# LuZWCHA/MLIC

Measured on AMD Instinct MI355X. Metric: images/sec (enc+dec) at 1920×1088 MLICPP_L, 1/2/4/8 GPU; bpp/PSNR Δ vs ref, higher is better.
Workload: dtype f32 (dense convs: f32 via split-fp16 MFMA, 3 terms); 1 GPU; config 2: MLICPP_L compress+decompress of 1920x1088 images (full rANS bitstreams, inputs resident in HBM); model=MLICPP_L, global_batch=32, per_gpu_images=32, weights=rate set(s) [1] of synthetic.RATE_LAMBDAS, parallelism=image-sharded x1 (no cross-GPU context), request_streams=4, schedule=each request stream runs its K steps back to back (no per-step join)

## Files before the change

include/mlic_hip.h:

```cpp
#ifndef MLIC_HIP_H
#define MLIC_HIP_H
#include <stddef.h>
#include <stdint.h>

#ifdef __cplusplus
extern "C" {
#endif

typedef struct mlic_model mlic_model;

const char* mlic_last_error(void);
const char* mlic_version(void);

int mlic_create(const char* model_name, int n, const char* const* names, const float* const* ptrs,
                const int64_t* shapes, const int* ndims, void* stream, mlic_model** out);
int mlic_destroy(mlic_model* m);

int mlic_forward(mlic_model* m, void* stream, const float* x, int B, int H, int W, float* x_hat, float* y_lik,
                 float* z_lik, float vbr_scale);
int mlic_forward_v(mlic_model* m, void* stream, const float* x, int B, int H, int W, float* x_hat, float* y_lik,
                   float* z_lik, const float* vbr_scales);

int mlic_set_entropy_tables(mlic_model* m, const int32_t* gc_cdf, const int32_t* gc_len, const int32_t* gc_off,
                            int gc_n, int gc_stride, const int32_t* eb_cdf, const int32_t* eb_len,
                            const int32_t* eb_off, int eb_n, int eb_stride);

int mlic_set_lanes(mlic_model* m, int lanes);
int mlic_set_priority_base(mlic_model* m, int base);
int mlic_compress(mlic_model* m, void* stream, const float* x, int B, int H, int W, float vbr_scale);
int mlic_compress_v(mlic_model* m, void* stream, const float* x, int B, int H, int W, const float* vbr_scales);
int mlic_encoded_size(mlic_model* m, int b, size_t* y_len, size_t* z_len);
int mlic_encoded_copy(mlic_model* m, int b, uint8_t* y, uint8_t* z);
int mlic_encoded_streams(mlic_model* m, int b, int64_t* n_y, int64_t* n_z, int32_t* y_sym, int32_t* y_idx,
                         int32_t* z_sym);
int mlic_encoded_bits(mlic_model* m, int b, double* y_bits, double* z_bits);
int mlic_batch_stream(mlic_model* m, int first, int count, uint8_t* out, size_t cap, size_t* len);
int mlic_decompress_batch_stream(mlic_model* m, void* stream, const uint8_t* y, size_t y_len, const uint8_t* const* z,
                                 const size_t* z_len, int B, int hz, int wz, float* x_hat, const float* vbr_scales);
int mlic_decompress(mlic_model* m, void* stream, const uint8_t* const* y, const size_t* y_len,
                    const uint8_t* const* z, const size_t* z_len, int B, int hz, int wz, float* x_hat,
                    float vbr_scale);
int mlic_decompress_v(mlic_model* m, void* stream, const uint8_t* const* y, const size_t* y_len,
                      const uint8_t* const* z, const size_t* z_len, int B, int hz, int wz, float* x_hat,
                      const float* vbr_scales);

int mlic_forward_g(mlic_model* m, void* stream, const float* x, int B, int H, int W, float* x_hat, float* y_lik,
                   float* z_lik, const float* gain_plane);
int mlic_compress_g(mlic_model* m, void* stream, const float* x, int B, int H, int W, const float* gain_plane);
int mlic_decompress_g(mlic_model* m, void* stream, const uint8_t* const* y, const size_t* y_len,
                      const uint8_t* const* z, const size_t* z_len, int B, int hz, int wz, float* x_hat,
                      const float* gain_plane);
int mlic_image_roi_levels_u8(void* stream, const uint8_t* mask, const int64_t* mask_strides, int B, int H, int W, int lo,
                             int hi, uint8_t* levels);
int mlic_roi_gain_plane(void* stream, const uint8_t* levels, int B, int hz, int wz, const float* gains_host,
                        int n_levels, float* g);
int mlic_image_sq_err_roi_u8(void* stream, const uint8_t* a, const int64_t* a_strides, const uint8_t* b,
                             const int64_t* b_strides, const uint8_t* mask, const int64_t* mask_strides, int B, int H,
                             int W, uint64_t* out);

int mlic_run_module(mlic_model* m, void* stream, const char* which, int idx, const float* in0, const float* in1,
                    int B, int Cin, int H, int W, float* out);
int mlic_workspace_bytes(mlic_model* m, size_t* arena, size_t* weights);

int mlic_set_precision(mlic_model* m, int precision);
int mlic_set_synthesis_precision(mlic_model* m, int mode);
int mlic_set_poison(mlic_model* m, int on);
int mlic_set_kernel_option(const char* name, int value);
int mlic_get_kernel_option(const char* name, int* value);
int mlic_ab_families(int* built);
int mlic_range_fallbacks(mlic_model* m, int64_t* forward_full, int64_t* forward_gs, int64_t* decompress_gs,
                         int reset);
int mlic_set_profiling(mlic_model* m, int on);
int mlic_profile_read(mlic_model* m, int cat, int64_t* launches, double* ms, double* flops, double* bytes);
int mlic_profile_layers(mlic_model* m, char* buf, size_t cap, size_t* written);

int mlic_profile_categories(int* n);
int mlic_host_stats(mlic_model* m, double* enc_ms, double* dec_ms, double* wait_ms, int reset);
int mlic_profile_category_name(int cat, char* buf, size_t cap);

int mlic_conv_run(void* stream, int impl, const float* x, const float* w, const float* bias, float* y, int B, int Cin,
                  int Cout, int H, int W, int K, int stride, int epi, const float* aux, const float* res);
int mlic_conv_choice(int B, int Cin, int Cout, int H, int W, int K, int stride, int epi, int* impl);
int mlic_dw_run(void* stream, const float* x, const float* w, const float* bias, float* y, int B, int C, int H, int W,
                int stride, int gelu);
int mlic_dwpw_run(void* stream, const float* x, const float* dww, const float* dwb, const float* w, const float* bias,
                  float* y, int B, int C, int Cout, int H, int W, int epi, const float* res);
int mlic_bench_conv(int impl, int B, int Cin, int Cout, int H, int W, int K, int stride, int epi, int iters,
                    double* ms_per, double* tflops);
int mlic_local_attn_mask(void* stream, float* out, int H, int W);
int mlic_local_attn_run(void* stream, int impl, const float* qkv, const float* rel_table, const int32_t* rel_index,
                        float* out, int C, int H, int W, int B, float scale);
int mlic_local_attn_packed_run(void* stream, const float* qkv, const float* rel_table, const int32_t* rel_index,
                               uint16_t* out, int H, int W, int B, float scale);
int mlic_local_attn_packed_half_run(void* stream, const float* qkv, const float* rel_table, const int32_t* rel_index,
                                    uint16_t* out, int H, int W, int B, float scale, int ckbd);
int mlic_linatt_splits(int HW, int* nsplit);
int mlic_linear_attention_run(void* stream, const float* k, const float* v, const float* q, float* out, float* ctx_out,
                              int B, int heads, int hd, int H, int W, int nsplit, int kmask, int qmask);
int mlic_linatt_pack_run(void* stream, const float* q, const float* ctx, uint16_t* out_halves, int B, int heads, int hd,
                         int H, int W, int K, int qmask);
int mlic_ln_channels_run(void* stream, const float* x, const float* gamma, const float* beta, float* y, int B, int C,
                         int HW);
int mlic_taps_gather_run(void* stream, const float* part, const float* bias, float* out, int B, int H, int W);
int mlic_image_sq_err_u8(void* stream, const float* a, const float* b, int B, int64_t n_per, double* out);
int mlic_ms_ssim_scratch_bytes(int B, int C, int H, int W, size_t* bytes);
int mlic_image_ms_ssim_u8(void* stream, const float* a, const int64_t* a_strides, const float* b,
                          const int64_t* b_strides, int B, int C, int H, int W, void* scratch,
                          size_t scratch_bytes, double* out, double* terms);

typedef struct mlic_lpips mlic_lpips;
int mlic_lpips_create(int n, const char* const* names, const float* const* ptrs, const int64_t* shapes,
                      const int* ndims, void* stream, mlic_lpips** out);
int mlic_lpips_destroy(mlic_lpips* h);
int mlic_lpips_set_precision(mlic_lpips* h, int precision);
int mlic_lpips_scratch_bytes(int B, int H, int W, size_t* bytes);
int mlic_image_lpips_u8(mlic_lpips* h, void* stream, const float* a, const int64_t* a_strides, const float* b,
                        const int64_t* b_strides, int B, int H, int W, void* scratch, size_t scratch_bytes,
                        double* out, double* terms);
int mlic_lpips_profile(mlic_lpips* h, int on, double* ms3);
int mlic_lpips_range_fallbacks(mlic_lpips* h, int64_t* count, int reset);

typedef struct mlic_dists mlic_dists;
int mlic_dists_create(int n, const char* const* names, const float* const* ptrs, const int64_t* shapes,
                      const int* ndims, void* stream, mlic_dists** out);
int mlic_dists_destroy(mlic_dists* h);
int mlic_dists_set_precision(mlic_dists* h, int precision);
int mlic_dists_scratch_bytes(int B, int H, int W, size_t* bytes);
int mlic_image_dists_u8(mlic_dists* h, void* stream, const float* a, const int64_t* a_strides, const float* b,
                        const int64_t* b_strides, int B, int H, int W, void* scratch, size_t scratch_bytes,
                        double* out, double* terms);
int mlic_dists_profile(mlic_dists* h, int on, double* ms3);
int mlic_dists_range_fallbacks(mlic_dists* h, int64_t* count, int reset);

int mlic_image_ingest_u8(void* stream, const uint8_t* src, const int64_t* src_strides, int B, int H, int W, float* dst,
                         int Hp, int Wp);
int mlic_image_egress_u8(void* stream, const float* src, const int64_t* src_strides, int B, int H, int W, uint8_t* dst,
                         const int64_t* dst_strides, const uint8_t* ref, const int64_t* ref_strides, uint64_t* sq_err);
int mlic_image_blur3_pad(void* stream, const float* src, const int32_t* src_index, int n, int H, int W, int Hp, int Wp,
                         const float* w9, float* dst);

typedef struct mlic_container_info {
  uint32_t H, W;
  uint32_t hz, wz;
  int32_t level;
  int32_t reserved;
  uint64_t y_off, y_len;
  uint64_t z_off, z_len;
} mlic_container_info;
int mlic_container_bytes(size_t y_len, size_t z_len, int vbr, size_t* bytes);
int mlic_container_write(uint32_t H, uint32_t W, int level, uint32_t hz, uint32_t wz, const uint8_t* y, size_t y_len,
                         const uint8_t* z, size_t z_len, uint8_t* out, size_t cap, size_t* len);
int mlic_container_parse(const uint8_t* data, size_t n, int vbr, int n_levels, uint64_t max_pixels,
                         mlic_container_info* info);

typedef struct mlic_container_roi_info {
  mlic_container_info file;
  uint64_t map_off, map_len;
} mlic_container_roi_info;
int mlic_container_write_roi(uint32_t H, uint32_t W, int level, uint32_t hz, uint32_t wz, const uint8_t* y,
                             size_t y_len, const uint8_t* z, size_t z_len, const uint8_t* levels, uint8_t* out,
                             size_t cap, size_t* len);
int mlic_container_parse_roi(const uint8_t* data, size_t n, int n_levels, uint64_t max_pixels,
                             mlic_container_roi_info* info, uint8_t* levels, size_t levels_cap);

// ... 45 lines not shown
```

mlic_amd/_lib.py:

```python
from __future__ import annotations

import ctypes as C
import os
import threading

_HERE = os.path.dirname(os.path.abspath(__file__))
LIB_PATH = os.environ.get("MLIC_HIP_LIB", os.path.join(_HERE, "libmlic_hip.so"))

_lock = threading.Lock()
_lib = None


class MlicError(RuntimeError):
    pass


class ContainerInfo(C.Structure):
    _fields_ = [("H", C.c_uint32), ("W", C.c_uint32), ("hz", C.c_uint32), ("wz", C.c_uint32), ("level", C.c_int32),
                ("reserved", C.c_int32), ("y_off", C.c_uint64), ("y_len", C.c_uint64), ("z_off", C.c_uint64),
                ("z_len", C.c_uint64)]


class ContainerRoiInfo(C.Structure):
    _fields_ = [("file", ContainerInfo), ("map_off", C.c_uint64), ("map_len", C.c_uint64)]


class ContainerTiledInfo(C.Structure):
    _fields_ = [("H", C.c_uint32), ("W", C.c_uint32), ("T", C.c_uint32), ("V", C.c_uint32), ("ny", C.c_uint32),
                ("nx", C.c_uint32), ("vbr", C.c_int32), ("reserved", C.c_int32), ("table_off", C.c_uint64),
                ("payload_off", C.c_uint64), ("payload_len", C.c_uint64)]


def _sig(lib):
    p, i, i64, f, sz = C.c_void_p, C.c_int, C.c_int64, C.c_float, C.c_size_t
    P = C.POINTER
    lib.mlic_last_error.restype = C.c_char_p
    lib.mlic_version.restype = C.c_char_p
    sigs = {
        "mlic_create": [C.c_char_p, i, P(C.c_char_p), P(p), P(i64), P(i), p, P(p)],
        "mlic_destroy": [p],
        "mlic_forward": [p, p, p, i, i, i, p, p, p, f],
        "mlic_forward_v": [p, p, p, i, i, i, p, p, p, p],
        "mlic_compress_v": [p, p, p, i, i, i, p],
        "mlic_decompress_v": [p, p, P(p), P(sz), P(p), P(sz), i, i, i, p, p],
        "mlic_set_entropy_tables": [p, p, p, p, i, i, p, p, p, i, i],
        "mlic_compress": [p, p, p, i, i, i, f],
        "mlic_encoded_size": [p, i, P(sz), P(sz)],
        "mlic_encoded_copy": [p, i, p, p],
        "mlic_encoded_streams": [p, i, P(i64), P(i64), p, p, p],
        "mlic_decompress": [p, p, P(p), P(sz), P(p), P(sz), i, i, i, p, f],
        "mlic_run_module": [p, p, C.c_char_p, i, p, p, i, i, i, i, p],
        "mlic_workspace_bytes": [p, P(sz), P(sz)],
        "mlic_local_attn_mask": [p, p, i, i],
        "mlic_set_profiling": [p, i],
        "mlic_set_lanes": [p, i],
        "mlic_set_priority_base": [p, i],
        "mlic_set_precision": [p, i],
        "mlic_set_synthesis_precision": [p, i],
        "mlic_set_poison": [p, i],
        "mlic_set_kernel_option": [C.c_char_p, i],
        "mlic_get_kernel_option": [C.c_char_p, P(i)],
        "mlic_ab_families": [P(i)],
        "mlic_batch_stream": [p, i, i, p, sz, P(sz)],
        "mlic_decompress_batch_stream": [p, p, p, sz, P(p), P(sz), i, i, i, p, p],
        "mlic_range_fallbacks": [p, P(i64), P(i64), P(i64), i],
        "mlic_profile_layers": [p, p, sz, P(sz)],
        "mlic_bench_conv": [i, i, i, i, i, i, i, i, i, i, P(C.c_double), P(C.c_double)],
        "mlic_profile_read": [p, i, P(i64), P(C.c_double), P(C.c_double), P(C.c_double)],
        "mlic_profile_categories": [P(i)],
        "mlic_host_stats": [p, P(C.c_double), P(C.c_double), P(C.c_double), i],
        "mlic_profile_category_name": [i, p, sz],
        "mlic_conv_run": [p, i, p, p, p, p, i, i, i, i, i, i, i, i, p, p],
        "mlic_conv_choice": [i, i, i, i, i, i, i, i, P(i)],
        "mlic_dw_run": [p, p, p, p, p, i, i, i, i, i, i],
        "mlic_dwpw_run": [p, p, p, p, p, p, p, i, i, i, i, i, i, p],
        "mlic_local_attn_run": [p, i, p, p, p, p, i, i, i, i, f],
        "mlic_local_attn_packed_run": [p, p, p, p, p, i, i, i, f],
        "mlic_local_attn_packed_half_run": [p, p, p, p, p, i, i, i, f, i],
        "mlic_linatt_splits": [i, P(i)],
        "mlic_linear_attention_run": [p, p, p, p, p, p, i, i, i, i, i, i, i, i],
        "mlic_linatt_pack_run": [p, p, p, p, i, i, i, i, i, i, i],
        "mlic_ln_channels_run": [p, p, p, p, p, i, i, i],
        "mlic_taps_gather_run": [p, p, p, p, i, i, i],
        "mlic_image_sq_err_u8": [p, p, p, i, i64, p],
        "mlic_ms_ssim_scratch_bytes": [i, i, i, i, P(sz)],
        "mlic_image_ms_ssim_u8": [p, p, P(i64), p, P(i64), i, i, i, i, p, sz, p, p],
        "mlic_lpips_create": [i, P(C.c_char_p), P(p), P(i64), P(i), p, P(p)],
        "mlic_lpips_destroy": [p],
        "mlic_lpips_set_precision": [p, i],
        "mlic_lpips_scratch_bytes": [i, i, i, P(sz)],
        "mlic_image_lpips_u8": [p, p, p, P(i64), p, P(i64), i, i, i, p, sz, p, p],
        "mlic_lpips_range_fallbacks": [p, P(i64), i],
        "mlic_lpips_profile": [p, i, P(C.c_double)],
        "mlic_dists_create": [i, P(C.c_char_p), P(p), P(i64), P(i), p, P(p)],
        "mlic_dists_destroy": [p],
        "mlic_dists_set_precision": [p, i],
        "mlic_dists_scratch_bytes": [i, i, i, P(sz)],
        "mlic_image_dists_u8": [p, p, p, P(i64), p, P(i64), i, i, i, p, sz, p, p],
        "mlic_dists_range_fallbacks": [p, P(i64), i],
        "mlic_dists_profile": [p, i, P(C.c_double)],
        "mlic_image_ingest_u8": [p, p, P(i64), i, i, i, p, i, i],
        "mlic_image_egress_u8": [p, p, P(i64), i, i, i, p, P(i64), p, P(i64), p],
        "mlic_image_blur3_pad": [p, p, p, i, i, i, i, i, p, p],
        "mlic_container_bytes": [sz, sz, i, P(sz)],
        "mlic_container_write": [C.c_uint32, C.c_uint32, i, C.c_uint32, C.c_uint32, p, sz, p, sz, p, sz, P(sz)],
        "mlic_container_parse": [p, sz, i, i, C.c_uint64, P(ContainerInfo)],
        "mlic_forward_g": [p, p, p, i, i, i, p, p, p, p],
        "mlic_compress_g": [p, p, p, i, i, i, p],
        "mlic_decompress_g": [p, p, P(p), P(sz), P(p), P(sz), i, i, i, p, p],
        "mlic_image_roi_levels_u8": [p, p, P(i64), i, i, i, i, i, p],
        "mlic_roi_gain_plane": [p, p, i, i, i, P(f), i, p],
        "mlic_image_sq_err_roi_u8": [p, p, P(i64), p, P(i64), p, P(i64), i, i, i, p],
        "mlic_container_write_roi": [C.c_uint32, C.c_uint32, i, C.c_uint32, C.c_uint32, p, sz, p, sz, p, p, sz, P(sz)],
        "mlic_container_parse_roi": [p, sz, i, C.c_uint64, P(ContainerRoiInfo), p, sz],
        "mlic_tile_grid": [C.c_uint32, C.c_uint32, C.c_uint32, C.c_uint32, P(C.c_uint32), P(C.c_uint32), p, sz],
        "mlic_image_tile_blend_u8": [p, p, p, i, i, i, i, i, i, i, i, p, P(i64), p, P(i64), p],
        "mlic_container_write_tiled": [C.c_uint32, C.c_uint32, C.c_uint32, C.c_uint32, i, p, p, sz, p, sz, P(sz)],
        "mlic_container_parse_tiled": [p, sz, C.c_uint64, P(ContainerTiledInfo)],
        "mlic_container_tiled_tile": [p, sz, P(ContainerTiledInfo), C.c_uint64, P(C.c_uint64), P(C.c_uint64)],
        "mlic_encode_image_u8": [p, p, p, P(i64), i, i, f, i, p, sz, P(sz)],
        "mlic_encode_image_u8_budget": [p, p, p, P(i64), i, i, f, i, C.c_double, i, p, sz, P(sz), P(i)],
        "mlic_decode_image_u8": [p, p, p, sz, i, C.c_uint64, p, p, P(i64), sz, P(i), P(i), P(i)],
        "mlic_neglog2_sum": [p, p, i, i64, p],
        "mlic_gaussian_likelihood": [p, p, p, p, i64, f, p],
        "mlic_scale_indexes": [p, p, i64, p, i, p],
        "mlic_encoded_bits": [p, i, P(C.c_double), P(C.c_double)],
        "mlic_pmf_to_quantized_cdf": [p, i, i, p],
        "mlic_rans_encode": [p, p, i64, p, p, p, i, i, p, sz, P(sz)],
        "mlic_rans_decode": [p, sz, p, i64, p, p, p, i, i, p],
        "mlic_rans_decode_narrow": [p, sz, p, i64, i, p, p, p, i, i, p, P(i)],
    }
    for name, args in sigs.items():
        fn = getattr(lib, name)
        fn.argtypes = args
        fn.restype = C.c_int
    return lib


def _check_build_record():
    import json
    from . import build as _build
    if os.environ.get("MLIC_HIP_LIB"):
        return
    rec_path = _build.RECORD
    if not os.path.exists(rec_path):
        raise MlicError(f"{rec_path} missing: rebuild with `python -m mlic_amd.build` (records the sources the "
                        f"library was built from)")
    with open(rec_path) as f:
        rec = json.load(f)
    if rec.get("sources_sha256") != _build.source_digest():
        raise MlicError("libmlic_hip.so was built from other sources than the ones in this tree (stale build): "
                        "rebuild with `python -m mlic_amd.build`")


def lib():
# ... 30 lines not shown
```

mlic_amd/csrc/capi.cpp:

```cpp
#include "../../include/mlic_hip.h"

#include <algorithm>
#include <cmath>
#include <cstring>
#include <string>
#include <vector>

#include "container.h"
#include "model.h"
#include "options.h"

using namespace mlic;

struct mlic_model {
  Model* impl;
  float* stage = nullptr;
  size_t stage_bytes = 0;
  float* stage2 = nullptr;
  size_t stage2_bytes = 0;
  int enc_H = 0, enc_W = 0, enc_level = -1;
  int enc_passes = 0;
};

struct mlic_lpips {
// ... 462 lines not shown

int mlic_conv_choice(int B, int Cin, int Cout, int H, int W, int K, int stride, int epi, int* impl) {
  return guard([&] {
    MLIC_CHECK(impl && B > 0 && Cin > 0 && Cout > 0 && H > 0 && W > 0 && (K == 1 || K == 3 || K == 5) && stride > 0,
               "conv_choice: bad arguments");
    const int pad = K / 2;
    ConvParams P{};
    P.nseg = 1;
    P.seg[0] = {nullptr, Cin, (int64_t)Cin * H * W};
    P.Cin = Cin; P.H = H; P.W = W; P.Cout = Cout; P.K = K; P.stride = stride; P.pad = pad;
    P.Ho = (H + 2 * pad - K) / stride + 1;
    P.Wo = (W + 2 * pad - K) / stride + 1;
    P.B = B;
    P.epi = epi;
    const int cin_pad = (Cin + 31) / 32 * 32;
    static const _Float16 tag = 0;
    const bool split = Cin >= 16;
    const bool x4 = split && Cout >= 64;
    const ConvWeights cw{nullptr, split ? &tag : nullptr, split ? &tag : nullptr, cin_pad, x4 ? &tag : nullptr, 0};
    *impl = conv_select(P, cw, 2);
  });
}

int mlic_conv_run(void* stream, int impl, const float* x, const float* w, const float* bias, float* y, int B, int Cin,
                  int Cout, int H, int W, int K, int stride, int epi, const float* aux, const float* res) {
  return guard([&] {
    hipStream_t st = (hipStream_t)stream;
    const int pad = K / 2;
    const int Ho = (H + 2 * pad - K) / stride + 1, Wo = (W + 2 * pad - K) / stride + 1;
    const int cin_pad = (Cin + 31) / 32 * 32;
    const int64_t nw = (int64_t)Cout * Cin * K * K, nh = (int64_t)Cout * K * K * cin_pad;
    float* wp = nullptr;
    _Float16 *wh = nullptr, *wl = nullptr;
    HIP_OK(hipMallocAsync((void**)&wp, nw * 4, st));
    HIP_OK(hipMallocAsync((void**)&wh, nh * 2, st));
    HIP_OK(hipMallocAsync((void**)&wl, nh * 2, st));
    pack_conv(w, wp, Cout, Cin, K * K, st);
    const int wexp = split_weights(w, wh, wl, Cout, Cin, K * K, cin_pad, true, st);
    ConvParams P{};
    P.nseg = 1;
    P.seg[0] = {x, Cin, (int64_t)Cin * H * W};
    P.Cin = Cin; P.H = H; P.W = W; P.Cout = Cout; P.Ho = Ho; P.Wo = Wo; P.K = K; P.stride = stride; P.pad = pad;
    P.wpk = wp; P.bias = bias; P.out = y; P.B = B; P.epi = epi;
    const bool shuffle = (epi & EPI_SHUFFLE) != 0;
    MLIC_CHECK(!shuffle || Cout % 4 == 0, "shuffle needs Cout % 4 == 0");
    P.out_cs = shuffle ? (int64_t)4 * Ho * Wo : (int64_t)Ho * Wo;
    P.out_bs = (int64_t)Cout * Ho * Wo;
    MLIC_CHECK(!(epi & (EPI_GDN | EPI_IGDN)) || aux, "GDN epilogue needs aux");
    MLIC_CHECK(!(epi & EPI_RES) || res, "residual epilogue needs res");
    P.aux = aux; P.aux_bs = (int64_t)Cout * Ho * Wo;
    P.res = res; P.res_bs = P.out_bs;
    _Float16 *wx = nullptr, *wxh = nullptr;
    if (conv_x4_ok(P, cin_pad)) {
      HIP_OK(hipMallocAsync((void**)&wx, x4_weight_halves(Cout, K * K, cin_pad) * 2, st));
      x4_pack_weights(wh, wl, Cout, K * K, cin_pad, wx, st);
      if (impl == CONV_X4H) {
        HIP_OK(hipMallocAsync((void**)&wxh, x4_weight_halves(Cout, K * K, cin_pad, true) * 2, st));
        x4_pack_weights(wh, wl, Cout, K * K, cin_pad, wxh, st, true);
      }
    }
    ConvWeights cw{wp, wh, wl, cin_pad, wx, wexp};
    cw.wx4h = wxh;
    const int which = impl < 0 ? conv_select(P, cw, 2) : impl;
    if (which == CONV_X4H) MLIC_CHECK(conv_x4_ok(P, cin_pad), "x4: unsupported shape");
    if (which == CONV_PW) MLIC_CHECK(pw_resident_ok(P, cin_pad), "pw_resident: unsupported shape");
    if (which == CONV_NARROW) MLIC_CHECK(conv_narrow_ok(P), "narrow: unsupported shape");
    if (which == CONV_SMALLCIN) MLIC_CHECK(conv_smallcin_ok(P), "smallcin: unsupported shape");
    if (which == CONV_HALO) MLIC_CHECK(conv_halo_ok(P, cin_pad), "halo: unsupported shape");
    if (which == CONV_X4) MLIC_CHECK(conv_x4_ok(P, cin_pad), "x4: unsupported shape");
    void* ws = nullptr;
    const int64_t wsb = conv_ws_bytes(which, P, cw);
    if (wsb > 0) HIP_OK(hipMallocAsync(&ws, wsb, st));
    conv_run(which, P, cw, st, ws);
    if (ws) HIP_OK(hipFreeAsync(ws, st));
    if (wx) HIP_OK(hipFreeAsync(wx, st));
    if (wxh) HIP_OK(hipFreeAsync(wxh, st));
    HIP_OK(hipFreeAsync(wp, st));
    HIP_OK(hipFreeAsync(wh, st));
    HIP_OK(hipFreeAsync(wl, st));
    HIP_OK(hipStreamSynchronize(st));
  });
}

int mlic_dw_run(void* stream, const float* x, const float* w, const float* bias, float* y, int B, int C, int H, int W,
                int stride, int gelu) {
  return guard([&] {
    DwParams P{};
    P.nseg = 1;
    P.seg[0] = {x, C, (int64_t)C * H * W};
    P.C = C; P.H = H; P.W = W; P.stride = stride;
    P.Ho = (H - 1) / stride + 1;
    P.Wo = (W - 1) / stride + 1;
    P.w = w; P.bias = bias; P.out = y; P.out_bs = (int64_t)C * P.Ho * P.Wo; P.gelu = gelu; P.B = B;
    dw3x3(P, (hipStream_t)stream);
    HIP_OK(hipStreamSynchronize((hipStream_t)stream));
  });
}

int mlic_dwpw_run(void* stream, const float* x, const float* dww, const float* dwb, const float* w, const float* bias,
                  float* y, int B, int C, int Cout, int H, int W, int epi, const float* res) {
  return guard([&] {
    hipStream_t st = (hipStream_t)stream;
    const int cin_pad = (C + 31) / 32 * 32;
    const int64_t nh = (int64_t)Cout * cin_pad;
    _Float16 *wh = nullptr, *wl = nullptr;
    HIP_OK(hipMallocAsync((void**)&wh, nh * 2, st));
    HIP_OK(hipMallocAsync((void**)&wl, nh * 2, st));
    const int wexp = split_weights(w, wh, wl, Cout, C, 1, cin_pad, true, st);
    ConvParams P{};
    P.nseg = 1;
    P.seg[0] = {x, C, (int64_t)C * H * W};
    P.Cin = C; P.H = H; P.W = W; P.Cout = Cout; P.Ho = H; P.Wo = W; P.K = 1; P.stride = 1; P.pad = 0;
    P.wexp = wexp; P.bias = bias; P.out = y; P.B = B; P.epi = epi;
    P.out_cs = (int64_t)H * W;
    P.out_bs = (int64_t)Cout * H * W;
    MLIC_CHECK(!(epi & EPI_RES) || res, "residual epilogue needs res");
    P.res = res; P.res_bs = P.out_bs;
    MLIC_CHECK(dwpw_ok(P, cin_pad), "dwpw: unsupported shape");
    dwpw_forward(P, wh, wl, cin_pad, dww, dwb, st);
    HIP_OK(hipFreeAsync(wh, st));
    HIP_OK(hipFreeAsync(wl, st));
    HIP_OK(hipStreamSynchronize(st));
  });
}

int mlic_local_attn_run(void* stream, int impl, const float* qkv, const float* rel_table, const int32_t* rel_index,
                        float* out, int C, int H, int W, int B, float scale) {
  return guard([&] {
    LocalAttnParams A{};
    A.qkv = qkv;
    A.qkv_bs = (int64_t)3 * C * H * W;
    A.out = out;
    A.out_bs = (int64_t)25 * C * H * W;
    A.rel_table = rel_table;
    A.rel_index = rel_index;
    A.scale = scale;
    A.C = C; A.H = H; A.W = W; A.B = B;
    if (impl == 0) local_attn_valu(A, (hipStream_t)stream);
    else local_attn_mfma(A, (hipStream_t)stream);
    HIP_OK(hipStreamSynchronize((hipStream_t)stream));
  });
}

int mlic_local_attn_packed_run(void* stream, const float* qkv, const float* rel_table, const int32_t* rel_index,
                               uint16_t* out, int H, int W, int B, float scale) {
  return guard([&] {
    LocalAttnParams A{};
    A.qkv = qkv;
    A.qkv_bs = (int64_t)3 * 32 * H * W;
    A.rel_table = rel_table;
    A.rel_index = rel_index;
    A.scale = scale;
    A.C = 32; A.H = H; A.W = W; A.B = B;
    local_attn_packed(A, reinterpret_cast<_Float16*>(out), (H * W + 31) / 32 * 32, (hipStream_t)stream);
    HIP_OK(hipStreamSynchronize((hipStream_t)stream));
  });
}

int mlic_local_attn_packed_half_run(void* stream, const float* qkv, const float* rel_table, const int32_t* rel_index,
                                    uint16_t* out, int H, int W, int B, float scale, int ckbd) {
  return guard([&] {
    MLIC_CHECK(ckbd == 1 || ckbd == 2, "ckbd: 1 (anchors) or 2 (non-anchors)");
    LocalAttnParams A{};
    A.qkv = qkv;
    A.qkv_bs = (int64_t)3 * 32 * H * W;
    A.rel_table = rel_table;
// ... 602 lines not shown
```

mlic_amd/csrc/common.h:

```cpp
#pragma once
#include <hip/hip_runtime.h>

#include <atomic>
#include <cstdint>
#include <cstdio>
#include <stdexcept>
#include <string>

namespace mlic {

struct Error : std::runtime_error {
  using std::runtime_error::runtime_error;
};

#define MLIC_CHECK(cond, msg)                                                                  \
  do {                                                                                          \
    if (!(cond)) throw ::mlic::Error(std::string("mlic: ") + (msg) + " [" #cond "] at " +       \
                                     __FILE__ + ":" + std::to_string(__LINE__));               \
  } while (0)

#define HIP_OK(expr)                                                                            \
  do {                                                                                          \
    hipError_t _e = (expr);                                                                     \
    if (_e != hipSuccess)                                                                       \
      throw ::mlic::Error(std::string("hip: ") + hipGetErrorString(_e) + " in " #expr " at " + \
                          __FILE__ + ":" + std::to_string(__LINE__));                           \
  } while (0)

struct View {
  float* p = nullptr;
  int C = 0, H = 0, W = 0;
  int64_t bs = 0;
  int64_t hw() const { return (int64_t)H * W; }
  View ch(int c0, int nc) const {
    View v = *this;
    v.p = p + (int64_t)c0 * hw();
    v.C = nc;
    return v;
  }
};

enum Epi : int {
  EPI_NONE = 0,
  EPI_GELU = 1,
  EPI_GDN = 2,
  EPI_IGDN = 4,
  EPI_TANH_HALF = 8,
  EPI_MASK_ANCHOR = 16,
  EPI_MASK_NONANCHOR = 32,
  EPI_RES = 64,
  EPI_SHUFFLE = 128,
  EPI_SQUARE_IN = 256,
  EPI_RELU_IN = 512,
};

constexpr int MAXSEG = 6;

struct Seg {
  const float* p;
  int C;
  int64_t bs;
};

struct ConvParams {
  Seg seg[MAXSEG];
  int nseg;
  int Cin, H, W;
  int Cout, Ho, Wo;
  int K, stride, pad;
  const float* wpk;
  int wexp;
  const float* bias;
  float* out;
  int64_t out_bs;
  int64_t out_cs;
  int epi;
  const float* aux;
  int64_t aux_bs;
  const float* res;
  int64_t res_bs;
  int B;
  int* rflag;
  int in_mask;
  int scatter;
  const float* skx;
  int64_t skx_bs;
  int sk_cin, sk_H, sk_W;
  const float* skw;
  const float* skb;
};

__device__ __forceinline__ float softmax_exp(float x) { return __builtin_amdgcn_exp2f(x * 1.44269504088896341f); }

template <int HD>
__device__ __forceinline__ void query_softmax(const float* qp, int HW, float (&q)[HD]) {
  float mx = -3.0e38f;
#pragma unroll
  for (int c = 0; c < HD; ++c) {
    q[c] = qp[(int64_t)c * HW];
    mx = fmaxf(mx, q[c]);
  }
  float sum = 0.0f;
#pragma unroll
  for (int c = 0; c < HD; ++c) {
    q[c] = softmax_exp(q[c] - mx);
    sum += q[c];
  }
  const float inv = 1.0f / sum;
#pragma unroll
  for (int c = 0; c < HD; ++c) q[c] *= inv;
}

__device__ __forceinline__ bool f16_unsafe(float v) { return (__float_as_uint(v) & 0x7fffffffu) >= 0x477ff000u; }
__device__ __forceinline__ void range_report(int* flag, bool bad) {
  if (bad && flag) atomicOr(flag, 1);
}
__device__ __forceinline__ float gelu_erf(float x) {
  const float ax = __builtin_fabsf(x);
  const float z = ax * 0.70710678118654752440f;
  const float t = __builtin_amdgcn_rcpf(__builtin_fmaf(0.3275911f, z, 1.0f));
  float q = __builtin_fmaf(0.5307027101516724f, t, -0.726576030254364f);
  q = __builtin_fmaf(q, t, 0.710706889629364f);
  q = __builtin_fmaf(q, t, -0.14224836230278015f);
  q = __builtin_fmaf(q, t, 0.1274147927761078f);
  q = q * t;
  const float e = __builtin_amdgcn_exp2f(z * (z * -1.44269504088896341f));
  return __builtin_fmaxf(x, 0.0f) - ax * (q * e);
}
typedef float mlic_float2 __attribute__((ext_vector_type(2)));
__device__ __forceinline__ mlic_float2 gelu_erf2(mlic_float2 x) {
  const mlic_float2 ax = {__builtin_fabsf(x.x), __builtin_fabsf(x.y)};
  const mlic_float2 z = ax * 0.70710678118654752440f;
  const mlic_float2 d = __builtin_elementwise_fma(mlic_float2{0.3275911f, 0.3275911f}, z, mlic_float2{1.0f, 1.0f});
  const mlic_float2 t = {__builtin_amdgcn_rcpf(d.x), __builtin_amdgcn_rcpf(d.y)};
  mlic_float2 q = __builtin_elementwise_fma(mlic_float2{0.5307027101516724f, 0.5307027101516724f}, t,
                                            mlic_float2{-0.726576030254364f, -0.726576030254364f});
  q = __builtin_elementwise_fma(q, t, mlic_float2{0.710706889629364f, 0.710706889629364f});
  q = __builtin_elementwise_fma(q, t, mlic_float2{-0.14224836230278015f, -0.14224836230278015f});
  q = __builtin_elementwise_fma(q, t, mlic_float2{0.1274147927761078f, 0.1274147927761078f});
  q = q * t;
  const mlic_float2 zz = z * (z * -1.44269504088896341f);
  const mlic_float2 e = {__builtin_amdgcn_exp2f(zz.x), __builtin_amdgcn_exp2f(zz.y)};
  const mlic_float2 m = {__builtin_fmaxf(x.x, 0.0f), __builtin_fmaxf(x.y, 0.0f)};
  return m - ax * (q * e);
}
__device__ __forceinline__ float gelu_erff(float x) { return 0.5f * x * (1.0f + erff(x * 0.70710678118654752440f)); }
__device__ __forceinline__ float gelu_epi(float x) {
#ifndef MLIC_GELU_EPI_ERFF
  return gelu_erf(x);
#else
  return gelu_erff(x);
#endif
}

__device__ __forceinline__ float gdn_apply(float x, float v, bool inverse) {
  return inverse ? x * __builtin_amdgcn_sqrtf(v) : x * __builtin_amdgcn_rsqf(v);
}

__device__ __forceinline__ bool is_anchor(int h, int w) { return ((h + w) & 1) == 1; }

__device__ __forceinline__ void conv_store(const ConvParams& P, int b, int co, int p, float v) {
  const int epi = P.epi;
  const int HWo = P.Ho * P.Wo;
  v = ldexpf(v, -P.wexp);
  if (P.bias) v += P.bias[co];
  if (epi & EPI_GELU) v = gelu_epi(v);
  if (epi & (EPI_GDN | EPI_IGDN)) {
    const float x = P.aux[(int64_t)b * P.aux_bs + (int64_t)co * HWo + p];
    v = gdn_apply(x, v, (epi & EPI_GDN) == 0);
  }
  if (epi & EPI_TANH_HALF) v = 0.5f * tanhf(v);
  int oh = 0, ow = 0;
  if (epi & (EPI_MASK_ANCHOR | EPI_MASK_NONANCHOR | EPI_SHUFFLE)) {
    oh = p / P.Wo;
    ow = p - oh * P.Wo;
  }
  if (epi & EPI_MASK_ANCHOR) v = is_anchor(oh, ow) ? v : 0.0f;
  if (epi & EPI_MASK_NONANCHOR) v = is_anchor(oh, ow) ? 0.0f : v;
  int64_t off;
  if (epi & EPI_SHUFFLE) {
    const int oc = co >> 2;
    const int y2 = 2 * oh + ((co >> 1) & 1), x2 = 2 * ow + (co & 1);
    off = (int64_t)oc * P.out_cs + (int64_t)y2 * (2 * P.Wo) + x2;
  } else {
    off = (int64_t)co * P.out_cs + p;
  }
  if (epi & EPI_RES) v = P.res[(int64_t)b * P.res_bs + off] + v;
  P.out[(int64_t)b * P.out_bs + off] = v;
}

__host__ __device__ __forceinline__ bool conv_vec_ok(const ConvParams& P) {
  const uintptr_t a = reinterpret_cast<uintptr_t>(P.out) | reinterpret_cast<uintptr_t>(P.aux) |
                      reinterpret_cast<uintptr_t>(P.res);
  return (a & 15) == 0 && ((P.out_bs | P.out_cs | P.aux_bs | P.res_bs) & 3) == 0 && (P.Wo & 3) == 0;
}

__device__ __forceinline__ void conv_store4(const ConvParams& P, int b, int co, int p, float4 v) {
  const int epi = P.epi;
  float a[4] = {v.x, v.y, v.z, v.w};
  const float bi = P.bias ? P.bias[co] : 0.0f;
#pragma unroll
  for (int e = 0; e < 4; ++e) {
    a[e] = ldexpf(a[e], -P.wexp) + bi;
    if (epi & EPI_GELU) a[e] = gelu_epi(a[e]);
  }
  if (epi & (EPI_GDN | EPI_IGDN)) {
    const float4 x = *reinterpret_cast<const float4*>(P.aux + (int64_t)b * P.aux_bs + (int64_t)co * P.Ho * P.Wo + p);
    const float xs[4] = {x.x, x.y, x.z, x.w};
#pragma unroll
    for (int e = 0; e < 4; ++e) a[e] = gdn_apply(xs[e], a[e], (epi & EPI_GDN) == 0);
  }
  if (epi & EPI_TANH_HALF) {
#pragma unroll
    for (int e = 0; e < 4; ++e) a[e] = 0.5f * tanhf(a[e]);
  }
  if (epi & (EPI_MASK_ANCHOR | EPI_MASK_NONANCHOR)) {
    const int oh = p / P.Wo, ow = p - oh * P.Wo;
#pragma unroll
    for (int e = 0; e < 4; ++e) {
      const bool anc = is_anchor(oh, ow + e);
      if ((epi & EPI_MASK_ANCHOR) && !anc) a[e] = 0.0f;
      if ((epi & EPI_MASK_NONANCHOR) && anc) a[e] = 0.0f;
    }
  }
  const int64_t off = (int64_t)co * P.out_cs + p;
  if (epi & EPI_RES) {
    const float4 r = *reinterpret_cast<const float4*>(P.res + (int64_t)b * P.res_bs + off);
    a[0] = r.x + a[0]; a[1] = r.y + a[1]; a[2] = r.z + a[2]; a[3] = r.w + a[3];
  }
  *reinterpret_cast<float4*>(P.out + (int64_t)b * P.out_bs + off) = make_float4(a[0], a[1], a[2], a[3]);
}

__device__ __forceinline__ void conv_store_shuf4(const ConvParams& P, int b, int co0, int p, float4 v) {
  const int epi = P.epi;
  float a[4] = {v.x, v.y, v.z, v.w};
  const float b0 = P.bias ? P.bias[co0] : 0.0f, b1 = P.bias ? P.bias[co0 + 1] : 0.0f;
  a[0] = ldexpf(a[0], -P.wexp) + b0; a[1] = ldexpf(a[1], -P.wexp) + b1;
  a[2] = ldexpf(a[2], -P.wexp) + b0; a[3] = ldexpf(a[3], -P.wexp) + b1;
#pragma unroll
  for (int e = 0; e < 4; ++e) {
    if (epi & EPI_GELU) a[e] = gelu_epi(a[e]);
    if (epi & EPI_TANH_HALF) a[e] = 0.5f * tanhf(a[e]);
  }
  const int oh = p / P.Wo, ow = p - oh * P.Wo;
  const int64_t off = (int64_t)(co0 >> 2) * P.out_cs + (int64_t)(2 * oh + ((co0 >> 1) & 1)) * (2 * P.Wo) + 2 * ow;
  if (epi & EPI_RES) {
    const float4 r = *reinterpret_cast<const float4*>(P.res + (int64_t)b * P.res_bs + off);
    a[0] = r.x + a[0]; a[1] = r.y + a[1]; a[2] = r.z + a[2]; a[3] = r.w + a[3];
  }
  *reinterpret_cast<float4*>(P.out + (int64_t)b * P.out_bs + off) = make_float4(a[0], a[1], a[2], a[3]);
}

inline int device_cu_count() {
  static std::atomic<int> cache[64];
  int dev = 0;
  HIP_OK(hipGetDevice(&dev));
  MLIC_CHECK(dev >= 0 && dev < 64, "device id");
  int n = cache[dev].load(std::memory_order_relaxed);
  if (n == 0) {
    HIP_OK(hipDeviceGetAttribute(&n, hipDeviceAttributeMultiprocessorCount, dev));
    cache[dev].store(n, std::memory_order_relaxed);
  }
  return n;
}

}
```

mlic_amd/csrc/conv_dispatch.cpp:

```cpp
#include "kernels.h"

namespace mlic {

static bool x4_k_on(int K) {
  static const int mask = [] {
    const char* e = opt_str(OPT_X4_K);
    int m = 0;
    for (const char* c = e ? e : "135"; *c; ++c)
      if (*c >= '0' && *c <= '9') m |= 1 << (*c - '0');
    return m;
  }();
  return (mask >> K) & 1;
}

int conv_select(const ConvParams& P, const ConvWeights& w, int precision) {
  if (P.in_mask || P.scatter) return CONV_PW;
  if (conv_smallcin_ok(P)) return CONV_SMALLCIN;
  if (conv_narrow_ok(P)) return CONV_NARROW;
  if (precision == 0 || !w.wh) return CONV_F32;
  if (precision == 1) return CONV_X3;
  if ((int64_t)P.Ho * P.Wo >= 1024 && pw_resident_ok(P, w.cin_pad)) return CONV_PW;
  const bool big1 = (int64_t)P.Cin * P.Cout >= (1 << 18), mid1 = P.Cin >= 192 && P.Cout >= 192;
  const bool x4_shape = P.K == 1 ? (big1 || mid1) : P.Cout >= 64;
  if (w.wx4 && opt(OPT_X4) && x4_k_on(P.K) && x4_shape && conv_x4_ok(P, w.cin_pad)) return CONV_X4;
  if (P.K == 5 && conv_halo_ok(P, w.cin_pad) &&
      (int64_t)((P.Cout + 127) / 128) * ((P.Wo + 31) / 32) * ((P.Ho + 3) / 4) >= 8)
    return CONV_HALO;
  return CONV_X3V2;
}

int conv_prof_cat(int impl, const ConvParams& P) {
  switch (impl) {
    case CONV_F32: return PCAT_CONV_F32 + conv_variant(P);
    case CONV_X3: return PCAT_CONV_X3 + conv_f16x3_variant(P);
    case CONV_X3V2: {
      const int v = conv_x3v2_variant(P);
      return v == 3 ? PCAT_CONV_X3V2_WIDE : PCAT_CONV_X3V2 + v;
    }
    case CONV_PW: return PCAT_CONV_PW;
    case CONV_NARROW: return PCAT_CONV_NARROW;
    case CONV_HALO: return PCAT_CONV_HALO;
    case CONV_X4:
    case CONV_X4H: return PCAT_CONV_X4;
    default: return PCAT_CONV_SMALLCIN;
  }
}

int64_t conv_ws_bytes(int impl, const ConvParams& P, const ConvWeights& w) {
  if (impl != CONV_X4 && impl != CONV_X4H) return 0;
  const bool hi = impl == CONV_X4H;
  const int64_t act = x4_direct_ok(P, hi) ? 0 : (2 * x4_act_halves(P, w.cin_pad, hi) + 255) / 256 * 256;
  return act + x4_part_bytes(P, w.cin_pad, hi);
}

void conv_run(int impl, const ConvParams& P0, const ConvWeights& w, hipStream_t st, void* ws) {
  ConvParams P = P0;
  const bool split = impl == CONV_X3 || impl == CONV_X3V2 || impl == CONV_PW || impl == CONV_HALO || impl == CONV_X4 ||
                     impl == CONV_X4H;
  P.wexp = split ? w.wexp : 0;
  MLIC_CHECK(!(P.epi & EPI_RELU_IN) || impl == CONV_X4 || impl == CONV_X4H,
             "EPI_RELU_IN: only x4's operand pack applies it");
  switch (impl) {
    case CONV_F32: conv_forward(P, st); break;
    case CONV_X3: conv_f16x3_forward(P, w.wh, w.wl, w.cin_pad, st); break;
    case CONV_X3V2: conv_x3v2_forward(P, w.wh, w.wl, w.cin_pad, st); break;
    case CONV_PW: pw_resident_forward(P, w.wh, w.wl, w.cin_pad, st); break;
    case CONV_NARROW: conv_narrow_forward(P, st); break;
    case CONV_SMALLCIN: conv_smallcin_forward(P, st); break;
    case CONV_HALO: conv_halo_forward(P, w.wh, w.wl, w.cin_pad, st); break;
    case CONV_X4:
    case CONV_X4H: {
      const bool hi = impl == CONV_X4H;
      const _Float16* wx = hi ? w.wx4h : w.wx4;
      const bool direct = x4_direct_ok(P, hi);
      MLIC_CHECK((ws || direct) && wx, "conv_x4: workspace and packed weights required");
      _Float16* act = direct ? nullptr : static_cast<_Float16*>(ws);
      const int64_t abytes = direct ? 0 : (2 * x4_act_halves(P, w.cin_pad, hi) + 255) / 256 * 256;
      float* part = x4_part_bytes(P, w.cin_pad, hi) > 0 ? reinterpret_cast<float*>(static_cast<char*>(ws) + abytes)
                                                         : nullptr;
      if (!direct) x4_pack_act(P, w.cin_pad, act, st, hi);
      conv_x4_forward(P, act, wx, w.cin_pad, st, part, hi);
      break;
    }
    default: throw Error("mlic: unknown conv implementation " + std::to_string(impl));
  }
}

const char* prof_cat_name(int cat) {
  static const char* names[PCAT_COUNT] = {
      "conv_mfma_kernel<64,64>",     "conv_mfma_kernel<64,128>",  "conv_mfma_kernel<128,64>",
      "conv_mfma_kernel<128,128>",   "conv_f16x3_kernel<32,256>", "conv_f16x3_kernel<64,128>",
      "conv_f16x3_kernel<128,64>",   "conv_f16x3_kernel<128,128>", "conv_x3v2_kernel<64,128>",
      "conv_x3v2_kernel<128,256>",   "conv_x3v2_kernel<128,128>", "conv_x3v2_kernel<256,256>",
      "pw_resident_kernel",
      "conv3x3_narrow_kernel",       "conv1x1_smallcin_kernel",   "conv_halo_kernel",
      "dw3x3_kernel",
      "local_attn_kernel",           "linear_attention",          "elementwise",
      "conv_x4_kernel",              "chain_kernel",              "dwpw_kernel"};
  return (cat >= 0 && cat < PCAT_COUNT) ? names[cat] : "";
}

}
```

mlic_amd/csrc/conv_pw.hip:

```cpp
#include "common.h"
#include "kernels.h"

namespace mlic {

typedef float floatx16 __attribute__((ext_vector_type(16)));
typedef _Float16 half8 __attribute__((ext_vector_type(8)));

constexpr int PW_WAVES = 8;
constexpr int PW_THREADS = PW_WAVES * 64;
constexpr int LDS_BYTES = 160 * 1024;

__device__ __forceinline__ __amdgpu_buffer_rsrc_t make_rsrc(const float* base, uint32_t bytes) {
  const uint64_t a = reinterpret_cast<uint64_t>(base);
  const uint32_t lo = __builtin_amdgcn_readfirstlane((uint32_t)a);
  const uint32_t hi = __builtin_amdgcn_readfirstlane((uint32_t)(a >> 32));
  float* pb = reinterpret_cast<float*>(((uint64_t)hi << 32) | lo);
  return __builtin_amdgcn_make_buffer_rsrc(pb, 0, bytes, 0x00020000);
}

__device__ __forceinline__ void opaque(uint32_t& v) { asm volatile("" : "+s"(v)); }

template <int CIN>
constexpr int pw_apitch() { return CIN + 8; }

template <int CIN, int CT, int MODE, bool RES, int XF = 0>
__global__ __launch_bounds__(PW_THREADS) void pw_resident_kernel(ConvParams P, const _Float16* __restrict__ wh,
                                                                  const _Float16* __restrict__ wl, int cin_pad) {
  constexpr int KS = CIN / 16;
  constexpr int APITCH = pw_apitch<CIN>();
  constexpr int ROWS = CT * 32;
  constexpr int A_SZ = ROWS * APITCH;
  static_assert(CIN % 16 == 0 && 2 * A_SZ * 2 + ROWS * 4 <= LDS_BYTES, "pw_resident: weights must fit in LDS");
  __shared__ __attribute__((aligned(16))) _Float16 sm[2 * A_SZ + 2 * ROWS];
  float* sbias = reinterpret_cast<float*>(sm + 2 * A_SZ);

  const int tid = threadIdx.x;
  constexpr int QPR = CIN / 8;
  constexpr int NIT = (ROWS * QPR + PW_THREADS - 1) / PW_THREADS;
  uint4 wst[2 * NIT];
#pragma unroll
  for (int it = 0; it < NIT; ++it) {
    const int id = tid + it * PW_THREADS;
    const int row = id / QPR, q = id - row * QPR;
    wst[2 * it] = wst[2 * it + 1] = make_uint4(0, 0, 0, 0);
    if (id < ROWS * QPR && row < P.Cout) {
      wst[2 * it] = *reinterpret_cast<const uint4*>(wh + (int64_t)row * cin_pad + 8 * q);
      wst[2 * it + 1] = *reinterpret_cast<const uint4*>(wl + (int64_t)row * cin_pad + 8 * q);
    }
  }
  const float bias_v = (tid < ROWS && P.bias && tid < P.Cout) ? P.bias[tid] : 0.0f;
#pragma unroll
  for (int it = 0; it < NIT; ++it) {
    const int id = tid + it * PW_THREADS;
    const int row = id / QPR, q = id - row * QPR;
    if (id < ROWS * QPR) {
      *reinterpret_cast<uint4*>(sm + row * APITCH + 8 * q) = wst[2 * it];
      *reinterpret_cast<uint4*>(sm + A_SZ + row * APITCH + 8 * q) = wst[2 * it + 1];
    }
  }
  static_assert(ROWS <= PW_THREADS, "one bias per thread");
  if (tid < ROWS) sbias[tid] = bias_v;
  __syncthreads();

  const int lane = tid & 63;
  const int wave = __builtin_amdgcn_readfirstlane(tid >> 6);
  const int l32 = lane & 31, h = lane >> 5;
  const int HW = P.Ho * P.Wo;
  const int tpi = (HW + 31) >> 5;
  const int ntiles = tpi * P.B;
  const int tstride = gridDim.x * PW_WAVES;
  int tile = blockIdx.x * PW_WAVES + wave;
  if (tile >= ntiles) return;

  constexpr bool square = MODE == 2 || MODE == 3;
  const float* xbase = P.seg[0].p;
  const int64_t xbs = P.seg[0].bs;
  const uint32_t hw4 = (uint32_t)(P.H * P.W) * 4u;
  const uint32_t ho4 = (uint32_t)HW * 4u;
  const uint32_t img_bytes = (uint32_t)CIN * hw4;
  const int S = P.stride;

  auto rsrc_of = [&](int t) { return make_rsrc(xbase + (int64_t)(t / tpi) * xbs, img_bytes); };
  auto voff_of = [&](int t) {
    const int b = t / tpi;
    const int p = min(((t - b * tpi) << 5) + l32, HW - 1);
    const int pin = S == 1 ? p : (p / P.Wo) * S * P.W + (p % P.Wo) * S;
    return (uint32_t)pin * 4u + (uint32_t)(8 * h) * hw4;
  };

  constexpr int D = KS / 2;
  float ring[D][8];
  {
    const auto rs = rsrc_of(tile);
    const uint32_t vo = voff_of(tile);
#pragma unroll
    for (int j = 0; j < D; ++j)
#pragma unroll
      for (int i = 0; i < 8; ++i)
        ring[j][i] = __builtin_bit_cast(float, __builtin_amdgcn_raw_buffer_load_b32(rs, vo, (16 * j + i) * hw4, 0));
  }

  const _Float16* Ah = sm + l32 * APITCH + 8 * h;
  const _Float16* Al = Ah + A_SZ;
  bool bad = false;
  for (; tile < ntiles; tile += tstride) {
    int nt = tile + tstride;
    if (nt >= ntiles) nt = tile;
    const auto rsc = rsrc_of(tile);
// ... 6 lines not shown
      const int pt = min(((tile - bt * tpi) << 5) + l32, HW - 1);
      const int yt = pt / P.Wo;
      kin = is_anchor(yt, pt - yt * P.Wo) == (P.in_mask == 1);
    }

    floatx16 acc[CT];
#pragma unroll
    for (int c = 0; c < CT; ++c)
#pragma unroll
      for (int r = 0; r < 16; ++r) acc[c][r] = 0.0f;
    uint32_t so = (uint32_t)(16 * D) * hw4;
    opaque(so);

#pragma unroll
    for (int j = 0; j < KS; ++j) {
      half8 bh, bl;
#pragma unroll
      for (int i = 0; i < 8; ++i) {
        float v = ring[j % D][i];
        if (XF & 1) v = kin ? v : 0.0f;
        if (square) v *= v;
        const _Float16 hv = (_Float16)v;
        bh[i] = hv;
        bl[i] = (_Float16)(v - (float)hv);
      }
      if (j == KS - D) {
        so = 0;
        opaque(so);
      }
#pragma unroll
      for (int i = 0; i < 8; ++i) {
        ring[j % D][i] = __builtin_bit_cast(float, j + D < KS ? __builtin_amdgcn_raw_buffer_load_b32(rsc, voc, so, 0)
                                                              : __builtin_amdgcn_raw_buffer_load_b32(rsn, von, so, 0));
        so += (i == 7) ? 9 * hw4 : hw4;
        opaque(so);
      }
      __builtin_amdgcn_sched_barrier(0);
#ifndef MLIC_PW_ABL
#define MLIC_PW_ABL 0
#endif
      if (MLIC_PW_ABL & 1) {
        const half8 ah0 = *reinterpret_cast<const half8*>(Ah + 16 * j);
        acc[0] = __builtin_amdgcn_mfma_f32_32x32x16_f16(ah0, bh + bl, acc[0], 0, 0, 0);
        continue;
      }
#pragma unroll
      for (int c = 0; c < CT; c += 2) {
        const int c1 = (c + 1 < CT) ? c + 1 : c;
        const half8 ah0 = *reinterpret_cast<const half8*>(Ah + c * 32 * APITCH + 16 * j);
        const half8 al0 = *reinterpret_cast<const half8*>(Al + c * 32 * APITCH + 16 * j);
        const half8 ah1 = *reinterpret_cast<const half8*>(Ah + c1 * 32 * APITCH + 16 * j);
        const half8 al1 = *reinterpret_cast<const half8*>(Al + c1 * 32 * APITCH + 16 * j);
        acc[c] = __builtin_amdgcn_mfma_f32_32x32x16_f16(al0, bh, acc[c], 0, 0, 0);
        if (c1 != c) acc[c1] = __builtin_amdgcn_mfma_f32_32x32x16_f16(al1, bh, acc[c1], 0, 0, 0);
        acc[c] = __builtin_amdgcn_mfma_f32_32x32x16_f16(ah0, bl, acc[c], 0, 0, 0);
        if (c1 != c) acc[c1] = __builtin_amdgcn_mfma_f32_32x32x16_f16(ah1, bl, acc[c1], 0, 0, 0);
        acc[c] = __builtin_amdgcn_mfma_f32_32x32x16_f16(ah0, bh, acc[c], 0, 0, 0);
        if (c1 != c) acc[c1] = __builtin_amdgcn_mfma_f32_32x32x16_f16(ah1, bh, acc[c1], 0, 0, 0);
      }
    }

    const int b = tile / tpi;
    const int p = ((tile - b * tpi) << 5) + l32;
    const uint32_t cs4 = (uint32_t)P.out_cs * 4u;
    int pf = p;
    if (XF & 2) {
      const int y = p / P.Wo, q = p - y * P.Wo;
      pf = y * 2 * P.Wo + 2 * q + ((y + (P.scatter == 1 ? 1 : 0)) & 1);
    }
    const uint32_t vo_out = (uint32_t)pf * 4u + (uint32_t)(4 * h) * cs4;
    const auto rs_out = make_rsrc(P.out + (int64_t)b * P.out_bs, (uint32_t)P.Cout * cs4);
    constexpr bool gdn = MODE == 2 || MODE == 3, igdn = MODE == 3, gelu = MODE == 1, tanh_mask = MODE == 4;
    bool keep = true;
    if (tanh_mask && (P.epi & (EPI_MASK_ANCHOR | EPI_MASK_NONANCHOR))) {
      const int oh = p / P.Wo, ow = p - oh * P.Wo;
      keep = is_anchor(oh, ow) == ((P.epi & EPI_MASK_ANCHOR) != 0);
    }
    constexpr bool res = RES;
    const auto rs_aux = make_rsrc(gdn ? P.aux + (int64_t)b * P.aux_bs : P.out, gdn ? (uint32_t)P.Cout * ho4 : 0u);
    const uint32_t vo_aux = (uint32_t)p * 4u + (uint32_t)(4 * h) * ho4;
    const auto rs_res = make_rsrc(res ? P.res + (int64_t)b * P.res_bs : P.out, res ? (uint32_t)P.Cout * cs4 : 0u);
    const float* sb = sbias + 4 * h;
    const float unscale = ldexpf(1.0f, -P.wexp);
    uint32_t so_o = 0, so_a = 0;
    if (p < HW) {
#pragma unroll
      for (int c = 0; c < CT; ++c) {
        float xa[16], xr[16];
        uint32_t oo = so_o, oa = so_a;
#pragma unroll
        for (int r = 0; r < 16; ++r) {
          if (r > 0) {
            const uint32_t step = ((r & 3) == 0) ? 5u : 1u;
            oo += step * cs4;
            oa += step * ho4;
            opaque(oo);
            opaque(oa);
          }
          if (gdn) xa[r] = __builtin_bit_cast(float, __builtin_amdgcn_raw_buffer_load_b32(rs_aux, vo_aux, oa, 0));
          xr[r] = res ? __builtin_bit_cast(float, __builtin_amdgcn_raw_buffer_load_b32(rs_res, vo_out, oo, 0)) : 0.0f;
        }
        float4 bq[4];
#pragma unroll
        for (int g = 0; g < 4; ++g) bq[g] = *reinterpret_cast<const float4*>(sb + c * 32 + 8 * g);
        float v[16];
#pragma unroll
        for (int r = 0; r < 16; ++r) {
          const float4 b4 = bq[r >> 2];
          const float bv = (r & 3) == 0 ? b4.x : (r & 3) == 1 ? b4.y : (r & 3) == 2 ? b4.z : b4.w;
          float x = __builtin_fmaf(acc[c][r], unscale, bv);
          bad |= !(fabsf(x) <= 3.4e38f);
          if (gelu) x = gelu_erf(x);
          if (gdn) x = gdn_apply(xa[r], x, igdn);
          if (tanh_mask) x = keep ? 0.5f * tanhf(x) : 0.0f;
          v[r] = x + xr[r];
        }
        oo = so_o;
        if ((MLIC_PW_ABL & 2) && P.Cout > 0) {
          asm volatile("" :: "v"(v[0]), "v"(v[5]), "v"(v[10]), "v"(v[15]));
        } else
        if (c * 32 + 32 <= P.Cout) {
#pragma unroll
          for (int r = 0; r < 16; ++r) {
            if (r > 0) {
              oo += (((r & 3) == 0) ? 5u : 1u) * cs4;
              opaque(oo);
            }
            __builtin_amdgcn_raw_buffer_store_b32(__builtin_bit_cast(uint32_t, v[r]), rs_out, vo_out, oo, 0);
          }
        } else {
#pragma unroll
          for (int r = 0; r < 16; ++r) {
            if (r > 0) {
              oo += (((r & 3) == 0) ? 5u : 1u) * cs4;
              opaque(oo);
            }
            if (c * 32 + (r & 3) + 8 * (r >> 2) + 4 * h < P.Cout)
              __builtin_amdgcn_raw_buffer_store_b32(__builtin_bit_cast(uint32_t, v[r]), rs_out, vo_out, oo, 0);
          }
        }
        so_o += 32 * cs4;
        so_a += 32 * ho4;
        opaque(so_o);
        opaque(so_a);
      }
    }
  }
  range_report(P.rflag, bad);
}

static int num_cus() { return device_cu_count(); }

static int pw_mode(const ConvParams& P) {
  const int e = P.epi & ~EPI_RES;
  if (e == EPI_NONE) return 0;
  if (e == EPI_GELU) return 1;
  if (e == (EPI_GDN | EPI_SQUARE_IN)) return 2;
  if (e == (EPI_IGDN | EPI_SQUARE_IN)) return 3;
  if (e == EPI_TANH_HALF || e == (EPI_TANH_HALF | EPI_MASK_ANCHOR) || e == (EPI_TANH_HALF | EPI_MASK_NONANCHOR))
    return 4;
  return -1;
}

#define PW_ALL(X, CIN, CT) \
  X(CIN, CT, 0, 0) X(CIN, CT, 0, 1) X(CIN, CT, 1, 0) X(CIN, CT, 1, 1) \
  X(CIN, CT, 2, 0) X(CIN, CT, 2, 1) X(CIN, CT, 3, 0) X(CIN, CT, 3, 1)
#define PW_COMBOS(X)                                                                              \
  PW_ALL(X, 96, 3) PW_ALL(X, 128, 4) PW_ALL(X, 160, 5) PW_ALL(X, 192, 6)                          \
                           \
  PW_ALL(X, 48, 2)                                                                                \
                               \
  X(192, 4, 0, 0) X(96, 4, 0, 0) X(48, 4, 0, 0)                                                   \
     \
  X(224, 4, 1, 0) X(128, 1, 4, 1)                                                                 \
                                   \
  X(32, 6, 1, 0) X(64, 6, 1, 0) X(96, 6, 1, 0) X(128, 6, 1, 0) X(160, 6, 1, 0) X(192, 4, 1, 0)   \
                     \
  X(32, 1, 0, 0) X(64, 2, 0, 0) X(32, 3, 0, 0)                                                    \
        \
  X(96, 4, 1, 0) X(64, 4, 1, 0) X(128, 2, 0, 1) X(96, 2, 0, 0)
#define PW_XCOMBOS(X) X(32, 1, 0, 0, 1) X(128, 1, 4, 1, 2) X(128, 2, 0, 1, 2)

static int pw_xf(const ConvParams& P) { return (P.in_mask ? 1 : 0) | (P.scatter ? 2 : 0); }

bool pw_resident_ok(const ConvParams& P, int cin_pad) {
  if (P.K != 1 || (P.stride != 1 && P.stride != 2) || P.pad != 0 || P.nseg != 1) return false;
  const int mode = pw_mode(P);
  if (mode < 0) return false;
  if (P.Ho != (P.H - 1) / P.stride + 1 || P.Wo != (P.W - 1) / P.stride + 1) return false;
  if (P.seg[0].C != P.Cin || cin_pad < P.Cin) return false;
  if (P.stride != 1 && (mode == 2 || mode == 3 || mode == 4)) return false;
  const int64_t HW = (int64_t)P.H * P.W;
  if ((int64_t)P.Cin * HW * 4 >= (1ll << 31) || (int64_t)P.Cout * HW * 4 >= (1ll << 31)) return false;
  const int ct = (P.Cout + 31) / 32;
  const int res = (P.epi & EPI_RES) ? 1 : 0;
  if (const int xf = pw_xf(P)) {
    if (P.stride != 1 || (unsigned)P.in_mask > 2u || (unsigned)P.scatter > 2u) return false;
    if (P.scatter && ((P.epi & (EPI_MASK_ANCHOR | EPI_MASK_NONANCHOR)) || P.out_cs != 2 * HW ||
                      (int64_t)P.Cout * P.out_cs * 4 >= (1ll << 31)))
      return false;
#define MLIC_PW_XOK(CIN, CT, M, R, X) \
  if (P.Cin == CIN && ct == CT && mode == M && res == R && xf == X) return true;
    PW_XCOMBOS(MLIC_PW_XOK)
#undef MLIC_PW_XOK
    return false;
  }
#define MLIC_PW_OK(CIN, CT, M, R) \
  if (P.Cin == CIN && ct == CT && mode == M && res == R) return true;
  PW_COMBOS(MLIC_PW_OK)
#undef MLIC_PW_OK
  return false;
}

template <int CIN, int CT, int M, bool R, int XF = 0>
static void launch_pw(const ConvParams& P, const _Float16* wh, const _Float16* wl, int cin_pad, hipStream_t st) {
  const int64_t ntiles = (int64_t)((P.Ho * P.Wo + 31) / 32) * P.B;
  const int64_t want = (ntiles + PW_WAVES - 1) / PW_WAVES;
  const dim3 grid((unsigned)std::min<int64_t>(want, (int64_t)num_cus()));
  hipLaunchKernelGGL((pw_resident_kernel<CIN, CT, M, R, XF>), grid, dim3(PW_THREADS), 0, st, P, wh, wl, cin_pad);
  HIP_OK(hipGetLastError());
}

void pw_resident_forward(const ConvParams& P, const _Float16* wh, const _Float16* wl, int cin_pad, hipStream_t st) {
  MLIC_CHECK(pw_resident_ok(P, cin_pad), "pw_resident: unsupported shape");
  const int mode = pw_mode(P);
  const int ct = (P.Cout + 31) / 32;
  const int res = (P.epi & EPI_RES) ? 1 : 0;
  if (const int xf = pw_xf(P)) {
#define MLIC_PW_XRUN(CIN, CT, M, R, X)                                 \
  if (P.Cin == CIN && ct == CT && mode == M && res == R && xf == X) {  \
    launch_pw<CIN, CT, M, R != 0, X>(P, wh, wl, cin_pad, st);          \
    return;                                                            \
  }
    PW_XCOMBOS(MLIC_PW_XRUN)
#undef MLIC_PW_XRUN
  }
  if (pw3_ok(P, cin_pad)) return pw3_forward(P, wh, wl, cin_pad, st);
  MLIC_CHECK(!P.skx, "pw_resident: the computed skip residual is pw3's");
#define MLIC_PW_RUN(CIN, CT, M, R)                                  \
  if (P.Cin == CIN && ct == CT && mode == M && res == R) {          \
    launch_pw<CIN, CT, M, R != 0>(P, wh, wl, cin_pad, st);          \
    return;                                                         \
  }
  PW_COMBOS(MLIC_PW_RUN)
#undef MLIC_PW_RUN
}

constexpr int NR_TH = 16, NR_TW = 128, NR_CC = 2;
constexpr int NR_PH = NR_TH + 2, NR_PQ = NR_TW / 4 + 2;
constexpr int NR_PITCH = NR_PQ * 4;
constexpr int NR_PATCH4 = NR_CC * NR_PH * NR_PQ;
constexpr int NR_STAGE = (NR_PATCH4 + 255) / 256;

template <int COUT>
__global__ __launch_bounds__(256) void conv3x3_narrow_kernel(ConvParams P) {
  typedef float float2v __attribute__((ext_vector_type(2)));
  typedef float float4v __attribute__((ext_vector_type(4)));
  constexpr int NW = NR_CC * 9 * COUT / 2;
  static_assert(COUT % 2 == 0, "Cout pairs");
  __shared__ __attribute__((aligned(16))) float4v sp[2][NR_PATCH4];
  __shared__ __attribute__((aligned(16))) float4v swp[2][NW];
  const int tid = threadIdx.x;
  const int tx = tid & 15, ty = tid >> 4;
  const int ow0 = blockIdx.x * NR_TW, oh0 = blockIdx.y * NR_TH;
  const int b = blockIdx.z;
  const int H = P.H, W = P.W, W4 = W >> 2;
  const int64_t HW = (int64_t)H * W;
  const float4v* x4 = reinterpret_cast<const float4v*>(P.seg[0].p + (int64_t)b * P.seg[0].bs);
  const int nchunk = (P.Cin + NR_CC - 1) / NR_CC;
  const float* w = P.wpk;
  constexpr int WSTAGE = (NW + 255) / 256;

  float4v stage[NR_STAGE];
  float4v wst[WSTAGE];
  auto load = [&](int ch) {
#pragma unroll
    for (int s = 0; s < NR_STAGE; ++s) {
      const int e = tid + s * 256;
      float4v v = {0.f, 0.f, 0.f, 0.f};
      if (e < NR_PATCH4) {
        const int c = e / (NR_PH * NR_PQ), rem = e - c * (NR_PH * NR_PQ);
        const int py = rem / NR_PQ, pq = rem - py * NR_PQ;
        const int ci = ch * NR_CC + c, ih = oh0 + py - 1, iq = (ow0 >> 2) - 1 + pq;
        if (ci < P.Cin && ih >= 0 && ih < H && iq >= 0 && iq < W4) v = x4[(ci * HW >> 2) + (int64_t)ih * W4 + iq];
      }
      stage[s] = v;
    }
#pragma unroll
    for (int s = 0; s < WSTAGE; ++s) {
      const int e = tid + s * 256;
      float4v v = {0.f, 0.f, 0.f, 0.f};
      if (e < NW) {
        const int c = e / (9 * COUT / 2), rem = e - c * (9 * COUT / 2);
        const int tap = rem / (COUT / 2), cp = rem - tap * (COUT / 2);
        const int ci = ch * NR_CC + c;
        if (ci < P.Cin) {
          const float* wr = w + ((int64_t)tap * P.Cin + ci) * COUT + 2 * cp;
          v = float4v{wr[0], wr[0], wr[1], wr[1]};
        }
      }
      wst[s] = v;
    }
  };
  auto store = [&](int buf) {
#pragma unroll
    for (int s = 0; s < NR_STAGE; ++s) {
      const int e = tid + s * 256;
      if (e < NR_PATCH4) sp[buf][e] = stage[s];
    }
#pragma unroll
// ... 235 lines not shown
```

mlic_amd/csrc/conv_x4.hip:

```cpp
#include "common.h"
#include "kernels.h"

#include <cstdio>
#include <type_traits>
#include <utility>
#include <vector>

namespace mlic {

typedef float floatx4 __attribute__((ext_vector_type(4)));
typedef _Float16 half8 __attribute__((ext_vector_type(8)));

namespace {
constexpr int X4T = 512;
constexpr int TR = 8, TC = 32;
constexpr int BN = TR * TC;
constexpr int ROWB = 128;
constexpr int ROWH = 64;

#ifndef MLIC_X4_HALO_PITCH
#define MLIC_X4_HALO_PITCH 144
#endif
#ifndef MLIC_X4_HALO_SKEW
#define MLIC_X4_HALO_SKEW (MLIC_X4_HALO_PITCH == 144)
#endif
constexpr int HPITCH = MLIC_X4_HALO_PITCH;
constexpr bool HPAD = HPITCH != ROWB;
constexpr bool HSKEW = MLIC_X4_HALO_SKEW;
static_assert(HPITCH == ROWB || (HPITCH >= ROWB + 16 && HPITCH % 16 == 0), "x4 halo pitch");
static_assert(!HSKEW || HPITCH == 144, "x4 halo skew: 9-granule rows");
__host__ __device__ constexpr int hgran(int g) {
  return (HSKEW ? ((g >> 1) & 1) + (g >> 2) * 4 + (g & 1) * 16 : g) * 16;
}
constexpr int HLO = hgran(4) - hgran(0);
static_assert(hgran(5) - hgran(1) == HLO && hgran(6) - hgran(2) == HLO && hgran(7) - hgran(3) == HLO, "x4 halo lo offset");
constexpr int HTAIL = (HPAD && hgran(7) + 16 > HPITCH) ? hgran(7) + 16 - HPITCH : 0;
constexpr int x4_halo_lds(int K, int bm) {
  return 2 * bm * ROWB + 2 * (TR + K - 1) * (TC + K - 1) * HPITCH + HTAIL;
}

__device__ __forceinline__ int swz(int row) { return (row >> 1) & 7; }

__device__ __forceinline__ void glds16(const void* src, void* lds) {
  __builtin_amdgcn_global_load_lds((const __attribute__((address_space(1))) void*)src,
                                   (__attribute__((address_space(3))) void*)lds, 16, 0, 0);
}

__device__ __forceinline__ void glds16_asm(const void* src, const void* lds) {
  const uint32_t l = __builtin_amdgcn_readfirstlane(
      (uint32_t)reinterpret_cast<uintptr_t>((const __attribute__((address_space(3))) void*)lds));
  asm volatile("s_mov_b32 m0, %1\n\ts_nop 0\n\tglobal_load_lds_dwordx4 %0, off" : : "v"(src), "s"(l) : "m0");
}

__device__ __forceinline__ half8 lds_frag(const char* base, int row, int granule) {
  return *reinterpret_cast<const half8*>(base + row * ROWB + ((granule ^ swz(row)) << 4));
}
}

#ifndef MLIC_X4_ABL_RS
#define MLIC_X4_ABL_RS 0
#endif
#ifndef MLIC_X4_SPREAD
#define MLIC_X4_SPREAD 0
#endif
#ifndef MLIC_X4_STAGGER
#define MLIC_X4_STAGGER 0
#endif
template <int K, int BM, bool RS, bool HI, bool DIR = false, bool HALO = false>
__global__ __launch_bounds__(X4T) void conv_x4_kernel(ConvParams P, const _Float16* __restrict__ act,
                                                      const _Float16* __restrict__ wx, int nchunk, int H, int W,
                                                      int abl, int nsplit) {
  constexpr int KK = K * K;
  constexpr int WAVES_M = BM == 192 ? 4 : (BM == 96 || BM == 224) ? 2 : BM / 64, WAVES_N = 8 / WAVES_M;
  constexpr int WN = BN / WAVES_N;
  constexpr int TM = BM / (16 * WAVES_M), TN = WN / 16;
  constexpr int WR = 16 * TM;
  constexpr int A_BYTES = BM * ROWB, B_BYTES = BN * ROWB;
  constexpr int NAB = RS ? 2 : 3;
  constexpr int HR = TR + K - 1, HC = TC + K - 1, HLINES = HR * HC;
  constexpr int BSLOT = HALO ? HLINES * HPITCH : B_BYTES;
  constexpr int B_OFF = NAB * A_BYTES, LDS = NAB * A_BYTES + 2 * BSLOT + (HALO ? HTAIL : 0);
  static_assert(!HALO || LDS == x4_halo_lds(K, BM), "x4 halo: the launch rule's footprint");
  constexpr int NA = A_BYTES / 1024 / 8;
  constexpr int NB = B_BYTES / 1024 / 8;
  static_assert(NA >= 1 && NB == 4 && LDS <= 160 * 1024, "x4 tile");
  static_assert(!HALO || (RS && !DIR && K > 1), "x4 halo: register-staged K x K only");
  __shared__ __attribute__((aligned(1024))) char sm[LDS];

  const int tid = threadIdx.x, lane = tid & 63, wave = tid >> 6;
  const int wm = wave / WAVES_N, wn = wave % WAVES_N;
  const int pad = K / 2;
  const int npix = P.Ho * P.Wo;
  const int S = K == 1 ? 1 : P.stride;
  const int Hp = (K == 1 ? H : P.H) + 2 * pad, Wp = (K == 1 ? W : P.W) + 2 * pad;
  const int ntx = (W + TC - 1) / TC;
  const int nct = gridDim.x, npt = gridDim.y, nblk = nct * npt;
  const int bid = blockIdx.y * nct + blockIdx.x;
  int logical = bid;
  if (nblk >= 16) {
    const int xcd = bid & 7, q = nblk >> 3, r = nblk & 7;
    logical = (xcd < r ? xcd * (q + 1) : r * (q + 1) + (xcd - r) * q) + (bid >> 3);
  }
  constexpr int XG = 4;
  int ct, pt;
  if (K == 1 && nct >= 2 * XG) {
    const int band = XG * npt, g = logical / band, first = g * XG, r = logical - g * band;
    const int gs = min(XG, nct - first);
    ct = first + r % gs;
    pt = r / gs;
  } else {
    ct = logical % nct;
    pt = logical / nct;
  }
  const int oy0 = (pt / ntx) * TR, ox0 = (pt % ntx) * TC;
  const int b = blockIdx.z % P.B, split = blockIdx.z / P.B;
  const int nsteps = nchunk * KK;
  const int s0 = HALO ? split * nchunk / nsplit * KK : split * nsteps / nsplit;
  const int s1 = HALO ? (split + 1) * nchunk / nsplit * KK : (split + 1) * nsteps / nsplit;
  if (nsplit > 1) P.out += (int64_t)split * P.B * P.out_bs;

  const int64_t plane = (int64_t)Hp * Wp * ROWH;
  const _Float16* bsrc[NB];
#pragma unroll
  for (int i = 0; i < NB; ++i) {
    const int n = (wave * NB + i) * 8 + (lane >> 3);
    const int oy = min(oy0 + n / TC, H - 1), ox = min(ox0 + n % TC, W - 1);
    const int G = (lane & 7) ^ swz(n);
    bsrc[i] = act + (int64_t)b * nchunk * plane + ((int64_t)oy * S * Wp + ox * S) * ROWH + G * 8;
  }
  const _Float16* asrc = wx + ((int64_t)ct * nsteps * BM) * ROWH + (wave * NA) * 512 + lane * 8;

  auto glds_one = [&](int g, int sb, int sa, int abuf) {
    if (g < NB) {
      const int cc = sb / KK, tap = sb - cc * KK;
      const int ky = tap / K, kx = tap - ky * K;
      const int64_t d = cc * plane + ((int64_t)ky * Wp + kx) * ROWH;
      glds16_asm(bsrc[g] + d, sm + B_OFF + (sb & 1) * B_BYTES + (wave * NB + g) * 1024);
    } else {
      const int i = g - NB;
      glds16_asm(asrc + (int64_t)sa * BM * ROWH + i * 512, sm + abuf * A_BYTES + (wave * NA + i) * 1024);
    }
  };
  constexpr int NG = NA + NB;

  floatx4 acc[TM][TN];
#pragma unroll
  for (int i = 0; i < TM; ++i)
#pragma unroll
    for (int j = 0; j < TN; ++j) acc[i][j] = floatx4{0.f, 0.f, 0.f, 0.f};

  const int G = lane >> 4, l16 = lane & 15;
// ... 282 lines not shown
#pragma unroll
    for (int i = 0; i < TM; ++i) {
      const int row = wm * WR + i * 16 + l16;
      ah[i] = lds_frag(As, row, G);
      al[i] = lds_frag(As, row, G + 4);
    }
    half8 bh[2], bl[2];
    bh[0] = lds_frag(Bs, wn * WN + l16, G);
    bl[0] = lds_frag(Bs, wn * WN + l16, G + 4);
#pragma unroll
    for (int j = 0; j < TN; ++j) {
      if (!(abl & 1)) {
#pragma unroll
        for (int g = j * NG / TN; g < (j + 1) * NG / TN; ++g) glds_one(g, sb, sa, anext);
      }
      __builtin_amdgcn_sched_barrier(0);
      if (j + 1 < TN) {
        const int n = wn * WN + (j + 1) * 16 + l16;
        bh[(j + 1) & 1] = lds_frag(Bs, n, G);
        bl[(j + 1) & 1] = lds_frag(Bs, n, G + 4);
      }
      if (abl & 2) {
        asm volatile("" :: "v"(bh[j & 1]), "v"(bl[j & 1]));
        continue;
      }
#pragma unroll
      for (int i = 0; i < TM; ++i)
        acc[i][j] = __builtin_amdgcn_mfma_f32_16x16x32_f16(al[i], bh[j & 1], acc[i][j], 0, 0, 0);
#pragma unroll
      for (int i = 0; i < TM; ++i)
        acc[i][j] = __builtin_amdgcn_mfma_f32_16x16x32_f16(ah[i], bl[j & 1], acc[i][j], 0, 0, 0);
#pragma unroll
      for (int i = 0; i < TM; ++i)
        acc[i][j] = __builtin_amdgcn_mfma_f32_16x16x32_f16(ah[i], bh[j & 1], acc[i][j], 0, 0, 0);
    }

  }
  }

  constexpr int EP = WN + 4;
  asm volatile("s_waitcnt vmcnt(0)" ::: "memory");
  __syncthreads();
  if (abl & 4) {
#pragma unroll
    for (int i = 0; i < TM; ++i)
#pragma unroll
      for (int j = 0; j < TN; ++j) asm volatile("" :: "v"(acc[i][j]));
    return;
  }
  float* ep = reinterpret_cast<float*>(sm) + wave * 16 * EP;
  const int co_w = ct * BM + wm * WR;
  const bool shuf = (P.epi & EPI_SHUFFLE) != 0;
  const bool vec = conv_vec_ok(P) && !(shuf && (P.epi & (EPI_GDN | EPI_IGDN | EPI_MASK_ANCHOR | EPI_MASK_NONANCHOR)));
#pragma unroll
  for (int i = 0; i < TM; ++i) {
#pragma unroll
    for (int j = 0; j < TN; ++j)
#pragma unroll
      for (int e = 0; e < 4; ++e) ep[(4 * G + e) * EP + j * 16 + l16] = acc[i][j][e];
#pragma unroll 1
    for (int k = 0; k < WN / 16; ++k) {
      const int idx = k * 64 + lane;
      int r0, n;
      float4 v;
      if (!shuf) {
        r0 = idx / (WN / 4);
        n = 4 * (idx % (WN / 4));
        v = *reinterpret_cast<const float4*>(ep + r0 * EP + n);
      } else {
        const int combo = idx / (WN / 2);
        r0 = 4 * (combo >> 1) + 2 * (combo & 1);
        n = 2 * (idx % (WN / 2));
        const float2 c0 = *reinterpret_cast<const float2*>(ep + r0 * EP + n);
        const float2 c1 = *reinterpret_cast<const float2*>(ep + (r0 + 1) * EP + n);
        v = make_float4(c0.x, c1.x, c0.y, c1.y);
      }
      const int nn = wn * WN + n;
      const int oy = oy0 + nn / TC, ox = ox0 + nn % TC;
      const int co = co_w + i * 16 + r0;
      const int p = oy * W + ox;
      if (oy >= H || ox >= W || p >= npix) continue;
      if (!shuf) {
        if (vec && co < P.Cout && ox + 3 < W && p + 3 < npix) {
          conv_store4(P, b, co, p, v);
        } else if (co < P.Cout) {
          const float vs[4] = {v.x, v.y, v.z, v.w};
#pragma unroll
          for (int e = 0; e < 4; ++e)
            if (ox + e < W && p + e < npix) conv_store(P, b, co, p + e, vs[e]);
        }
      } else {
        if (vec && co + 1 < P.Cout && ox + 1 < W) {
          conv_store_shuf4(P, b, co, p, v);
        } else {
          if (co < P.Cout) conv_store(P, b, co, p, v.x);
          if (co + 1 < P.Cout) conv_store(P, b, co + 1, p, v.y);
          if (ox + 1 < W) {
            if (co < P.Cout) conv_store(P, b, co, p + 1, v.z);
            if (co + 1 < P.Cout) conv_store(P, b, co + 1, p + 1, v.w);
          }
        }
      }
    }
  }
}

struct X4Pack {
  Seg seg[MAXSEG];
  int nseg, Cin, H, W, pad, nchunk, square, npix;
  int relu;
  int hi;
  _Float16* dst;
  int* rflag;
};

__global__ __launch_bounds__(256) void x4_pack_act_kernel(X4Pack Q) {
  const int Hp = Q.H + 2 * Q.pad, Wp = Q.W + 2 * Q.pad;
  const int pos = blockIdx.x * 64 + (threadIdx.x & 63);
  const int g = threadIdx.x >> 6;
  const int cc = blockIdx.y, b = blockIdx.z;
  const int y = pos / Wp - Q.pad, x = pos % Wp - Q.pad;
  const bool inb = pos < Hp * Wp && y >= 0 && y < Q.H && x >= 0 && x < Q.W && y * Q.W + x < Q.npix;
  const int64_t HW = Q.npix;
  bool bad = false;
  auto load8 = [&](int ch0, float (&v)[8]) {
    int s = 0, c0 = 0;
    while (s + 1 < Q.nseg && ch0 >= c0 + Q.seg[s].C) { c0 += Q.seg[s].C; ++s; }
    const Seg sg = Q.seg[s];
    const float* src = sg.p + (int64_t)b * sg.bs + (int64_t)(ch0 - c0) * HW + (int64_t)y * Q.W + x;
#pragma unroll
    for (int j = 0; j < 8; ++j) {
      const bool ok = inb && ch0 + j < Q.Cin && ch0 - c0 + j < sg.C;
      v[j] = ok ? src[(int64_t)j * HW] : 0.0f;
      if (Q.square) v[j] *= v[j];
      if (Q.relu) v[j] = v[j] < 0.0f ? 0.0f : v[j];
      bad |= f16_unsafe(v[j]);
    }
  };
  half8 h, l;
  float v[8];
  if (Q.hi) {
    load8(cc * 64 + 8 * g, v);
#pragma unroll
    for (int j = 0; j < 8; ++j) h[j] = (_Float16)v[j];
    load8(cc * 64 + 32 + 8 * g, v);
#pragma unroll
    for (int j = 0; j < 8; ++j) l[j] = (_Float16)v[j];
  } else {
    load8(cc * 32 + 8 * g, v);
#pragma unroll
    for (int j = 0; j < 8; ++j) {
      const _Float16 hv = (_Float16)v[j];
      h[j] = hv;
      l[j] = (_Float16)(v[j] - (float)hv);
    }
  }
  constexpr int SP = ROWH + 8;
  __shared__ __attribute__((aligned(16))) _Float16 stg[64 * SP];
  const int lane = threadIdx.x & 63;
  *reinterpret_cast<half8*>(stg + lane * SP + 8 * g) = h;
  *reinterpret_cast<half8*>(stg + lane * SP + 32 + 8 * g) = l;
  __syncthreads();
  const int nlines = min(64, Hp * Wp - (int)blockIdx.x * 64);
  _Float16* d = Q.dst + (((int64_t)b * Q.nchunk + cc) * Hp * Wp + (int64_t)blockIdx.x * 64) * ROWH;
#pragma unroll
  for (int k = 0; k < 2; ++k) {
    const int q = k * 256 + threadIdx.x;
    if (q / 8 < nlines)
      *reinterpret_cast<half8*>(d + q * 8) = *reinterpret_cast<const half8*>(stg + (q / 8) * SP + (q % 8) * 8);
  }
  range_report(Q.rflag, bad);
}
// ... 148 lines not shown
                     hipStream_t st, bool hi) {
  const int64_t n = x4_weight_halves(Cout, KK, cin_pad, hi);
  hipLaunchKernelGGL(x4_pack_weights_kernel, dim3((unsigned)((n + 255) / 256)), dim3(256), 0, st, wh, wl, dst, Cout,
                     KK, cin_pad, x4_bm(Cout), n, hi ? 1 : 0);
  HIP_OK(hipGetLastError());
}
static void x4_grid(const ConvParams& P, int& H, int& W) {
  H = P.K == 1 ? (P.H * P.W + TC - 1) / TC : P.H;
  W = P.K == 1 ? TC : P.W;
}
static void x4_tgrid(const ConvParams& P, int& H, int& W) {
  H = P.K == 1 ? (P.H * P.W + TC - 1) / TC : P.Ho;
  W = P.K == 1 ? TC : P.Wo;
}

int64_t x4_act_halves(const ConvParams& P, int cin_pad, bool hi) {
  const int pad = P.K / 2;
  int H, W;
  x4_grid(P, H, W);
  return (int64_t)P.B * x4_nchunk(cin_pad, hi) * (H + 2 * pad) * (W + 2 * pad) * ROWH;
}

bool conv_x4_ok(const ConvParams& P, int cin_pad) {
  if (!(P.K == 1 || P.K == 3 || P.K == 5) || P.pad != P.K / 2) return false;
  if (!(P.stride == 1 || (P.stride == 2 && P.K == 3))) return false;
  if (P.Ho != (P.H - 1) / P.stride + 1 || P.Wo != (P.W - 1) / P.stride + 1) return false;
  if (cin_pad % 32 != 0 || cin_pad < P.Cin || P.Cout < 32) return false;
  for (int s = 0; s + 1 < P.nseg; ++s)
    if (P.seg[s].C % 16 != 0) return false;
  return true;
}

void x4_pack_act(const ConvParams& P, int cin_pad, _Float16* dst, hipStream_t st, bool hi) {
  X4Pack Q{};
  for (int s = 0; s < P.nseg; ++s) Q.seg[s] = P.seg[s];
  Q.nseg = P.nseg;
  Q.Cin = P.Cin;
  x4_grid(P, Q.H, Q.W);
  Q.npix = P.H * P.W;
  Q.pad = P.K / 2;
  Q.nchunk = x4_nchunk(cin_pad, hi);
  Q.hi = hi ? 1 : 0;
  Q.square = (P.epi & EPI_SQUARE_IN) ? 1 : 0;
  Q.relu = (P.epi & EPI_RELU_IN) ? 1 : 0;
  Q.dst = dst;
  Q.rflag = P.rflag;
  const int npos = (Q.H + 2 * Q.pad) * (Q.W + 2 * Q.pad);
  hipLaunchKernelGGL(x4_pack_act_kernel, dim3((npos + 63) / 64, Q.nchunk, P.B), dim3(256), 0, st, Q);
  HIP_OK(hipGetLastError());
}

__global__ __launch_bounds__(256) void x4_split_reduce_kernel(ConvParams P, const float* __restrict__ part,
                                                              int nsplit) {
  const int HWo = P.Ho * P.Wo;
  const int64_t n = (int64_t)P.B * P.Cout * HWo;
  const int64_t i = (int64_t)blockIdx.x * 256 + threadIdx.x;
  if (i >= n) return;
  const int p = (int)(i % HWo);
  const int64_t r = i / HWo;
  const int co = (int)(r % P.Cout), b = (int)(r / P.Cout);
  float v = part[i];
  for (int k = 1; k < nsplit; ++k) v += part[(int64_t)k * n + i];
  conv_store(P, b, co, p, v);
}

static bool x4_rs() { return opt(OPT_X4_RS) != 0; }

template <int K, int BM>
constexpr bool x4_halo_fits() {
  return K > 1 && x4_halo_lds(K, BM) <= 160 * 1024;
}
static bool x4_halo(const ConvParams& P, bool hi) {
  const int setting = opt(OPT_X4_HALO);
  if (setting == 0 || P.K == 1 || P.stride != 1) return false;
  if (P.K == 3 && setting == 5) return false;
  const int bm = x4_bm(P.Cout);
  return x4_halo_lds(P.K, bm) <= 160 * 1024;
}

bool x4_direct_ok(const ConvParams& P, bool hi) {
  return opt(OPT_X4_DIRECT) && P.K == 1 && !hi && !(P.epi & (EPI_SQUARE_IN | EPI_RELU_IN)) && x4_rs();
}

template <int K, int BM>
static void launch_x4(const ConvParams& P, const _Float16* act, const _Float16* wx, int nchunk, hipStream_t st,
                      int nsplit, bool hi) {
  int H, W;
  x4_tgrid(P, H, W);
  const int ntx = (W + TC - 1) / TC, nty = (H + TR - 1) / TR;
  dim3 grid((P.Cout + BM - 1) / BM, ntx * nty, P.B * nsplit);
  const int abl = opt(OPT_X4_ABL);
  if (K == 1 && !act)
    hipLaunchKernelGGL((conv_x4_kernel<K, BM, true, false, K == 1>), grid, dim3(X4T), 0, st, P, act, wx, nchunk, H, W,
                       abl, nsplit);
  else if (hi && x4_halo(P, hi)) {
    if constexpr (x4_halo_fits<K, BM>())
      hipLaunchKernelGGL((conv_x4_kernel<K, BM, true, true, false, true>), grid, dim3(X4T), 0, st, P, act, wx, nchunk,
                         H, W, abl, nsplit);
  } else if (hi)
    hipLaunchKernelGGL((conv_x4_kernel<K, BM, true, true>), grid, dim3(X4T), 0, st, P, act, wx, nchunk, H, W, abl,
                       nsplit);
  else if (x4_rs() && x4_halo(P, hi)) {
    if constexpr (x4_halo_fits<K, BM>())
      hipLaunchKernelGGL((conv_x4_kernel<K, BM, true, false, false, true>), grid, dim3(X4T), 0, st, P, act, wx, nchunk,
                         H, W, abl, nsplit);
  } else if (x4_rs())
    hipLaunchKernelGGL((conv_x4_kernel<K, BM, true, false>), grid, dim3(X4T), 0, st, P, act, wx, nchunk, H, W, abl,
                       nsplit);
  else if constexpr (BM != 192 && BM != 96 && BM != 224)
    hipLaunchKernelGGL((conv_x4_kernel<K, BM, false, false>), grid, dim3(X4T), 0, st, P, act, wx, nchunk, H, W, abl, 1);
  else
    hipLaunchKernelGGL((conv_x4_kernel<K, BM, true, false>), grid, dim3(X4T), 0, st, P, act, wx, nchunk, H, W, abl,
                       nsplit);
  HIP_OK(hipGetLastError());
}

int x4_splitk(const ConvParams& P, int cin_pad, bool hi) {
  if (!opt(OPT_X4_SPLITK) || !x4_rs() || P.K == 1) return 1;
  int H, W;
  x4_tgrid(P, H, W);
  const int tiles = ((P.Cout + x4_bm(P.Cout) - 1) / x4_bm(P.Cout)) * ((W + TC - 1) / TC) * ((H + TR - 1) / TR);
  const int nsteps = x4_nchunk(cin_pad, hi) * P.K * P.K;
  if (tiles > 48 || nsteps < 48) return 1;
  const int s = std::min(4, nsteps / 24);
  return x4_halo(P, hi) ? std::max(1, std::min(s, x4_nchunk(cin_pad, hi))) : s;
}

int64_t x4_part_bytes(const ConvParams& P, int cin_pad, bool hi) {
  const int s = x4_splitk(P, cin_pad, hi);
  return s > 1 ? (int64_t)s * P.B * P.Cout * P.Ho * P.Wo * 4 : 0;
}

void conv_x4_forward(const ConvParams& P, const _Float16* act, const _Float16* wx, int cin_pad, hipStream_t st,
                     float* part, bool hi) {
  MLIC_CHECK(conv_x4_ok(P, cin_pad) && wx && (act || x4_direct_ok(P, hi)), "conv_x4: unsupported shape");
  ConvParams Q = P;
  if (act) Q.epi &= ~(EPI_SQUARE_IN | EPI_RELU_IN);
  const int nchunk = x4_nchunk(cin_pad, hi);
  const int bm = x4_bm(P.Cout);
  const int nsplit = part ? x4_splitk(P, cin_pad, hi) : 1;
  ConvParams R = Q;
  if (nsplit > 1) {
    R.epi = EPI_NONE;
    R.bias = nullptr;
    R.wexp = 0;
    R.aux = nullptr;
    R.res = nullptr;
    R.out = part;
    R.out_cs = (int64_t)P.Ho * P.Wo;
    R.out_bs = (int64_t)P.Cout * R.out_cs;
  }
#define MLIC_X4_BM(K)                                                  \
  (bm == 256 ? launch_x4<K, 256>(R, act, wx, nchunk, st, nsplit, hi)       \
   : bm == 192 ? launch_x4<K, 192>(R, act, wx, nchunk, st, nsplit, hi)     \
   : bm == 96 ? launch_x4<K, 96>(R, act, wx, nchunk, st, nsplit, hi)       \
   : bm == 224 ? launch_x4<K, 224>(R, act, wx, nchunk, st, nsplit, hi)     \
   : bm == 128 ? launch_x4<K, 128>(R, act, wx, nchunk, st, nsplit, hi)     \
               : launch_x4<K, 64>(R, act, wx, nchunk, st, nsplit, hi))
  switch (P.K) {
    case 1: MLIC_X4_BM(1); break;
    case 3: MLIC_X4_BM(3); break;
    default: MLIC_X4_BM(5); break;
  }
#undef MLIC_X4_BM
  if (nsplit > 1) {
    const int64_t n = (int64_t)P.B * P.Cout * P.Ho * P.Wo;
    hipLaunchKernelGGL(x4_split_reduce_kernel, dim3((unsigned)((n + 255) / 256)), dim3(256), 0, st, Q,
                       (const float*)part, nsplit);
    HIP_OK(hipGetLastError());
  }
}

}
```

mlic_amd/csrc/kernels.h:

```cpp
#pragma once
#include "common.h"
#include "options.h"

#include <algorithm>

namespace mlic {

int conv_variant(const ConvParams& P);
void conv_forward(const ConvParams& P, hipStream_t st);

int conv_f16x3_variant(const ConvParams& P);
void conv_f16x3_forward(const ConvParams& P, const _Float16* wh, const _Float16* wl, int cin_pad, hipStream_t st);
int conv_x3v2_variant(const ConvParams& P);
void conv_x3v2_forward(const ConvParams& P, const _Float16* wh, const _Float16* wl, int cin_pad, hipStream_t st);
int split_weights(const float* w, _Float16* wh, _Float16* wl, int Cout, int Cin, int KK, int cin_pad, bool prescale,
                  hipStream_t st);

bool pw_resident_ok(const ConvParams& P, int cin_pad);
void pw_resident_forward(const ConvParams& P, const _Float16* wh, const _Float16* wl, int cin_pad, hipStream_t st);
bool conv_narrow_ok(const ConvParams& P);
void conv_narrow_forward(const ConvParams& P, hipStream_t st);
bool ab_families_built();
bool conv_halo_ok(const ConvParams& P, int cin_pad);
void conv_halo_forward(const ConvParams& P, const _Float16* wh, const _Float16* wl, int cin_pad, hipStream_t st);
void taps_gather(const float* part, int64_t part_bs, const float* bias, float* out, int64_t out_bs, int H, int W,
                 int B, hipStream_t st);
bool conv_smallcin_ok(const ConvParams& P);
void conv_smallcin_forward(const ConvParams& P, hipStream_t st);

bool dwpw_ok(const ConvParams& P, int cin_pad);
bool dwpw_grid_ok(const ConvParams& P);
bool dwpw2_ok(const ConvParams& P, int cin_pad);
bool dwpw2_lds_ok(const ConvParams& P, int cin_pad);
void dwpw2_lds_forward(const ConvParams& P, const _Float16* wh, const _Float16* wl, int cin_pad, const float* dww,
                       const float* dwb, hipStream_t st);
bool dwpw3_shape_ok(const ConvParams& P, int cin_pad);
bool pw3_ok(const ConvParams& P, int cin_pad);
void pw3_forward(const ConvParams& P, const _Float16* wh, const _Float16* wl, int cin_pad, hipStream_t st);
void dwpw3_forward(const ConvParams& P, const _Float16* wh, const _Float16* wl, int cin_pad, const float* dww,
                   const float* dwb, hipStream_t st);
void dwpw2_forward(const ConvParams& P, const _Float16* wh, const _Float16* wl, int cin_pad, const float* dww,
                   const float* dwb, hipStream_t st);
void dwpw_forward(const ConvParams& P, const _Float16* wh, const _Float16* wl, int cin_pad, const float* dww,
                  const float* dwb, hipStream_t st);

int x4_bm(int Cout);
int x4_nchunk(int cin_pad, bool hi);
int64_t x4_weight_halves(int Cout, int KK, int cin_pad, bool hi = false);
void x4_pack_weights(const _Float16* wh, const _Float16* wl, int Cout, int KK, int cin_pad, _Float16* dst,
                     hipStream_t st, bool hi = false);
int64_t x4_act_halves(const ConvParams& P, int cin_pad, bool hi = false);
bool conv_x4_ok(const ConvParams& P, int cin_pad);
void x4_pack_act(const ConvParams& P, int cin_pad, _Float16* dst, hipStream_t st, bool hi = false);
bool x4_direct_ok(const ConvParams& P, bool hi);
int x4_splitk(const ConvParams& P, int cin_pad, bool hi = false);
int64_t x4_part_bytes(const ConvParams& P, int cin_pad, bool hi = false);
void conv_x4_forward(const ConvParams& P, const _Float16* act, const _Float16* wx, int cin_pad, hipStream_t st,
                     float* part = nullptr, bool hi = false);

enum ConvImpl : int {
  CONV_F32 = 0, CONV_X3 = 1, CONV_X3V2 = 2, CONV_PW = 3, CONV_NARROW = 4, CONV_SMALLCIN = 5, CONV_HALO = 6,
  CONV_X4 = 7,
  CONV_X4H = 8
};
struct ConvWeights {
  const float* wpk;
  const _Float16* wh;
  const _Float16* wl;
  int cin_pad;
  const _Float16* wx4 = nullptr;
  int wexp = 0;
  const _Float16* wx4h = nullptr;
};
int conv_select(const ConvParams& P, const ConvWeights& w, int precision);
int64_t conv_ws_bytes(int impl, const ConvParams& P, const ConvWeights& w);
void conv_run(int impl, const ConvParams& P, const ConvWeights& w, hipStream_t st, void* ws = nullptr);

enum ProfCat : int {
  PCAT_CONV_F32 = 0,
  PCAT_CONV_X3 = 4,
  PCAT_CONV_X3V2 = 8,
  PCAT_CONV_X3V2_WIDE = 11,
  PCAT_CONV_PW = 12,
  PCAT_CONV_NARROW = 13,
  PCAT_CONV_SMALLCIN = 14,
  PCAT_CONV_HALO = 15,
  PCAT_DW = 16,
  PCAT_LOCAL = 17,
  PCAT_LINATT = 18,
  PCAT_ELEM = 19,
  PCAT_CONV_X4 = 20,
  PCAT_CHAIN = 21,
  PCAT_DWPW = 22,
  PCAT_COUNT = 23
};
int conv_prof_cat(int impl, const ConvParams& P);
const char* prof_cat_name(int cat);

struct DwParams {
  Seg seg[MAXSEG];
  int nseg;
  int C, H, W, Ho, Wo, stride;
  const float* w;
  const float* bias;
  float* out;
  int64_t out_bs;
  int gelu;
  int B;
  int ckbd;
};
void dw3x3(const DwParams& P, hipStream_t st);
bool dw_half_ok(const DwParams& P);

void ln_channels(const float* x, int64_t x_bs, float* y, int64_t y_bs, const float* g, const float* b, int C,
                 int HW, int B, hipStream_t st);

struct LocalAttnParams {
  const float* qkv;
  int64_t qkv_bs;
  float* out;
  int64_t out_bs;
  const float* rel_table;
  const int* rel_index;
  float scale;
  int C, H, W, B;
  int ckbd;
};
void local_attn(const LocalAttnParams& P, hipStream_t st);
void local_attn_mfma(const LocalAttnParams& P, hipStream_t st);
void local_attn_valu(const LocalAttnParams& P, hipStream_t st);
void local_attn_packed(const LocalAttnParams& P, _Float16* out, int npos, hipStream_t st);

inline int ctx_splits(int HW) { return std::max(1, std::min(64, HW / 256)); }
int64_t linear_attention_part_floats(int heads, int hd, int B, int nsplit);
void linear_attention(const float* K, int64_t k_bs, const float* V, int64_t v_bs, const float* Q, int64_t q_bs,
                      float* out, int64_t o_bs, float* part, float* ctx, int heads, int hd, int H, int W, int B,
                      int nsplit, int kmask, int qmask, hipStream_t st);
// ... 137 lines not shown
```

mlic_amd/csrc/model.cpp:

```cpp
#include "model.h"


#include <algorithm>
#include <cmath>
#include <cstdio>
#include <cstring>
#include <thread>

namespace mlic {

static bool gs_subpel(const std::string& name, const ConvW& w) {
  return name.rfind("g_s.", 0) == 0 && w.K == 3 && w.wh != nullptr;
}

Cfg config_for(const std::string& name) {
  Cfg c;
  c.name = name;
  if (name == "MLICPP_L" || name == "MLICPP_L_VBR") { c.N = 192; c.M = 320; c.S = 10; }
  else if (name == "MLICPP_S" || name == "MLICPP_S_VBR") { c.N = 96; c.M = 160; c.S = 5; }
  else if (name == "MLICPP_M") { c.N = 160; c.M = 256; c.S = 8; }
  else if (name == "MLICPP_S2") { c.N = 128; c.M = 128; c.S = 2; }
  else if (name == "MLICPP_M_SMALL_DEC" || name == "MLICPP_M_SMALL_DEC_VBR") { c.N = 192; c.M = 320; c.S = 10; c.sd = true; }
  else throw Error("mlic: unknown model name " + name);
  c.vbr = name.size() > 4 && name.substr(name.size() - 4) == "_VBR";
// ... 115 lines not shown
    CopyDesc* dd = nullptr;
    HIP_OK(hipMalloc(&dd, copies.size() * sizeof(CopyDesc)));
    owned_.push_back(dd);
    HIP_OK(hipMemcpyAsync(dd, copies.data(), copies.size() * sizeof(CopyDesc), hipMemcpyHostToDevice, st));
    copy_many(dd, (int)copies.size(), st);
    HIP_OK(hipStreamSynchronize(st));
  }
  for (auto& kv : convs_) {
    const std::string b = ends_with(kv.first, ".__x4perm") ? kv.first.substr(0, kv.first.size() - 9) : kv.first;
    auto it = raw_.find(b + ".bias");
    if (it != raw_.end()) kv.second.b = it->second;
  }
  for (auto& kv : dws_) {
    auto it = raw_.find(kv.first + ".bias");
    if (it != raw_.end()) kv.second.b = it->second;
  }
  for (int i = 0; i < n; ++i) {
    const std::string k = names[i];
    if (!ends_with(k, ".gamma") || ndims[i] != 2) continue;
    const std::string p = k.substr(0, k.size() - 6);
    const int C = shape(i, 0);
    float* beta_eff = take(C);
    float* gamma_pk = take((int64_t)C * C);
    float* gamma_eff = take((int64_t)C * C);
    MLIC_CHECK(off <= total, "weight block");
    gdn_prep(rw(p + ".beta"), rw(p + ".gamma"), rw(p + ".beta_reparam.lower_bound.bound"),
             rw(p + ".beta_reparam.pedestal"), rw(p + ".gamma_reparam.lower_bound.bound"),
             rw(p + ".gamma_reparam.pedestal"), beta_eff, gamma_pk, gamma_eff, C, st);
    ConvW w;
    w.w = gamma_pk;
    w.b = beta_eff;
    w.Cin = w.Cout = C;
    w.K = 1;
    w.cin_pad = (C + 31) / 32 * 32;
    const int64_t nh = (int64_t)C * w.cin_pad;
    w.wh = reinterpret_cast<_Float16*>(take((nh + 1) / 2));
    w.wl = reinterpret_cast<_Float16*>(take((nh + 1) / 2));
    MLIC_CHECK(off <= total, "weight block");
    w.wexp = split_weights(gamma_eff, w.wh, w.wl, C, C, 1, w.cin_pad, true, st);
    w.name = p + ".__gdn";
    convs_[p + ".__gdn"] = w;
  }
  MLIC_CHECK(off <= total, "weight block overflow");
  {
    int64_t nx = 0;
    for (auto& kv : convs_) {
      const ConvW& w = kv.second;
      if (w.wh && (w.K == 1 || w.K == 3 || w.K == 5) && w.Cout >= 64) {
        nx += (x4_weight_halves(w.Cout, w.K * w.K, w.cin_pad) + 127) & ~(int64_t)127;
        if (gs_subpel(kv.first, w)) nx += (x4_weight_halves(w.Cout, w.K * w.K, w.cin_pad, true) + 127) & ~(int64_t)127;
      }
    }
    if (nx > 0) {
      _Float16* xb = nullptr;
      HIP_OK(hipMalloc(&xb, nx * sizeof(_Float16)));
      owned_.push_back(xb);
      wbytes_ += nx * sizeof(_Float16);
      int64_t xo = 0;
      for (auto& kv : convs_) {
        ConvW& w = kv.second;
        if (!(w.wh && (w.K == 1 || w.K == 3 || w.K == 5) && w.Cout >= 64)) continue;
        w.wx4 = xb + xo;
        x4_pack_weights(w.wh, w.wl, w.Cout, w.K * w.K, w.cin_pad, w.wx4, st);
        xo += (x4_weight_halves(w.Cout, w.K * w.K, w.cin_pad) + 127) & ~(int64_t)127;
        if (gs_subpel(kv.first, w)) {
          w.wx4h = xb + xo;
          x4_pack_weights(w.wh, w.wl, w.Cout, w.K * w.K, w.cin_pad, w.wx4h, st, true);
          xo += (x4_weight_halves(w.Cout, w.K * w.K, w.cin_pad, true) + 127) & ~(int64_t)127;
        }
      }
    }
  }
  {
    const int win = cfg_.win, ww = win * win;
    std::vector<int> ri(ww * ww);
    for (int a = 0; a < ww; ++a)
      for (int c = 0; c < ww; ++c)
        ri[a * ww + c] = (a / win - c / win + win - 1) * (2 * win - 1) + (a % win - c % win + win - 1);
    rel_index_ = reinterpret_cast<int*>(take(ww * ww));
    HIP_OK(hipMemcpyAsync(rel_index_, ri.data(), ri.size() * 4, hipMemcpyHostToDevice, st));
  }
  add_chains(st);
  add_hoist(ep0, st);
  MLIC_CHECK(raw_.count("__scale_table"), "scale table missing");
  scale_table_ = const_cast<float*>(raw_["__scale_table"]);
  HIP_OK(hipStreamSynchronize(st));
}

void Model::add_fusion_x4(const std::string& base, const float* w_dev, int Cout, hipStream_t st) {
  constexpr int CIN = 800;
  std::vector<float> w((size_t)Cout * CIN), wp((size_t)Cout * CIN);
  HIP_OK(hipMemcpyAsync(w.data(), w_dev, w.size() * 4, hipMemcpyDeviceToHost, st));
  HIP_OK(hipStreamSynchronize(st));
  for (int co = 0; co < Cout; ++co)
    for (int c = 0; c < 32; ++c)
      for (int cell = 0; cell < 25; ++cell) wp[(size_t)co * CIN + cell * 32 + c] = w[(size_t)co * CIN + c * 25 + cell];
  const int64_t nh = (int64_t)Cout * CIN, nx = x4_weight_halves(Cout, 1, CIN);
  char* blk = nullptr;
  const size_t bytes = (size_t)nh * 4 + 2 * (size_t)nh * 2 + (size_t)nx * 2 + 1024;
  HIP_OK(hipMalloc(&blk, bytes));
  owned_.push_back(blk);
  wbytes_ += bytes;
  float* wf = reinterpret_cast<float*>(blk);
  _Float16* wh = reinterpret_cast<_Float16*>(blk + (size_t)nh * 4);
  _Float16* wl = wh + nh;
  _Float16* wx = reinterpret_cast<_Float16*>((reinterpret_cast<uintptr_t>(wl + nh) + 255) & ~(uintptr_t)255);
  HIP_OK(hipMemcpyAsync(wf, wp.data(), wp.size() * 4, hipMemcpyHostToDevice, st));
  const int wexp = split_weights(wf, wh, wl, Cout, CIN, 1, CIN, true, st);
  x4_pack_weights(wh, wl, Cout, 1, CIN, wx, st);
  HIP_OK(hipStreamSynchronize(st));
  ConvW cw;
  cw.w = wf;
  cw.Cout = Cout;
  cw.Cin = CIN;
  cw.K = 1;
  cw.wh = wh;
  cw.wl = wl;
  cw.cin_pad = CIN;
  cw.wx4 = wx;
  cw.wexp = wexp;
  cw.name = base;
  convs_[base + ".__x4perm"] = cw;
}

void Model::add_taps(const std::string& base, const float* w_dev, int Cin, hipStream_t st) {
  constexpr int C = 12;
  std::vector<float> w((size_t)C * Cin * 9), wt((size_t)9 * C * Cin);
  HIP_OK(hipMemcpyAsync(w.data(), w_dev, w.size() * 4, hipMemcpyDeviceToHost, st));
  HIP_OK(hipStreamSynchronize(st));
  for (int c = 0; c < C; ++c)
    for (int ci = 0; ci < Cin; ++ci)
      for (int t = 0; t < 9; ++t) wt[((size_t)t * C + c) * Cin + ci] = w[((size_t)c * Cin + ci) * 9 + t];
  float* tmp = nullptr;
  HIP_OK(hipMalloc(&tmp, wt.size() * 4));
  HIP_OK(hipMemcpyAsync(tmp, wt.data(), wt.size() * 4, hipMemcpyHostToDevice, st));
  convs_[base + ".__taps"] = make_conv(tmp, 9 * C, Cin, 1, base + ".__taps", st);
  HIP_OK(hipStreamSynchronize(st));
  HIP_OK(hipFree(tmp));
}

bool Model::taps_on() const {
  return opt(OPT_TAPS) && prec() == PREC_F16X3_V2;
}

void Model::add_chains(hipStream_t st) {
  std::vector<std::pair<std::string, std::vector<std::string>>> todo;
  for (auto& kv : convs_) {
    const std::string& k = kv.first;
    if (k.rfind("entropy_parameters", 0) == 0 && ends_with(k, ".fusion.0")) {
      const std::string p = k.substr(0, k.size() - 2);
      todo.push_back({p, {p + ".0", p + ".2", p + ".4", p + ".6"}});
    } else if (k.rfind("local_context", 0) == 0 && ends_with(k, ".mlp.fc1")) {
      const std::string p = k.substr(0, k.size() - 4);
      todo.push_back({p, {p + ".fc1", p + ".fc2"}});
    }
  }
  const int hyp = 2 * cfg_.hM();
  int64_t total = 0;
  std::vector<ChainW> cws;
  for (auto& t : todo) {
    ChainW c;
    c.name = t.first;
    c.nl = (int)t.second.size();
    bool ok = true;
    for (int l = 0; l < c.nl; ++l) {
      auto it = convs_.find(t.second[l]);
// ... 24 lines not shown
  owned_.push_back(blk);
  wbytes_ += (size_t)total * sizeof(_Float16);
  int64_t off = 0;
  for (ChainW& c : cws) {
    c.wimg = blk + off;
    const bool ctx = ends_with(c.name, "#ctx");
    const std::string base = ctx ? c.name.substr(0, c.name.size() - 4) : c.name;
    const auto& names = c.nl == 4 ? std::vector<std::string>{base + ".0", base + ".2", base + ".4", base + ".6"}
                                  : std::vector<std::string>{base + ".fc1", base + ".fc2"};
    for (int l = 0; l < c.nl; ++l) {
      const ConvW& w = convs_.at(names[l]);
      const int cin = l == 0 ? c.cin0 : w.Cin;
      if (cin > 0) chain_pack(w.wh, w.wl, w.Cout, cin, w.cin_pad, l > 0 ? 1 : 0, blk + off, st);
      off += chain_layer_halves(w.Cout, cin);
    }
    if (ctx) {
      c.name = base;
      chains_ctx_[base] = c;
    } else {
      chains_[c.name] = c;
    }
  }
}

ConvW Model::make_conv(const float* w_dev, int Cout, int Cin, int K, const std::string& name, hipStream_t st) {
  ConvW w;
  w.Cout = Cout;
  w.Cin = Cin;
  w.K = K;
  w.cin_pad = (Cin + 31) / 32 * 32;
  w.name = name;
  const int64_t nw = (int64_t)Cout * Cin * K * K, nh = (int64_t)Cout * K * K * w.cin_pad;
  const int64_t nx = (K == 1 || K == 3 || K == 5) && Cout >= 64 ? x4_weight_halves(Cout, K * K, w.cin_pad) : 0;
  const size_t bytes = ((size_t)nw * 4 + 255) / 256 * 256 + 2 * (((size_t)nh * 2 + 255) / 256 * 256) + (size_t)nx * 2 + 256;
  char* blk = nullptr;
  HIP_OK(hipMalloc(&blk, bytes));
  owned_.push_back(blk);
  wbytes_ += bytes;
  w.w = reinterpret_cast<float*>(blk);
  w.wh = reinterpret_cast<_Float16*>(blk + ((size_t)nw * 4 + 255) / 256 * 256);
  w.wl = w.wh + ((size_t)nh * 2 + 255) / 256 * 256 / 2;
  pack_conv(w_dev, w.w, Cout, Cin, K * K, st);
  w.wexp = split_weights(w_dev, w.wh, w.wl, Cout, Cin, K * K, w.cin_pad, true, st);
  if (nx) {
    w.wx4 = w.wl + ((size_t)nh * 2 + 255) / 256 * 256 / 2;
    x4_pack_weights(w.wh, w.wl, Cout, K * K, w.cin_pad, w.wx4, st);
  }
  return w;
}

void Model::add_hoist(const std::map<std::string, std::pair<const float*, int>>& ep0, hipStream_t st) {
  const int hyp = 2 * cfg_.hM(), S = cfg_.S;
  if ((int)ep0.size() != 2 * S || chains_ctx_.size() != (size_t)(2 * S)) return;
  const int C1 = convs_.at("entropy_parameters_anchor.0.fusion.0").Cout;
  float* tmp = nullptr;
  HIP_OK(hipMalloc(&tmp, sizeof(float) * (size_t)2 * S * C1 * hyp));
  for (int i = 0; i < S; ++i)
    for (int k = 0; k < 2; ++k) {
      const std::string p = std::string("entropy_parameters_") + (k ? "nonanchor." : "anchor.") + std::to_string(i) +
                            ".fusion.0";
      auto it = ep0.find(p);
      MLIC_CHECK(it != ep0.end() && convs_.at(p).Cout == C1, "hoist: EP layer 0");
      const float* src = it->second.first;
      const int cin = it->second.second;
      HIP_OK(hipMemcpy2DAsync(tmp + (size_t)(2 * i + k) * C1 * hyp, (size_t)hyp * 4, src + (cin - hyp), (size_t)cin * 4,
                              (size_t)hyp * 4, C1, hipMemcpyDeviceToDevice, st));
    }
  hoist_ = make_conv(tmp, 2 * S * C1, hyp, 1, "__hyper_hoist", st);
  hoist_rows_ = C1;
  HIP_OK(hipStreamSynchronize(st));
  HIP_OK(hipFree(tmp));
}

bool Model::hoist_on() const {
  const int env = opt(OPT_HOIST);
  bool want = env >= 0 ? env != 0 : false;
  if (env < 0)
    for (int i = 0; i < cfg_.S && !want; ++i)
      for (const char* k : {"anchor", "nonanchor"})
        if (!chains_.count(std::string("entropy_parameters_") + k + "." + std::to_string(i) + ".fusion")) want = true;
  return want && chain_on() && hoist_.Cout > 0;
}

bool Model::dwpw_on() const {
  return opt(OPT_DWPW) && prec() == PREC_F16X3_V2;
}

bool Model::chain_on() const {
  return opt(OPT_CHAIN) && prec() == PREC_F16X3_V2;
}

Model::~Model() {
  lanes_.clear();
  for (void* p : owned_) (void)hipFree(p);
}

Lane::~Lane() {
  if (rflag) (void)hipFree(rflag);
  for (void* p : {(void*)h_sym, (void*)h_sym16, (void*)h_idx8, (void*)hc_sym, (void*)hc_sym16, (void*)hc_idx8})
    if (p) (void)hipHostFree(p);
  if (cev) (void)hipEventDestroy(cev);
  if (cst) (void)hipStreamDestroy(cst);
  for (hipEvent_t e : ev_pool) (void)hipEventDestroy(e);
  if (own_stream && st) (void)hipStreamDestroy(st);
}

thread_local Lane* Model::tl_lane_ = nullptr;

Lane& Model::lane(int i) {
  while ((int)lanes_.size() <= i) {
    auto l = std::make_unique<Lane>();
    if (opt(OPT_LANE_PRIORITY)) {
      int least = 0, greatest = 0;
      HIP_OK(hipDeviceGetStreamPriorityRange(&least, &greatest));
      const int prio = std::min(least, greatest + prio_base_ + (int)lanes_.size());
      HIP_OK(hipStreamCreateWithPriority(&l->st, hipStreamNonBlocking, prio));
    } else {
      HIP_OK(hipStreamCreateWithFlags(&l->st, hipStreamNonBlocking));
    }
    l->own_stream = true;
    l->prof = prof_;
    HIP_OK(hipMalloc(&l->rflag, sizeof(int)));
    HIP_OK(hipMemsetAsync(l->rflag, 0, sizeof(int), l->st));
    lanes_.push_back(std::move(l));
  }
  return *lanes_[i];
}

void Model::set_lanes(int n) {
  MLIC_CHECK(n >= 1 && n <= 16, "lanes must be in [1, 16]");
  nlanes_ = n;
}

void Model::set_profiling(bool on) {
  prof_ = on;
  for (auto& l : lanes_) l->prof = on;
}

size_t Model::arena_bytes() const {
  size_t s = 0;
  for (auto& l : lanes_) s += l->arena.capacity();
  return s;
}

const ConvW& Model::cw(const std::string& k) const {
  auto it = convs_.find(k);
  if (it == convs_.end()) throw Error("mlic: missing conv weight " + k);
  return it->second;
}
const DwW& Model::dww(const std::string& k) const {
  auto it = dws_.find(k);
  if (it == dws_.end()) throw Error("mlic: missing depthwise weight " + k);
  return it->second;
}
const float* Model::rw(const std::string& k) const {
  auto it = raw_.find(k);
  if (it == raw_.end()) throw Error("mlic: missing tensor " + k);
  return it->second;
}

View Model::alloc(int C, int H, int W) {
  View v;
  v.p = L().arena.alloc((int64_t)L().B * C * H * W);
  v.C = C;
  v.H = H;
  v.W = W;
  v.bs = (int64_t)C * H * W;
  return v;
}

void Model::conv(const std::vector<View>& ins, const ConvW& w, int stride, int pad, const View& out, int epi,
                 const View* aux, const View* res) {
  const ConvParams P = conv_params(ins, w, stride, pad, out, epi, aux, res);
  run_conv(P, w, nullptr);
}

void Model::conv_pair(const std::vector<View>& ins, const ConvW& w1, const View& out1, int epi1, const ConvW& w2,
                      const View& out2, int epi2) {
  const ConvParams P1 = conv_params(ins, w1, 1, w1.K / 2, out1, epi1, nullptr, nullptr);
  const ConvParams P2 = conv_params(ins, w2, 1, w2.K / 2, out2, epi2, nullptr, nullptr);
  const ConvWeights c1{w1.w, w1.wh, w1.wl, w1.cin_pad, w1.wx4, w1.wexp}, c2{w2.w, w2.wh, w2.wl, w2.cin_pad, w2.wx4, w2.wexp};
  if (conv_select(P1, c1, prec()) != CONV_X4 || conv_select(P2, c2, prec()) != CONV_X4 ||
      w1.cin_pad != w2.cin_pad || w1.K != w2.K) {
    run_conv(P1, w1, nullptr);
    run_conv(P2, w2, nullptr);
    return;
  }
  const bool hi = gs_fp16_ && w1.wx4h && w2.wx4h;
  const size_t m = L().arena.mark();
  _Float16* act = reinterpret_cast<_Float16*>(L().arena.alloc((2 * x4_act_halves(P1, w1.cin_pad, hi) + 3) / 4));
  timed(PCAT_ELEM, 0.0, (hi ? 6.0 : 8.0) * L().B * P1.Cin * P1.H * P1.W,
        [&] { x4_pack_act(P1, w1.cin_pad, act, L().st, hi); }, w1.name + ".__x4_pack");
  run_conv(P1, w1, act, hi);
  run_conv(P2, w2, act, hi);
  L().arena.release(m);
}

void Model::run_conv(const ConvParams& P, const ConvW& w, const _Float16* packed, bool hi, bool split) {
  const ConvWeights cw{w.w, w.wh, w.wl, w.cin_pad, w.wx4, w.wexp};
  const int impl = packed ? (hi ? CONV_X4H : CONV_X4) : conv_select(P, cw, prec());
  const double outn = (double)P.B * w.Cout * P.Ho * P.Wo;
  const double flops = 2.0 * outn * P.Cin * w.K * w.K;
  const double bytes = 4.0 * ((double)P.B * P.Cin * P.H * P.W + (double)w.Cout * P.Cin * w.K * w.K +
                              outn * (1 + (P.aux ? 1 : 0) + (P.res ? 1 : 0)));
  std::string tag;
  if (L().prof) {
    char sh[96];
    std::snprintf(sh, sizeof sh, " [%d>%d k%d s%d e%x n%d]", P.Cin, P.Cout, P.K, P.stride, P.epi, P.nseg);
    tag = w.name + sh;
  }
  if (packed) {
    const int64_t pb = split ? x4_part_bytes(P, w.cin_pad, hi) : 0;
    const size_t m = L().arena.mark();
    float* part = pb > 0 ? L().arena.alloc((pb + 3) / 4) : nullptr;
    timed(conv_prof_cat(impl, P), flops, bytes,
          [&] { conv_x4_forward(P, packed, hi ? w.wx4h : w.wx4, w.cin_pad, L().st, part, hi); }, tag);
    L().arena.release(m);
    return;
  }
  const int64_t wsb = conv_ws_bytes(impl, P, cw);
  const size_t m = L().arena.mark();
  void* ws = wsb > 0 ? static_cast<void*>(L().arena.alloc((wsb + 3) / 4)) : nullptr;
  timed(conv_prof_cat(impl, P), flops, bytes, [&] { conv_run(impl, P, cw, L().st, ws); }, tag);
  L().arena.release(m);
}

ConvParams Model::conv_params(const std::vector<View>& ins, const ConvW& w, int stride, int pad, const View& out,
                              int epi, const View* aux, const View* res) {
  ConvParams P{};
  MLIC_CHECK(!ins.empty() && (int)ins.size() <= MAXSEG, "conv inputs");
  P.nseg = (int)ins.size();
  int cin = 0;
  for (int s = 0; s < P.nseg; ++s) {
    MLIC_CHECK(ins[s].H == ins[0].H && ins[s].W == ins[0].W, "concat inputs must share H, W");
    P.seg[s] = {ins[s].p, ins[s].C, ins[s].bs};
    cin += ins[s].C;
  }
  MLIC_CHECK(cin == w.Cin, "conv Cin mismatch");
  P.Cin = cin;
  P.H = ins[0].H;
  P.W = ins[0].W;
  P.Cout = w.Cout;
  P.K = w.K;
  P.stride = stride;
  P.pad = pad;
  P.Ho = (P.H + 2 * pad - w.K) / stride + 1;
  P.Wo = (P.W + 2 * pad - w.K) / stride + 1;
  P.wpk = w.w;
  P.wexp = w.wexp;
  P.rflag = L().rflag;
  P.bias = w.b;
  P.epi = epi;
  if (epi & EPI_SHUFFLE) {
    MLIC_CHECK(out.C * 4 == w.Cout && out.H == 2 * P.Ho && out.W == 2 * P.Wo, "shuffle output shape");
  } else {
    MLIC_CHECK(out.C == w.Cout && out.H == P.Ho && out.W == P.Wo, "conv output shape");
  }
  P.out = out.p;
  P.out_bs = out.bs;
  P.out_cs = out.hw();
  if (aux) {
    MLIC_CHECK(aux->C == w.Cout && aux->H == P.Ho && aux->W == P.Wo, "aux shape");
    P.aux = aux->p;
    P.aux_bs = aux->bs;
  }
  if (res) {
    MLIC_CHECK(res->C == out.C && res->H == out.H && res->W == out.W, "residual shape");
    P.res = res->p;
    P.res_bs = res->bs;
    P.epi |= EPI_RES;
  }
  P.B = L().B;
  return P;
}

DwParams Model::dw_params(const std::vector<View>& ins, const DwW& w, int stride, const View& out, bool gelu,
                          int ckbd) {
  DwParams P{};
  P.nseg = (int)ins.size();
  int c = 0;
  for (int s = 0; s < P.nseg; ++s) {
    P.seg[s] = {ins[s].p, ins[s].C, ins[s].bs};
    c += ins[s].C;
  }
  MLIC_CHECK(c == w.C && out.C == w.C, "depthwise channels");
  P.C = c;
  P.H = ins[0].H;
  P.W = ins[0].W;
  P.stride = stride;
  P.Ho = (P.H - 1) / stride + 1;
  P.Wo = (P.W - 1) / stride + 1;
  MLIC_CHECK(out.H == P.Ho && out.W * (ckbd ? 2 : 1) == P.Wo, "depthwise output shape");
  P.w = w.w;
  P.bias = w.b;
  P.out = out.p;
  P.out_bs = out.bs;
  P.gelu = gelu ? 1 : 0;
  P.B = L().B;
  P.ckbd = ckbd;
  return P;
}

void Model::dw(const std::vector<View>& ins, const DwW& w, int stride, const View& out, bool gelu, int ckbd) {
  const DwParams P = dw_params(ins, w, stride, out, gelu, ckbd);
  const double outn = (double)L().B * P.C * out.H * out.W;
  timed(PCAT_DW, 18.0 * outn, 4.0 * ((double)L().B * P.C * P.H * P.W + outn), [&] { dw3x3(P, L().st); }, w.name);
}

bool Model::dw_pw_half(const std::vector<View>& ins, const DwW& d, bool gelu, const ConvW& w, int epi, int mask_epi,
                       const View& out, const View* res, int ckbd, bool fusable) {
  const int H = ins[0].H, W = ins[0].W;
  if (W % 2 != 0 || !w.wh) return false;
  const View geo{nullptr, d.C, H, W, (int64_t)d.C * H * W};
  const ConvParams PF = conv_params({geo}, w, 1, 0, out, epi | mask_epi, nullptr, res);
  const ConvWeights cwt{w.w, w.wh, w.wl, w.cin_pad, w.wx4, w.wexp};
  if (fusable && dwpw_on() && ins.size() == 1 && dwpw_ok(PF, w.cin_pad) && dwpw_grid_ok(PF)) return false;
  if (conv_select(PF, cwt, prec()) != CONV_PW || pw3_ok(PF, w.cin_pad)) return false;
  const size_t m = L().arena.mark();
  const View sq = alloc(d.C, H, W / 2);
  const View og{out.p, out.C, H, W / 2, out.bs};
  View rg;
  if (res) rg = View{res->p, res->C, H, W / 2, res->bs};
  ConvParams PX = conv_params({sq}, w, 1, 0, og, epi, nullptr, res ? &rg : nullptr);
  PX.out_cs = out.hw();
  PX.scatter = ckbd;
  const bool ok = dw_half_ok(dw_params(ins, d, 1, sq, gelu, ckbd)) && pw_resident_ok(PX, w.cin_pad);
  if (ok) {
    dw(ins, d, 1, sq, gelu, ckbd);
    run_conv(PX, w, nullptr);
  }
  L().arena.release(m);
  return ok;
// ... 250 lines not shown
    A.qkv_bs = qkv.bs;
    A.rel_table = rw(p + ".relative_position_table");
    A.rel_index = rel_index_;
    A.scale = (float)std::pow((double)(C / 2), -0.5);
    A.C = C;
    A.H = H;
    A.W = W;
    A.B = L().B;
    A.ckbd = half ? 2 : 0;
    const double fl = (half ? 0.5 : 1.0) * pix * 2.0 * 2 * 25 * 25 * (C / 2) * 2;
    timed(PCAT_LOCAL, fl, 4.0 * pix * (3 * C + (half ? 0.5 : 1.0) * 25 * C), [&] { local_attn_packed(A, tp, npos, L().st); },
          p + ".attn");
    const View tv{nullptr, 25 * C, H, Wq, (int64_t)25 * C * H * Wq};
    run_conv(conv_params({tv}, fw, 1, 0, f, EPI_NONE, nullptr, nullptr), fw, tp);
  } else {
  View t = alloc(25 * C, H, W);
  {
    LocalAttnParams A{};
    A.qkv = qkv.p;
    A.qkv_bs = qkv.bs;
    A.out = t.p;
    A.out_bs = t.bs;
    A.rel_table = rw(p + ".relative_position_table");
    A.rel_index = rel_index_;
    A.scale = (float)std::pow((double)(C / 2), -0.5);
    A.C = C;
    A.H = H;
    A.W = W;
    A.B = L().B;
    const double fl = pix * 2.0 * 2 * 25 * 25 * (C / 2) * 2;
    timed(PCAT_LOCAL, fl, 4.0 * pix * (3 * C + 25 * C), [&] { local_attn(A, L().st); }, p + ".attn");
  }
  conv({t}, cw(p + ".fusion"), 1, 0, f, EPI_NONE);
  }
  View pj = conv1x1(f, p + ".proj", 1, EPI_NONE);
  View n2 = alloc(2 * C, H, Wq);
  const double pq = (double)L().B * H * Wq;
  timed(PCAT_ELEM, 16.0 * pq * C, 16.0 * pq * C, [&] {
    ln_channels(pj.p, pj.bs, n2.p, n2.bs, rw(p + ".norm2.weight"), rw(p + ".norm2.bias"), 2 * C, H * Wq, L().B, L().st);
  }, p + ".norm2");
  auto ch = cit;
  if (half) {
    run_chain(ch->second, {n2}, out, &pj, nullptr, 0, 0, 2, true);
  } else if (chain_on() && ch != chains_.end() && (H * W) % 4 == 0) {
    run_chain(ch->second, {n2}, out, &pj);
  } else {
    View h1 = conv1x1(n2, p + ".mlp.fc1", 1, EPI_GELU);
    conv({h1}, cw(p + ".mlp.fc2"), 1, 0, out, EPI_NONE, nullptr, &pj);
  }
  L().arena.release(m);
  return out;
}

View Model::channel_context(const View& x, int i) {
  const std::string p = "channel_context." + std::to_string(i) + ".fushion";
  const bool dwsep = !cfg_.sd;
  const int Cout = dwsep ? cw(p + ".4.point_conv").Cout : cw(p + ".4").Cout;
  View out = alloc(Cout, x.H, x.W);
  const size_t m = L().arena.mark();
  View a = conv3x3({x}, p + ".0", 1, dwsep, EPI_GELU);
  View b = conv3x3({a}, p + ".2", 1, dwsep, EPI_GELU);
  conv3x3({b}, p + ".4", 1, dwsep, EPI_NONE, nullptr, &out);
  L().arena.release(m);
  return out;
}

View Model::qkv_branch(const View& x, const std::string& p) {
  const DwW& d = dww(p + ".1");
  View out = alloc(d.C, x.H, x.W);
  const size_t m = L().arena.mark();
  View t = conv1x1(x, p + ".0", 1, EPI_NONE);
  dw({t}, d, 1, out, false);
  L().arena.release(m);
  return out;
}

View Model::inter_context(const View& x, int i) {
  const std::string p = "global_inter_context." + std::to_string(i);
  const int D = x.C, H = x.H, W = x.W, HW = H * W;
  const int heads = D / 32, hd = 32;
  const ConvW& sk = cw(p + ".skip");
  View out = alloc(sk.Cout, H, W);
  const size_t m = L().arena.mark();
  View q = qkv_branch(x, p + ".queries");
  View k = qkv_branch(x, p + ".keys");
  View v = qkv_branch(x, p + ".values");
  const ConvW& rp = cw(p + ".reprojection");
  View a = alloc(rp.Cout, H, W);
  linatt_reproject(k, v, q, heads, hd, 0, 0, rp, a, p + ".attn");
  View m1 = conv1x1(a, p + ".mlp.0", 1, EPI_GELU);
  View m2 = alloc(m1.C, H, W);
  dw({m1}, dww(p + ".mlp.2"), 1, m2, true);
  View s = conv1x1(a, p + ".skip", 1, EPI_NONE);
  conv({m2}, cw(p + ".mlp.4"), 1, 0, out, EPI_NONE, nullptr, &s);
  L().arena.release(m);
  return out;
}

void Model::linatt_reproject(const View& k, const View& v, const View& q, int heads, int hd, int kmask, int qmask,
                             const ConvW& rp, const View& a, const std::string& tag) {
  const int H = q.H, W = q.W, HW = H * W, D = heads * hd, B = L().B;
  const int nsplit = ctx_splits(HW);
  const size_t m = L().arena.mark();
  float* part = L().arena.alloc(linear_attention_part_floats(heads, hd, B, nsplit));
  float* ctx = L().arena.alloc((int64_t)B * heads * hd * hd);
  const double fl = (double)B * HW * D * hd * 4.0, by = 4.0 * B * HW * D * 4.0;
  const View geo{nullptr, D, H, W, (int64_t)D * HW};
  const ConvParams P = conv_params({geo}, rp, 1, 2, a, EPI_NONE, nullptr, nullptr);
  const ConvWeights cwt{rp.w, rp.wh, rp.wl, rp.cin_pad, rp.wx4, rp.wexp};
  if (opt(OPT_LINATT_FUSED) && rp.cin_pad == D && D % 32 == 0 && conv_select(P, cwt, prec()) == CONV_X4) {
    timed(PCAT_LINATT, fl * 0.5, 4.0 * B * HW * D * 2.0, [&] {
      linear_attention_ctx(k.p, k.bs, v.p, v.bs, part, ctx, heads, hd, H, W, B, nsplit, kmask, L().st);
    }, tag);
    _Float16* act = reinterpret_cast<_Float16*>(L().arena.alloc((2 * x4_act_halves(P, rp.cin_pad) + 3) / 4));
    timed(PCAT_LINATT, fl * 0.5, 4.0 * B * HW * D * 2.0, [&] {
      linatt_pack(q.p, q.bs, ctx, heads, hd, qmask, P, act, L().st);
    }, tag + ".pack");
    run_conv(P, rp, act, false, true);
  } else {
    View att = alloc(D, H, W);
    timed(PCAT_LINATT, fl, by, [&] {
      linear_attention(k.p, k.bs, v.p, v.bs, q.p, q.bs, att.p, att.bs, part, ctx, heads, hd, H, W, B, nsplit, kmask, qmask,
                       L().st);
    }, tag);
    conv({att}, rp, 1, 2, a, EPI_NONE);
  }
  L().arena.release(m);
}

View Model::intra_context(const View& x1, const View& x2, int i, bool half) {
  const std::string p = "global_intra_context." + std::to_string(i);
  const int D = x1.C, H = x1.H, W = x1.W, HW = H * W;
  const int heads = 2, hd = D / 2;
  const bool on = opt(OPT_INTRA_HALF) != 0;
  View out = alloc(2 * D, H, W);
  const size_t m = L().arena.mark();
  auto masked_branch = [&](const std::string& bp, int parity, View& o) {
    const ConvW& w = cw(bp + ".0");
    const DwW& d = dww(bp + ".1");
    const View geo{nullptr, w.Cout, H, W, (int64_t)w.Cout * HW};
    const ConvParams P0 = conv_params({x1}, w, 1, 0, geo, EPI_NONE, nullptr, nullptr);
    const ConvWeights cwt{w.w, w.wh, w.wl, w.cin_pad, w.wx4, w.wexp};
    ConvParams PX = P0;
    PX.in_mask = parity;
    if (!on || !w.wh || conv_select(P0, cwt, prec()) != CONV_PW || pw3_ok(P0, w.cin_pad) ||
        !pw_resident_ok(PX, w.cin_pad))
      return false;
    o = alloc(d.C, H, W);
    const size_t m3 = L().arena.mark();
    const View t = alloc(w.Cout, H, W);
    PX.out = t.p;
    PX.out_bs = t.bs;
    run_conv(PX, w, nullptr);
    dw({t}, d, 1, o, false);
    L().arena.release(m3);
    return true;
  };
  View q, k;
  {
    const size_t m2 = L().arena.mark();
    if (!masked_branch(p + ".queries", 2, q) || !masked_branch(p + ".keys", 1, k)) {
      L().arena.release(m2);
      View x1n = alloc(D, H, W);
      View x1a = alloc(D, H, W);
      timed(PCAT_ELEM, 0.0, 16.0 * L().B * D * HW, [&] {
        ckbd_mask(x1.p, x1.bs, x1n.p, x1n.bs, D, H, W, L().B, 0, L().st);
        ckbd_mask(x1.p, x1.bs, x1a.p, x1a.bs, D, H, W, L().B, 1, L().st);
      }, p + ".ckbd");
      q = qkv_branch(x1n, p + ".queries");
      k = qkv_branch(x1a, p + ".keys");
    }
  }
  View v = qkv_branch(x2, p + ".values");
  const ConvW& rp = cw(p + ".reprojection");
  View a = alloc(rp.Cout, H, W);
  linatt_reproject(k, v, q, heads, hd, 1, 2, rp, a, p + ".attn");
  View m1 = conv1x1(a, p + ".mlp.0", 1, EPI_GELU);
  if (!(on && half && dw_pw_half({m1}, dww(p + ".mlp.2"), true, cw(p + ".mlp.4"), EPI_NONE, 0, out, &a, 2, false))) {
    View m2 = alloc(m1.C, H, W);
    dw({m1}, dww(p + ".mlp.2"), 1, m2, true);
    conv({m2}, cw(p + ".mlp.4"), 1, 0, out, EPI_NONE, nullptr, &a);
  }
  L().arena.release(m);
  return out;
}

bool Model::ep_half_chain(const std::string& kind, int i, int H, int W, bool hoisted) const {
  const std::string p = "entropy_parameters_" + kind + "." + std::to_string(i) + ".fusion";
  if (!opt(OPT_EP_HALF) || W % 2 != 0 || (H * W) % 4 != 0) return false;
  return hoisted ? chains_ctx_.count(p) > 0 : (chain_on() && chains_.count(p) > 0);
}

View Model::entropy_parameters(const std::vector<View>& ctx, const View* hyper, const std::string& kind, int i,
                               const View* hoisted, bool phase_only) {
  const std::string p = "entropy_parameters_" + kind + "." + std::to_string(i) + ".fusion";
  const View& geo = ctx.empty() ? *hyper : ctx[0];
  const int H = geo.H, W = geo.W;
  const int ckbd = phase_only && opt(OPT_EP_HALF) && W % 2 == 0 ? (kind == "nonanchor" ? 2 : 1) : 0;
  const ConvW& l3 = cw(p + ".6");
  View out = alloc(l3.Cout, H, W);
  auto hc = chains_ctx_.find(p);
  if (hoisted && hc != chains_ctx_.end() && (H * W) % 4 == 0) {
    const int slot = 2 * i + (kind == "nonanchor" ? 1 : 0);
    const View aux = hoisted->ch(slot * hoist_rows_, hoist_rows_);
    run_chain(hc->second, ctx, out, nullptr, &aux, H, W, ckbd);
    return out;
  }
  std::vector<View> ins = ctx;
  if (hyper) ins.push_back(*hyper);
  auto ch = chains_.find(p);
  if (chain_on() && ch != chains_.end() && (H * W) % 4 == 0) {
    run_chain(ch->second, ins, out, nullptr, nullptr, 0, 0, ckbd);
    return out;
  }
  const size_t m = L().arena.mark();
  View a = alloc(cw(p + ".0").Cout, H, W);
  conv(ins, cw(p + ".0"), 1, 0, a, EPI_GELU);
  View b = conv1x1(a, p + ".2", 1, EPI_GELU);
  View c = conv1x1(b, p + ".4", 1, EPI_GELU);
  conv({c}, l3, 1, 0, out, EPI_NONE);
  L().arena.release(m);
  return out;
}

void Model::lrp(const std::vector<View>& ins, const std::string& kind, int i, const View& yh, bool anchor) {
  const std::string p = "lrp_" + kind + "." + std::to_string(i) + ".lrp_transform";
  const int nl = cfg_.sd ? 4 : 3;
  const size_t m = L().arena.mark();
  std::vector<View> cur = ins;
  for (int l = 0; l < nl; ++l) {
    const std::string q = p + "." + std::to_string(2 * l);
    if (l + 1 < nl) {
      View o = conv3x3(cur, q, 1, true, EPI_GELU);
      cur = {o};
    } else {
      const int mask = anchor ? EPI_MASK_ANCHOR : EPI_MASK_NONANCHOR;
      if (opt(OPT_LRP_HALF) && dw_pw_half(cur, dww(q + ".depth_conv"), false, cw(q + ".point_conv"), EPI_TANH_HALF,
                                          mask, yh, &yh, anchor ? 1 : 2, true))
        continue;
      conv3x3(cur, q, 1, true, EPI_TANH_HALF | mask, &yh, &yh);
    }
  }
  L().arena.release(m);
}
// ... 693 lines not shown
```

mlic_amd/csrc/model.h:

```cpp
#pragma once
#include <atomic>
#include <chrono>
#include <map>
#include <memory>
#include <cstring>
#include <string>
#include <vector>

#include "common.h"
#include "kernels.h"
#include "pool.h"
#include "rans.h"

namespace mlic {

struct Cfg {
  std::string name;
  int N = 0, M = 0, S = 0, C = 0, win = 5;
  bool sd = false, vbr = false;
  int hM() const { return sd ? M / 4 : M; }
  int gN() const { return sd ? N / 4 : N; }
};
Cfg config_for(const std::string& name);

struct ConvW {
  float* w = nullptr;
  const float* b = nullptr;
  int Cin = 0, Cout = 0, K = 0;
  _Float16* wh = nullptr;
  _Float16* wl = nullptr;
  int cin_pad = 0;
  _Float16* wx4 = nullptr;
  _Float16* wx4h = nullptr;
  int wexp = 0;
  std::string name;
};

struct ChainW {
  _Float16* wimg = nullptr;
  int nl = 0, cin0 = 0;
  int cout[4] = {0, 0, 0, 0};
  const float* bias[4] = {nullptr, nullptr, nullptr, nullptr};
  int wexp[4] = {0, 0, 0, 0};
  std::string name;
};

enum Precision : int { PREC_F32 = 0, PREC_F16X3 = 1, PREC_F16X3_V2 = 2 };
struct DwW {
  const float* w = nullptr;
  const float* b = nullptr;
  int C = 0;
  std::string name;
};

class Arena {
 public:
  ~Arena();
  void ensure(size_t bytes);
  float* alloc(int64_t nfloats);
  size_t mark() const { return top_; }
  void release(size_t m) { top_ = m; }
  void begin(bool dry) { dry_ = dry; top_ = 0; peak_ = 0; }
  size_t peak() const { return peak_; }
  size_t capacity() const { return cap_; }
  void poison_on(hipStream_t st) { poison_st_ = st; poison_ = true; }
  void poison_off() { poison_ = false; }

 private:
  char* base_ = nullptr;
  size_t cap_ = 0, top_ = 0, peak_ = 0;
  bool dry_ = false;
  bool poison_ = false;
  hipStream_t poison_st_ = nullptr;
};

struct ProfStat {
  int64_t launches = 0;
  double ms = 0, flops = 0, bytes = 0;
};

struct CoderView {
  const int32_t* sym = nullptr;
  const int16_t* sym16 = nullptr;
  const uint8_t* idx = nullptr;
  int64_t n_per = 0, stride = 0;
  int nph = 0;
  int64_t size() const { return n_per * nph; }
  void gather(int32_t* s, int32_t* i) const {
    for (int k = 0; k < nph; ++k) {
      for (int64_t j = 0; j < n_per; ++j) {
        if (s) s[k * n_per + j] = sym16 ? (int32_t)sym16[k * stride + j] : sym[k * stride + j];
        if (i) i[k * n_per + j] = (int32_t)idx[k * stride + j];
      }
    }
  }
  template <class E, class T>
  void put_phase(E& e, int k, const T& tables) const {
    if (sym16) e.put_reverse(sym16 + k * stride, idx + k * stride, n_per, tables);
    else e.put_reverse(sym + k * stride, idx + k * stride, n_per, tables);
  }
};

struct CoderBufs {
  int32_t* sym = nullptr;
  int16_t* sym16 = nullptr;
  uint8_t* idx8 = nullptr;
  int* ovf = nullptr;
};

struct EncodedImage {
  std::string y;
  std::string z;
  CoderView y_in;
  std::vector<int32_t> z_sym;
  double y_bits = 0, z_bits = 0;
};

// ... 18 lines not shown
  bool dry = false;
  std::vector<float> vbr_host;
  bool vbr_on = false;
  const float* gplane = nullptr;
  std::vector<EncodedImage> enc;
  int32_t* h_sym = nullptr;
  int16_t* h_sym16 = nullptr;
  uint8_t* h_idx8 = nullptr;
  size_t h_cap = 0;
  hipStream_t cst = nullptr;
  hipEvent_t cev = nullptr;
  int32_t* hc_sym = nullptr;
  int16_t* hc_sym16 = nullptr;
  uint8_t* hc_idx8 = nullptr;
  size_t hc_cap = 0;
  bool phase_d2h = false;
  struct ProfRec {
    hipEvent_t a, b;
    int cat;
    double flops, bytes;
    std::string tag;
  };
  bool prof = false;
  int* rflag = nullptr;
  int prec_force = -1;
  std::vector<ProfRec> recs;
  std::vector<hipEvent_t> ev_pool;
  size_t ev_used = 0;
  ~Lane();
};

class Model {
 public:
  Model(const std::string& name, int n, const char* const* names, const float* const* ptrs, const int64_t* shapes,
        const int* ndims, hipStream_t st);
  ~Model();
  const Cfg& cfg() const { return cfg_; }
  HostStats& host_stats() { return hstats_; }
  HostPool& host_pool();

  void forward(const float* x, int B, int H, int W, float* x_hat, float* y_lik, float* z_lik, const float* vbr_scales,
               hipStream_t st, const float* gain_plane = nullptr);
  void compress(const float* x, int B, int H, int W, const float* vbr_scales, hipStream_t st,
                const float* gain_plane = nullptr);
  const EncodedImage& encoded(int b) const { return enc_all_.at(b); }
  void decompress(const uint8_t* const* y, const size_t* ylen, const uint8_t* const* z, const size_t* zlen, int B,
                  int hz, int wz, float* x_hat, const float* vbr_scales, hipStream_t st, bool batch_stream = false,
                  const float* gain_plane = nullptr);
  std::string batch_stream(int first, int count) const;
  void set_tables(const CdfTables& gc, const CdfTables& eb) {
    gc_ = gc;
    eb_ = eb;
  }
  size_t arena_bytes() const;
  void set_profiling(bool on);
  void set_lanes(int n);
  void set_precision(int p) { precision_ = p; }
  int precision() const { return precision_; }
  void set_synthesis_precision(int p) { gs_fp16_ = p == 1; }
  int synthesis_precision() const { return gs_fp16_ ? 1 : 0; }
  int lanes() const { return nlanes_; }
  void set_priority_base(int b) { prio_base_ = b; }
  void set_poison(bool on) { poison_ = on; }
  struct Fallbacks {
    std::atomic<int64_t> forward_full{0}, forward_gs{0}, decompress_gs{0};
  };
  Fallbacks& fallbacks() { return fb_; }
  ProfStat profile_read(int cat);
  std::string profile_layers();
  size_t weight_bytes() const { return wbytes_; }
  void run_module(const std::string& which, int idx, const float* in0, const float* in1, int B, int Cin, int H, int W,
                  float* out, hipStream_t st);

 private:
  enum class Mode { Forward, Encode, Decode };
  Cfg cfg_;
  std::map<std::string, ConvW> convs_;
  std::map<std::string, ChainW> chains_;
  std::map<std::string, ChainW> chains_ctx_;
  ConvW hoist_;
  int hoist_rows_ = 0;
  bool hoist_on() const;
  void add_hoist(const std::map<std::string, std::pair<const float*, int>>& ep0, hipStream_t st);
  ConvW make_conv(const float* w_dev, int Cout, int Cin, int K, const std::string& name, hipStream_t st);
  void add_chains(hipStream_t st);
  bool range_hit(Lane& l);
  void range_clear(Lane& l);
  int prec() const { return L().prec_force >= 0 ? L().prec_force : precision_; }
  void run_chain(const ChainW& c, const std::vector<View>& ins, const View& out, const View* res,
                 const View* aux = nullptr, int H = 0, int W = 0, int ckbd = 0, bool sq_in = false);
  bool chain_on() const;
  bool dwpw_on() const;
  std::map<std::string, DwW> dws_;
  std::map<std::string, const float*> raw_;
  std::vector<void*> owned_;
  size_t wbytes_ = 0;
  float* scale_table_ = nullptr;
  int* rel_index_ = nullptr;
  CdfTables gc_, eb_;
  std::vector<EncodedImage> enc_all_;
  std::vector<std::unique_ptr<Lane>> lanes_;
  int nlanes_ = 4;
  int prio_base_ = 0;
  int precision_ = PREC_F16X3_V2;
  bool gs_fp16_ = false;
  HostStats hstats_;
  bool prof_ = false;
  bool poison_ = false;
  Fallbacks fb_;
  void gs_fp32_rerun(Lane& l, const View& yhat, const View& out, int B);
  static thread_local Lane* tl_lane_;
  Lane& L() const { return *tl_lane_; }
  Lane& lane(int i);
  hipEvent_t next_event();
  template <class F>
  void timed(int cat, double flops, double bytes, F&& launch, const std::string& tag = std::string());
  template <class F>
  void over_lanes(int B, hipStream_t caller, F&& fn, int max_lanes = 16);
  void compress_lane(const float* x, int B, int H, int W);
  void decompress_lane(const uint8_t* const* y, const size_t* ylen, const uint8_t* const* z, const size_t* zlen,
                       int B, int hz, int wz, float* x_hat, bool batch_stream);

  const ConvW& cw(const std::string& k) const;
  const DwW& dww(const std::string& k) const;
  const float* rw(const std::string& k) const;
  bool has(const std::string& k) const { return convs_.count(k) || dws_.count(k) || raw_.count(k); }

  View alloc(int C, int H, int W);
  void conv(const std::vector<View>& ins, const ConvW& w, int stride, int pad, const View& out, int epi,
            const View* aux = nullptr, const View* res = nullptr);
  ConvParams conv_params(const std::vector<View>& ins, const ConvW& w, int stride, int pad, const View& out, int epi,
                         const View* aux, const View* res);
  void run_conv(const ConvParams& P, const ConvW& w, const _Float16* packed, bool hi = false, bool split = false);
  void linatt_reproject(const View& k, const View& v, const View& q, int heads, int hd, int kmask, int qmask,
                        const ConvW& rp, const View& a, const std::string& tag);
  void add_fusion_x4(const std::string& base, const float* w_dev, int Cout, hipStream_t st);
  void add_taps(const std::string& base, const float* w_dev, int Cin, hipStream_t st);
  bool taps_on() const;
  void conv_pair(const std::vector<View>& ins, const ConvW& w1, const View& out1, int epi1, const ConvW& w2,
                 const View& out2, int epi2);
  DwParams dw_params(const std::vector<View>& ins, const DwW& w, int stride, const View& out, bool gelu, int ckbd);
  void dw(const std::vector<View>& ins, const DwW& w, int stride, const View& out, bool gelu, int ckbd = 0);
  bool dw_pw_half(const std::vector<View>& ins, const DwW& d, bool gelu, const ConvW& w, int epi, int mask_epi,
                  const View& out, const View* res, int ckbd, bool fusable);
  View conv3x3(const std::vector<View>& ins, const std::string& p, int stride, bool dwsep, int epi,
               const View* res = nullptr, const View* out = nullptr);
  View conv1x1(const View& in, const std::string& p, int stride, int epi, const View* res = nullptr);
  void gdn(const View& x, const std::string& p, bool inverse, const View& out, const View* res);
  View rbws(const View& x, const std::string& p, bool dwsep);
  View rb(const View& x, const std::string& p, bool dwsep);
  View rbu(const View& x, const std::string& p);
  View g_a(const View& x);
  View h_a(const View& y);
  View h_s(const View& z_hat);
  void g_s(const View& y_hat, const View& out);
  View local_context(const View& x, int i, bool half = false);
  bool ep_half_chain(const std::string& kind, int i, int H, int W, bool hoisted) const;
  View channel_context(const View& x, int i);
  View inter_context(const View& x, int i);
  View intra_context(const View& x1, const View& x2, int i, bool half = false);
  View entropy_parameters(const std::vector<View>& ctx, const View* hyper, const std::string& kind, int i,
                          const View* hoisted = nullptr, bool phase_only = false);
  void lrp(const std::vector<View>& ins, const std::string& kind, int i, const View& yh_slice, bool anchor);
  View qkv_branch(const View& x, const std::string& p);
  void slice_loop(Mode mode, const View& hyper, const View* y, const View& yhat, float* y_lik, const CoderBufs* cb,
                  class PhaseDecoder* dec);
  void eb(const View& z, const View& z_hat, float* z_lik, int32_t* z_sym);

  template <class F>
  void planned(int B, hipStream_t st, F&& body);
  void ensure_host(size_t n);
  void ensure_chost(size_t n);
  static int phase_d2h_mode();
  void set_vbr(const float* scales, int B, const float* gain_plane = nullptr);
  bool enc_plane_ = false;
};

}
```

mlic_amd/csrc/options.cpp:

```cpp
#include "options.h"

#include <atomic>
#include <cstdlib>
#include <cstring>
#include <stdexcept>
#include <string>

namespace mlic {
namespace {

int env_int(const char* e, int d) { return e ? std::atoi(e) : d; }
int raw(int v, const char* e, int d) { return v >= 0 ? v : env_int(e, d); }
int flag(int v, const char* e, int d) { return v >= 0 ? v != 0 : env_int(e, d) != 0; }
int lead0(int, const char* e, int) { return !(e && e[0] == '0'); }
int is1(int, const char* e, int d) { return env_int(e, d) == 1; }
int str(int, const char* e, int) { return e != nullptr; }
int halo(int v, const char* e, int d) { return v >= 0 ? (v == 0 ? 0 : 2) : env_int(e, d); }
int nj(int v, const char* e, int d) { return (v > 0 ? v : env_int(e, d)) == 2 ? 2 : 1; }
int narrow(int v, const char*, int d) { return v <= 0 || v > d ? d : v; }

struct Row {
  const char* name;
  const char* env;
  int dflt;
  int (*rule)(int v, const char* e, int d);
};
const Row kRows[] = {
    {"x4_halo", "MLIC_X4_HALO", 1, halo},
    {"x4_splitk", "MLIC_X4_SPLITK", 0, flag},
    {"linatt_fused", "MLIC_LINATT_FUSED", 1, flag},
    {"dw_strip", "MLIC_DW_STRIP", 1, flag},
    {"ep_half", "MLIC_EP_HALF", 1, flag},
    {"chain_nj", "MLIC_CHAIN_NJ", 1, nj},
    {"dwpw2", "MLIC_DWPW2", 2, raw},
    {"pw3", "MLIC_PW3", 1, raw},
    {"narrow_limit", nullptr, 32767, narrow},
    {"image_io_path", nullptr, -1, raw},
    {"lrp_half", "MLIC_LRP_HALF", 0, flag},
    {"intra_half", "MLIC_INTRA_HALF", 0, raw},
    {"gdn_skip", "MLIC_GDN_SKIP", 1, flag},
    {nullptr, "MLIC_X4", 1, flag},           {nullptr, "MLIC_X4_K", 0, str},
    {nullptr, "MLIC_X4_BM_FOR", 0, str},     {nullptr, "MLIC_X4_BM96", 1, lead0},
    {nullptr, "MLIC_X4_BM224", 1, lead0},    {nullptr, "MLIC_X4_RS", 1, flag},
    {nullptr, "MLIC_X4_DIRECT", 1, flag},    {nullptr, "MLIC_X4_ABL", 0, raw},
    {nullptr, "MLIC_V2_WIDE", 1, flag},      {nullptr, "MLIC_LOCAL_ATTN_VALU", 0, flag},
    {nullptr, "MLIC_TAPS", 1, flag},         {nullptr, "MLIC_HOIST", -1, raw},
    {nullptr, "MLIC_DWPW", 1, flag},         {nullptr, "MLIC_CHAIN", 1, flag},
    {nullptr, "MLIC_LA_PACKED", 1, flag},    {nullptr, "MLIC_LANE_PRIORITY", 1, flag},
    {nullptr, "MLIC_PHASE_D2H", 0, raw},     {nullptr, "MLIC_HOST_THREADS", 0, raw},
    {nullptr, "MLIC_POOL_PRIO", 2, raw},     {nullptr, "MLIC_LANES", 0, raw},
    {nullptr, "MLIC_PRECISION", 0, raw},     {nullptr, "MLIC_SYNTH_FP16", 0, is1},
    {nullptr, "MLIC_POISON", 0, flag},
};
static_assert(sizeof(kRows) / sizeof(kRows[0]) == OPT_COUNT, "one row per Opt");

struct {
  std::atomic<int> v{-1};
} g_set[OPT_SETTABLE];

struct Env {
  bool has[OPT_COUNT];
  std::string text[OPT_COUNT];
  int frozen[OPT_COUNT];
  Env() {
    for (int i = 0; i < OPT_COUNT; ++i) {
      const char* e = kRows[i].env ? std::getenv(kRows[i].env) : nullptr;
      has[i] = e != nullptr;
      if (e) text[i] = e;
      frozen[i] = kRows[i].rule(-1, e, kRows[i].dflt);
    }
  }
  const char* get(int i) const { return has[i] ? text[i].c_str() : nullptr; }
};
const Env& env() {
  static const Env e;
  return e;
}

Opt find(const char* name) {
  for (int i = 0; i < OPT_SETTABLE; ++i)
    if (std::strcmp(name, kRows[i].name) == 0) return (Opt)i;
  throw std::runtime_error(std::string("mlic: unknown kernel option ") + name);
}

}

int opt_live(Opt o) {
  const Env& e = env();
  if (o >= OPT_SETTABLE) return e.frozen[o];
  return kRows[o].rule(g_set[o].v.load(std::memory_order_relaxed), e.get(o), kRows[o].dflt);
}

const char* opt_str(Opt o) { return env().get(o); }

void opt_set(const char* name, int value) {
  const Opt o = find(name);
  if (o == OPT_IMAGE_IO_PATH && (value < -1 || value > 2))
    throw std::runtime_error("mlic: image_io_path must be -1 (by layout), 0, 1 or 2");
  g_set[o].v.store(value, std::memory_order_relaxed);
}

int opt_get(const char* name) { return opt_live(find(name)); }

OptionScope::OptionScope() : owner_(tl_opt_snap == nullptr) {
  if (!owner_) return;
  for (int i = 0; i < OPT_COUNT; ++i) vals_[i] = opt_live((Opt)i);
  tl_opt_snap = vals_;
}

OptionScope::OptionScope(const int* snap) : owner_(tl_opt_snap == nullptr && snap != nullptr) {
  if (owner_) tl_opt_snap = snap;
}

}
```

mlic_amd/csrc/options.h:

```cpp
#pragma once

namespace mlic {

enum Opt : int {
  OPT_X4_HALO, OPT_X4_SPLITK, OPT_LINATT_FUSED, OPT_DW_STRIP, OPT_EP_HALF, OPT_CHAIN_NJ, OPT_DWPW2, OPT_PW3,
  OPT_NARROW_LIMIT, OPT_IMAGE_IO_PATH, OPT_LRP_HALF, OPT_INTRA_HALF, OPT_GDN_SKIP,
  OPT_SETTABLE,
  OPT_X4 = OPT_SETTABLE, OPT_X4_K, OPT_X4_BM_FOR, OPT_X4_BM96, OPT_X4_BM224, OPT_X4_RS, OPT_X4_DIRECT, OPT_X4_ABL,
  OPT_V2_WIDE, OPT_LOCAL_ATTN_VALU, OPT_TAPS, OPT_HOIST, OPT_DWPW, OPT_CHAIN, OPT_LA_PACKED, OPT_LANE_PRIORITY,
  OPT_PHASE_D2H, OPT_HOST_THREADS, OPT_POOL_PRIO, OPT_LANES, OPT_PRECISION, OPT_SYNTH_FP16, OPT_POISON,
  OPT_COUNT
};

int opt_live(Opt o);
const char* opt_str(Opt o);
void opt_set(const char* name, int value);
int opt_get(const char* name);

inline thread_local const int* tl_opt_snap = nullptr;

inline int opt(Opt o) {
  const int* s = tl_opt_snap;
  return s ? s[o] : opt_live(o);
}

class OptionScope {
 public:
  OptionScope();
  explicit OptionScope(const int* snap);
  ~OptionScope() { if (owner_) tl_opt_snap = nullptr; }
  OptionScope(const OptionScope&) = delete;
  OptionScope& operator=(const OptionScope&) = delete;
  static const int* current() { return tl_opt_snap; }

 private:
  int vals_[OPT_COUNT];
  bool owner_;
};

}
```

Before: 116.2 images/sec.

## Group sibling 1x1 convs sharing an input into one stacked launch

Stacks the weights of sibling 1x1 convolutions that read the same input (q/k/v projections, mlp.0 with the skip branch, masked q/k) into one grouped weight block at load time. Each group then runs as a single pointwise or x4 launch with per-row-range weight exponents, partial GELU and anchor masking, followed by one shared depthwise pass. This is meant to read the input activation once instead of several times and to cut kernel launches. In exchange it adds extra template instantiations and per-row epilogue branching, and it falls back to the old path whenever shapes or the chosen kernel family do not match.

```diff
diff --git a/include/mlic_hip.h b/include/mlic_hip.h
--- a/include/mlic_hip.h
+++ b/include/mlic_hip.h
@@ -80,6 +80,8 @@
 
 int mlic_conv_run(void* stream, int impl, const float* x, const float* w, const float* bias, float* y, int B, int Cin,
                   int Cout, int H, int W, int K, int stride, int epi, const float* aux, const float* res);
+int mlic_conv_run_grouped(void* stream, int impl, const float* x, const float* w, const float* bias, float* y, int B,
+                          int Cin, int H, int W, int nmem, const int* rows, int act_rows, int mask_split);
 int mlic_conv_choice(int B, int Cin, int Cout, int H, int W, int K, int stride, int epi, int* impl);
 int mlic_dw_run(void* stream, const float* x, const float* w, const float* bias, float* y, int B, int C, int H, int W,
                 int stride, int gelu);
diff --git a/mlic_amd/_lib.py b/mlic_amd/_lib.py
--- a/mlic_amd/_lib.py
+++ b/mlic_amd/_lib.py
@@ -71,6 +71,7 @@
         "mlic_host_stats": [p, P(C.c_double), P(C.c_double), P(C.c_double), i],
         "mlic_profile_category_name": [i, p, sz],
         "mlic_conv_run": [p, i, p, p, p, p, i, i, i, i, i, i, i, i, p, p],
+        "mlic_conv_run_grouped": [p, i, p, p, p, p, i, i, i, i, i, P(i), i, i],
         "mlic_conv_choice": [i, i, i, i, i, i, i, i, P(i)],
         "mlic_dw_run": [p, p, p, p, p, i, i, i, i, i, i],
         "mlic_dwpw_run": [p, p, p, p, p, p, p, i, i, i, i, i, i, p],
diff --git a/mlic_amd/csrc/capi.cpp b/mlic_amd/csrc/capi.cpp
--- a/mlic_amd/csrc/capi.cpp
+++ b/mlic_amd/csrc/capi.cpp
@@ -568,6 +568,55 @@
   });
 }
 
+int mlic_conv_run_grouped(void* stream, int impl, const float* x, const float* w, const float* bias, float* y, int B,
+                          int Cin, int H, int W, int nmem, const int* rows, int act_rows, int mask_split) {
+  return guard([&] {
+    hipStream_t st = (hipStream_t)stream;
+    MLIC_CHECK(nmem >= 1 && nmem <= 3 && (impl == CONV_PW || impl == CONV_X4), "grouped conv: 1..3 members, impl 3 or 7");
+    int Cout = 0;
+    for (int k = 0; k < nmem; ++k) Cout += rows[k];
+    const int cin_pad = (Cin + 31) / 32 * 32;
+    const int64_t nh = (int64_t)Cout * cin_pad;
+    _Float16 *wh = nullptr, *wl = nullptr, *wx = nullptr;
+    HIP_OK(hipMallocAsync((void**)&wh, nh * 2, st));
+    HIP_OK(hipMallocAsync((void**)&wl, nh * 2, st));
+    ConvParams P{};
+    int r0 = 0;
+    for (int k = 0; k < nmem; ++k) {
+      const int e = split_weights(w + (int64_t)r0 * Cin, wh + (int64_t)r0 * cin_pad, wl + (int64_t)r0 * cin_pad, rows[k],
+                                  Cin, 1, cin_pad, true, st);
+      if (k == 0) P.wexp = e;
+      else {
+        P.grp_rows[k - 1] = r0;
+        P.grp_wexp[k - 1] = e;
+      }
+      r0 += rows[k];
+    }
+    P.nseg = 1;
+    P.seg[0] = {x, Cin, (int64_t)Cin * H * W};
+    P.Cin = Cin; P.H = H; P.W = W; P.Cout = Cout; P.Ho = H; P.Wo = W; P.K = 1; P.stride = 1; P.pad = 0;
+    P.bias = bias; P.out = y; P.B = B; P.epi = act_rows > 0 ? EPI_GELU : EPI_NONE;
+    P.out_cs = (int64_t)H * W;
+    P.out_bs = (int64_t)Cout * H * W;
+    P.act_rows = act_rows < Cout ? act_rows : 0;
+    P.mask_split = mask_split;
+    MLIC_CHECK(conv_grouped(P), "grouped conv: no grouped field set");
+    if (impl == CONV_X4) {
+      MLIC_CHECK(x4_grouped_ok(P, cin_pad), "x4: unsupported grouped shape");
+      HIP_OK(hipMallocAsync((void**)&wx, x4_weight_halves(Cout, 1, cin_pad) * 2, st));
+      x4_pack_weights(wh, wl, Cout, 1, cin_pad, wx, st);
+    } else {
+      MLIC_CHECK(pw_resident_ok(P, cin_pad), "pw_resident: unsupported grouped shape");
+    }
+    ConvWeights cw{nullptr, wh, wl, cin_pad, wx, P.wexp};
+    conv_run(impl, P, cw, st, nullptr);
+    if (wx) HIP_OK(hipFreeAsync(wx, st));
+    HIP_OK(hipFreeAsync(wh, st));
+    HIP_OK(hipFreeAsync(wl, st));
+    HIP_OK(hipStreamSynchronize(st));
+  });
+}
+
 int mlic_dw_run(void* stream, const float* x, const float* w, const float* bias, float* y, int B, int C, int H, int W,
                 int stride, int gelu) {
   return guard([&] {
diff --git a/mlic_amd/csrc/common.h b/mlic_amd/csrc/common.h
--- a/mlic_amd/csrc/common.h
+++ b/mlic_amd/csrc/common.h
@@ -88,7 +88,21 @@
   int sk_cin, sk_H, sk_W;
   const float* skw;
   const float* skb;
-};
+  int act_rows;
+  int mask_split;
+  int grp_rows[2];
+  int grp_wexp[2];
+};
+
+__host__ __device__ __forceinline__ bool conv_grouped(const ConvParams& P) {
+  return P.act_rows != 0 || P.mask_split != 0 || P.grp_rows[0] != 0;
+}
+__host__ __device__ __forceinline__ int conv_row_wexp(const ConvParams& P, int co) {
+  int e = P.wexp;
+  if (P.grp_rows[0] && co >= P.grp_rows[0]) e = P.grp_wexp[0];
+  if (P.grp_rows[1] && co >= P.grp_rows[1]) e = P.grp_wexp[1];
+  return e;
+}
 
 __device__ __forceinline__ float softmax_exp(float x) { return __builtin_amdgcn_exp2f(x * 1.44269504088896341f); }
 
@@ -159,12 +173,17 @@
 
 __device__ __forceinline__ bool is_anchor(int h, int w) { return ((h + w) & 1) == 1; }
 
+template <bool GX = false>
 __device__ __forceinline__ void conv_store(const ConvParams& P, int b, int co, int p, float v) {
   const int epi = P.epi;
   const int HWo = P.Ho * P.Wo;
-  v = ldexpf(v, -P.wexp);
+  v = ldexpf(v, -(GX ? conv_row_wexp(P, co) : P.wexp));
+  if (GX && P.mask_split) {
+    const int mh = p / P.Wo;
+    if (is_anchor(mh, p - mh * P.Wo) != (co >= P.mask_split)) v = 0.0f;
+  }
   if (P.bias) v += P.bias[co];
-  if (epi & EPI_GELU) v = gelu_epi(v);
+  if ((epi & EPI_GELU) && (!GX || P.act_rows == 0 || co < P.act_rows)) v = gelu_epi(v);
   if (epi & (EPI_GDN | EPI_IGDN)) {
     const float x = P.aux[(int64_t)b * P.aux_bs + (int64_t)co * HWo + p];
     v = gdn_apply(x, v, (epi & EPI_GDN) == 0);
@@ -195,14 +214,20 @@
   return (a & 15) == 0 && ((P.out_bs | P.out_cs | P.aux_bs | P.res_bs) & 3) == 0 && (P.Wo & 3) == 0;
 }
 
+template <bool GX = false>
 __device__ __forceinline__ void conv_store4(const ConvParams& P, int b, int co, int p, float4 v) {
   const int epi = P.epi;
   float a[4] = {v.x, v.y, v.z, v.w};
   const float bi = P.bias ? P.bias[co] : 0.0f;
+  const int wexp = GX ? conv_row_wexp(P, co) : P.wexp;
+  const bool act = (epi & EPI_GELU) && (!GX || P.act_rows == 0 || co < P.act_rows);
+  const int mh = (GX && P.mask_split) ? p / P.Wo : 0, mw = p - mh * P.Wo;
 #pragma unroll
   for (int e = 0; e < 4; ++e) {
-    a[e] = ldexpf(a[e], -P.wexp) + bi;
-    if (epi & EPI_GELU) a[e] = gelu_epi(a[e]);
+    a[e] = ldexpf(a[e], -wexp);
+    if (GX && P.mask_split && is_anchor(mh, mw + e) != (co >= P.mask_split)) a[e] = 0.0f;
+    a[e] = a[e] + bi;
+    if (act) a[e] = gelu_epi(a[e]);
   }
   if (epi & (EPI_GDN | EPI_IGDN)) {
     const float4 x = *reinterpret_cast<const float4*>(P.aux + (int64_t)b * P.aux_bs + (int64_t)co * P.Ho * P.Wo + p);
diff --git a/mlic_amd/csrc/conv_dispatch.cpp b/mlic_amd/csrc/conv_dispatch.cpp
--- a/mlic_amd/csrc/conv_dispatch.cpp
+++ b/mlic_amd/csrc/conv_dispatch.cpp
@@ -60,6 +60,8 @@
   P.wexp = split ? w.wexp : 0;
   MLIC_CHECK(!(P.epi & EPI_RELU_IN) || impl == CONV_X4 || impl == CONV_X4H,
              "EPI_RELU_IN: only x4's operand pack applies it");
+  MLIC_CHECK(!conv_grouped(P) || impl == CONV_PW || impl == CONV_X4,
+             "grouped launches: the resident and the x4 1x1 kernels only");
   switch (impl) {
     case CONV_F32: conv_forward(P, st); break;
     case CONV_X3: conv_f16x3_forward(P, w.wh, w.wl, w.cin_pad, st); break;
diff --git a/mlic_amd/csrc/conv_pw.hip b/mlic_amd/csrc/conv_pw.hip
--- a/mlic_amd/csrc/conv_pw.hip
+++ b/mlic_amd/csrc/conv_pw.hip
@@ -23,7 +23,7 @@
 template <int CIN>
 constexpr int pw_apitch() { return CIN + 8; }
 
-template <int CIN, int CT, int MODE, bool RES, int XF = 0>
+template <int CIN, int CT, int MODE, bool RES, int XF = 0, bool GX = false>
 __global__ __launch_bounds__(PW_THREADS) void pw_resident_kernel(ConvParams P, const _Float16* __restrict__ wh,
                                                                   const _Float16* __restrict__ wl, int cin_pad) {
   constexpr int KS = CIN / 16;
@@ -196,6 +196,11 @@
     const auto rs_res = make_rsrc(res ? P.res + (int64_t)b * P.res_bs : P.out, res ? (uint32_t)P.Cout * cs4 : 0u);
     const float* sb = sbias + 4 * h;
     const float unscale = ldexpf(1.0f, -P.wexp);
+    bool anc = false;
+    if (GX) {
+      const int oh = p / P.Wo;
+      anc = is_anchor(oh, p - oh * P.Wo);
+    }
     uint32_t so_o = 0, so_a = 0;
     if (p < HW) {
 #pragma unroll
@@ -218,13 +223,16 @@
 #pragma unroll
         for (int g = 0; g < 4; ++g) bq[g] = *reinterpret_cast<const float4*>(sb + c * 32 + 8 * g);
         float v[16];
+        const float unscale_c = GX ? ldexpf(1.0f, -conv_row_wexp(P, 32 * c)) : unscale;
+        const bool gelu_c = gelu && (!GX || P.act_rows == 0 || 32 * c < P.act_rows);
+        const bool keep_c = !GX || P.mask_split == 0 || anc == (32 * c >= P.mask_split);
 #pragma unroll
         for (int r = 0; r < 16; ++r) {
           const float4 b4 = bq[r >> 2];
           const float bv = (r & 3) == 0 ? b4.x : (r & 3) == 1 ? b4.y : (r & 3) == 2 ? b4.z : b4.w;
-          float x = __builtin_fmaf(acc[c][r], unscale, bv);
+          float x = __builtin_fmaf(GX ? (keep_c ? acc[c][r] : 0.0f) : acc[c][r], GX ? unscale_c : unscale, bv);
           bad |= !(fabsf(x) <= 3.4e38f);
-          if (gelu) x = gelu_erf(x);
+          if (GX ? gelu_c : gelu) x = gelu_erf(x);
           if (gdn) x = gdn_apply(xa[r], x, igdn);
           if (tanh_mask) x = keep ? 0.5f * tanhf(x) : 0.0f;
           v[r] = x + xr[r];
@@ -294,6 +302,7 @@
         \
   X(96, 4, 1, 0) X(64, 4, 1, 0) X(128, 2, 0, 1) X(96, 2, 0, 0)
 #define PW_XCOMBOS(X) X(32, 1, 0, 0, 1) X(128, 1, 4, 1, 2) X(128, 2, 0, 1, 2)
+#define PW_GCOMBOS(X) X(32, 3, 0, 0) X(64, 6, 0, 0) X(96, 9, 0, 0) X(96, 6, 1, 0) X(32, 2, 0, 0)
 
 static int pw_xf(const ConvParams& P) { return (P.in_mask ? 1 : 0) | (P.scatter ? 2 : 0); }
 
@@ -308,6 +317,16 @@
   if ((int64_t)P.Cin * HW * 4 >= (1ll << 31) || (int64_t)P.Cout * HW * 4 >= (1ll << 31)) return false;
   const int ct = (P.Cout + 31) / 32;
   const int res = (P.epi & EPI_RES) ? 1 : 0;
+  if (conv_grouped(P)) {
+    if (P.stride != 1 || pw_xf(P) || P.Cout % 32 != 0 || (P.act_rows | P.mask_split | P.grp_rows[0] | P.grp_rows[1]) % 32 != 0 ||
+        P.act_rows < 0 || P.mask_split < 0 || P.grp_rows[0] < 0 || P.grp_rows[1] < 0)
+      return false;
+#define MLIC_PW_GOK(CIN, CT, M, R) \
+  if (P.Cin == CIN && ct == CT && mode == M && res == R) return true;
+    PW_GCOMBOS(MLIC_PW_GOK)
+#undef MLIC_PW_GOK
+    return false;
+  }
   if (const int xf = pw_xf(P)) {
     if (P.stride != 1 || (unsigned)P.in_mask > 2u || (unsigned)P.scatter > 2u) return false;
     if (P.scatter && ((P.epi & (EPI_MASK_ANCHOR | EPI_MASK_NONANCHOR)) || P.out_cs != 2 * HW ||
@@ -326,12 +345,12 @@
   return false;
 }
 
-template <int CIN, int CT, int M, bool R, int XF = 0>
+template <int CIN, int CT, int M, bool R, int XF = 0, bool GX = false>
 static void launch_pw(const ConvParams& P, const _Float16* wh, const _Float16* wl, int cin_pad, hipStream_t st) {
   const int64_t ntiles = (int64_t)((P.Ho * P.Wo + 31) / 32) * P.B;
   const int64_t want = (ntiles + PW_WAVES - 1) / PW_WAVES;
   const dim3 grid((unsigned)std::min<int64_t>(want, (int64_t)num_cus()));
-  hipLaunchKernelGGL((pw_resident_kernel<CIN, CT, M, R, XF>), grid, dim3(PW_THREADS), 0, st, P, wh, wl, cin_pad);
+  hipLaunchKernelGGL((pw_resident_kernel<CIN, CT, M, R, XF, GX>), grid, dim3(PW_THREADS), 0, st, P, wh, wl, cin_pad);
   HIP_OK(hipGetLastError());
 }
 
@@ -340,6 +359,15 @@
   const int mode = pw_mode(P);
   const int ct = (P.Cout + 31) / 32;
   const int res = (P.epi & EPI_RES) ? 1 : 0;
+  if (conv_grouped(P)) {
+#define MLIC_PW_GRUN(CIN, CT, M, R)                                 \
+  if (P.Cin == CIN && ct == CT && mode == M && res == R) {          \
+    launch_pw<CIN, CT, M, R != 0, 0, true>(P, wh, wl, cin_pad, st); \
+    return;                                                         \
+  }
+    PW_GCOMBOS(MLIC_PW_GRUN)
+#undef MLIC_PW_GRUN
+  }
   if (const int xf = pw_xf(P)) {
 #define MLIC_PW_XRUN(CIN, CT, M, R, X)                                 \
   if (P.Cin == CIN && ct == CT && mode == M && res == R && xf == X) {  \
diff --git a/mlic_amd/csrc/conv_x4.hip b/mlic_amd/csrc/conv_x4.hip
--- a/mlic_amd/csrc/conv_x4.hip
+++ b/mlic_amd/csrc/conv_x4.hip
@@ -66,7 +66,7 @@
 #ifndef MLIC_X4_STAGGER
 #define MLIC_X4_STAGGER 0
 #endif
-template <int K, int BM, bool RS, bool HI, bool DIR = false, bool HALO = false>
+template <int K, int BM, bool RS, bool HI, bool DIR = false, bool HALO = false, bool GX = false>
 __global__ __launch_bounds__(X4T) void conv_x4_kernel(ConvParams P, const _Float16* __restrict__ act,
                                                       const _Float16* __restrict__ wx, int nchunk, int H, int W,
                                                       int abl, int nsplit) {
@@ -515,12 +515,12 @@
       if (oy >= H || ox >= W || p >= npix) continue;
       if (!shuf) {
         if (vec && co < P.Cout && ox + 3 < W && p + 3 < npix) {
-          conv_store4(P, b, co, p, v);
+          conv_store4<GX>(P, b, co, p, v);
         } else if (co < P.Cout) {
           const float vs[4] = {v.x, v.y, v.z, v.w};
 #pragma unroll
           for (int e = 0; e < 4; ++e)
-            if (ox + e < W && p + e < npix) conv_store(P, b, co, p + e, vs[e]);
+            if (ox + e < W && p + e < npix) conv_store<GX>(P, b, co, p + e, vs[e]);
         }
       } else {
         if (vec && co + 1 < P.Cout && ox + 1 < W) {
@@ -835,6 +835,11 @@
   return opt(OPT_X4_DIRECT) && P.K == 1 && !hi && !(P.epi & (EPI_SQUARE_IN | EPI_RELU_IN)) && x4_rs();
 }
 
+bool x4_grouped_ok(const ConvParams& P, int cin_pad) {
+  return conv_x4_ok(P, cin_pad) && x4_direct_ok(P, false) && !(P.epi & EPI_SHUFFLE) && P.act_rows >= 0 &&
+         P.mask_split >= 0 && P.grp_rows[0] >= 0 && P.grp_rows[1] >= 0;
+}
+
 template <int K, int BM>
 static void launch_x4(const ConvParams& P, const _Float16* act, const _Float16* wx, int nchunk, hipStream_t st,
                       int nsplit, bool hi) {
@@ -843,7 +848,11 @@
   const int ntx = (W + TC - 1) / TC, nty = (H + TR - 1) / TR;
   dim3 grid((P.Cout + BM - 1) / BM, ntx * nty, P.B * nsplit);
   const int abl = opt(OPT_X4_ABL);
-  if (K == 1 && !act)
+  if (K == 1 && !act && conv_grouped(P)) {
+    if constexpr (K == 1)
+      hipLaunchKernelGGL((conv_x4_kernel<K, BM, true, false, true, false, true>), grid, dim3(X4T), 0, st, P, act, wx,
+                         nchunk, H, W, abl, nsplit);
+  } else if (K == 1 && !act)
     hipLaunchKernelGGL((conv_x4_kernel<K, BM, true, false, K == 1>), grid, dim3(X4T), 0, st, P, act, wx, nchunk, H, W,
                        abl, nsplit);
   else if (hi && x4_halo(P, hi)) {
@@ -887,6 +896,7 @@
 void conv_x4_forward(const ConvParams& P, const _Float16* act, const _Float16* wx, int cin_pad, hipStream_t st,
                      float* part, bool hi) {
   MLIC_CHECK(conv_x4_ok(P, cin_pad) && wx && (act || x4_direct_ok(P, hi)), "conv_x4: unsupported shape");
+  MLIC_CHECK(!conv_grouped(P) || x4_grouped_ok(P, cin_pad), "conv_x4: grouped launches run on the 1x1 direct form");
   ConvParams Q = P;
   if (act) Q.epi &= ~(EPI_SQUARE_IN | EPI_RELU_IN);
   const int nchunk = x4_nchunk(cin_pad, hi);
diff --git a/mlic_amd/csrc/kernels.h b/mlic_amd/csrc/kernels.h
--- a/mlic_amd/csrc/kernels.h
+++ b/mlic_amd/csrc/kernels.h
@@ -53,6 +53,7 @@
 bool conv_x4_ok(const ConvParams& P, int cin_pad);
 void x4_pack_act(const ConvParams& P, int cin_pad, _Float16* dst, hipStream_t st, bool hi = false);
 bool x4_direct_ok(const ConvParams& P, bool hi);
+bool x4_grouped_ok(const ConvParams& P, int cin_pad);
 int x4_splitk(const ConvParams& P, int cin_pad, bool hi = false);
 int64_t x4_part_bytes(const ConvParams& P, int cin_pad, bool hi = false);
 void conv_x4_forward(const ConvParams& P, const _Float16* act, const _Float16* wx, int cin_pad, hipStream_t st,
diff --git a/mlic_amd/csrc/model.cpp b/mlic_amd/csrc/model.cpp
--- a/mlic_amd/csrc/model.cpp
+++ b/mlic_amd/csrc/model.cpp
@@ -221,6 +221,7 @@
   }
   add_chains(st);
   add_hoist(ep0, st);
+  add_groups(st);
   MLIC_CHECK(raw_.count("__scale_table"), "scale table missing");
   scale_table_ = const_cast<float*>(raw_["__scale_table"]);
   HIP_OK(hipStreamSynchronize(st));
@@ -411,6 +412,122 @@
   return want && chain_on() && hoist_.Cout > 0;
 }
 
+void Model::add_groups(hipStream_t st) {
+  auto stack = [&](const std::string& name, const std::vector<std::string>& mem) {
+    std::vector<const ConvW*> ms;
+    for (const std::string& k : mem) {
+      auto it = convs_.find(k);
+      if (it == convs_.end()) return;
+      ms.push_back(&it->second);
+    }
+    int rows = 0;
+    for (const ConvW* m : ms) {
+      if (m->K != 1 || !m->wh || m->Cin != ms[0]->Cin || m->cin_pad != ms[0]->cin_pad) return;
+      rows += m->Cout;
+    }
+    ConvW g;
+    g.Cin = ms[0]->Cin;
+    g.cin_pad = ms[0]->cin_pad;
+    g.Cout = rows;
+    g.K = 1;
+    g.wexp = ms[0]->wexp;
+    g.name = name;
+    const size_t nh = ((size_t)rows * g.cin_pad * 2 + 255) / 256 * 256;
+    const size_t nb = ((size_t)rows * 4 + 255) / 256 * 256;
+    const size_t nx = rows >= 64 ? (size_t)x4_weight_halves(rows, 1, g.cin_pad) * 2 : 0;
+    char* blk = nullptr;
+    HIP_OK(hipMalloc(&blk, 2 * nh + nb + nx + 256));
+    owned_.push_back(blk);
+    wbytes_ += 2 * nh + nb + nx + 256;
+    g.wh = reinterpret_cast<_Float16*>(blk);
+    g.wl = reinterpret_cast<_Float16*>(blk + nh);
+    float* bias = reinterpret_cast<float*>(blk + 2 * nh);
+    HIP_OK(hipMemsetAsync(bias, 0, nb, st));
+    int r0 = 0;
+    for (size_t k = 0; k < ms.size(); ++k) {
+      const ConvW* m = ms[k];
+      const size_t n = (size_t)m->Cout * g.cin_pad * 2;
+      HIP_OK(hipMemcpyAsync(g.wh + (size_t)r0 * g.cin_pad, m->wh, n, hipMemcpyDeviceToDevice, st));
+      HIP_OK(hipMemcpyAsync(g.wl + (size_t)r0 * g.cin_pad, m->wl, n, hipMemcpyDeviceToDevice, st));
+      if (m->b) HIP_OK(hipMemcpyAsync(bias + r0, m->b, (size_t)m->Cout * 4, hipMemcpyDeviceToDevice, st));
+      if (k > 0) {
+        g.grp_rows[k - 1] = r0;
+        g.grp_wexp[k - 1] = m->wexp;
+      }
+      r0 += m->Cout;
+    }
+    g.b = bias;
+    if (nx) {
+      g.wx4 = reinterpret_cast<_Float16*>(blk + 2 * nh + nb);
+      x4_pack_weights(g.wh, g.wl, rows, 1, g.cin_pad, g.wx4, st);
+    }
+    convs_[name] = g;
+  };
+  auto stack_dw = [&](const std::string& name, const std::vector<std::string>& mem) {
+    std::vector<const DwW*> ms;
+    int C = 0;
+    for (const std::string& k : mem) {
+      auto it = dws_.find(k);
+      if (it == dws_.end()) return;
+      ms.push_back(&it->second);
+      C += it->second.C;
+    }
+    float* blk = nullptr;
+    HIP_OK(hipMalloc(&blk, (size_t)C * 10 * 4));
+    owned_.push_back(blk);
+    wbytes_ += (size_t)C * 10 * 4;
+    HIP_OK(hipMemsetAsync(blk, 0, (size_t)C * 10 * 4, st));
+    DwW g;
+    g.w = blk;
+    g.b = blk + (size_t)C * 9;
+    g.C = C;
+    g.name = name;
+    int c0 = 0;
+    bool any_bias = false;
+    for (const DwW* m : ms) {
+      HIP_OK(hipMemcpyAsync(blk + (size_t)c0 * 9, m->w, (size_t)m->C * 9 * 4, hipMemcpyDeviceToDevice, st));
+      if (m->b) HIP_OK(hipMemcpyAsync(blk + (size_t)C * 9 + c0, m->b, (size_t)m->C * 4, hipMemcpyDeviceToDevice, st));
+      any_bias = any_bias || m->b;
+      c0 += m->C;
+    }
+    for (const DwW* m : ms)
+      if ((m->b != nullptr) != any_bias) return;
+    if (!any_bias) g.b = nullptr;
+    dws_[name] = g;
+  };
+  for (int i = 0; i < cfg_.S; ++i) {
+    const std::string pi = "global_inter_context." + std::to_string(i), pa = "global_intra_context." + std::to_string(i);
+    stack(pi + ".qkv.0", {pi + ".queries.0", pi + ".keys.0", pi + ".values.0"});
+    stack_dw(pi + ".qkv.1", {pi + ".queries.1", pi + ".keys.1", pi + ".values.1"});
+    stack(pi + ".skipmlp", {pi + ".mlp.0", pi + ".skip"});
+    stack(pa + ".qk.0", {pa + ".queries.0", pa + ".keys.0"});
+    stack_dw(pa + ".qk.1", {pa + ".queries.1", pa + ".keys.1"});
+  }
+}
+
+bool Model::conv_group(const View& x, const ConvW& g, const std::vector<const ConvW*>& mem, int act_rows,
+                       int mask_split, const View& out) {
+  if (prec() != PREC_F16X3_V2 || !g.wh) return false;
+  int fam = -1, r0 = 0;
+  for (const ConvW* m : mem) {
+    const View geo{nullptr, m->Cout, x.H, x.W, (int64_t)m->Cout * x.hw()};
+    const ConvParams PM = conv_params({x}, *m, 1, 0, geo, r0 < act_rows ? EPI_GELU : EPI_NONE, nullptr, nullptr);
+    const ConvWeights cwt{m->w, m->wh, m->wl, m->cin_pad, m->wx4, m->wexp};
+    const int f = conv_select(PM, cwt, prec());
+    if (f == CONV_PW && pw3_ok(PM, m->cin_pad)) return false;
+    if (fam >= 0 && f != fam) return false;
+    fam = f;
+    r0 += m->Cout;
+  }
+  if (fam != CONV_PW && fam != CONV_X4) return false;
+  ConvParams PG = conv_params({x}, g, 1, 0, out, act_rows > 0 ? EPI_GELU : EPI_NONE, nullptr, nullptr);
+  PG.act_rows = act_rows < g.Cout ? act_rows : 0;
+  PG.mask_split = mask_split;
+  if (fam == CONV_PW ? !pw_resident_ok(PG, g.cin_pad) : !(g.wx4 && x4_grouped_ok(PG, g.cin_pad))) return false;
+  run_conv(PG, g, nullptr, false, false, fam, 4.0 * (mem.size() - 1) * L().B * (double)x.C * x.hw());
+  return true;
+}
+
 bool Model::dwpw_on() const {
   return opt(OPT_DWPW) && prec() == PREC_F16X3_V2;
 }
@@ -525,13 +642,14 @@
   L().arena.release(m);
 }
 
-void Model::run_conv(const ConvParams& P, const ConvW& w, const _Float16* packed, bool hi, bool split) {
+void Model::run_conv(const ConvParams& P, const ConvW& w, const _Float16* packed, bool hi, bool split, int force,
+                     double extra_bytes) {
   const ConvWeights cw{w.w, w.wh, w.wl, w.cin_pad, w.wx4, w.wexp};
-  const int impl = packed ? (hi ? CONV_X4H : CONV_X4) : conv_select(P, cw, prec());
+  const int impl = packed ? (hi ? CONV_X4H : CONV_X4) : force >= 0 ? force : conv_select(P, cw, prec());
   const double outn = (double)P.B * w.Cout * P.Ho * P.Wo;
   const double flops = 2.0 * outn * P.Cin * w.K * w.K;
   const double bytes = 4.0 * ((double)P.B * P.Cin * P.H * P.W + (double)w.Cout * P.Cin * w.K * w.K +
-                              outn * (1 + (P.aux ? 1 : 0) + (P.res ? 1 : 0)));
+                              outn * (1 + (P.aux ? 1 : 0) + (P.res ? 1 : 0))) + extra_bytes;
   std::string tag;
   if (L().prof) {
     char sh[96];
@@ -577,6 +695,10 @@
   P.Wo = (P.W + 2 * pad - w.K) / stride + 1;
   P.wpk = w.w;
   P.wexp = w.wexp;
+  for (int g = 0; g < 2; ++g) {
+    P.grp_rows[g] = w.grp_rows[g];
+    P.grp_wexp[g] = w.grp_wexp[g];
+  }
   P.rflag = L().rflag;
   P.bias = w.b;
   P.epi = epi;
@@ -993,16 +1115,55 @@
   const ConvW& sk = cw(p + ".skip");
   View out = alloc(sk.Cout, H, W);
   const size_t m = L().arena.mark();
-  View q = qkv_branch(x, p + ".queries");
-  View k = qkv_branch(x, p + ".keys");
-  View v = qkv_branch(x, p + ".values");
+  const int grp = opt(OPT_CTX_GROUP);
+  View q, k, v;
+  bool qkv_done = false;
+  if ((grp & 1) && convs_.count(p + ".qkv.0") && dws_.count(p + ".qkv.1")) {
+    const ConvW& g = cw(p + ".qkv.0");
+    const DwW& gd = dww(p + ".qkv.1");
+    const ConvW &wq = cw(p + ".queries.0"), &wk = cw(p + ".keys.0"), &wv = cw(p + ".values.0");
+    const size_t m2 = L().arena.mark();
+    View o = alloc(gd.C, H, W);
+    const size_t m3 = L().arena.mark();
+    View t = alloc(g.Cout, H, W);
+    if (gd.C == g.Cout && wq.Cout == D && wk.Cout == D && wv.Cout == D && conv_group(x, g, {&wq, &wk, &wv}, 0, 0, t)) {
+      dw({t}, gd, 1, o, false);
+      L().arena.release(m3);
+      q = o.ch(0, D);
+      k = o.ch(D, D);
+      v = o.ch(2 * D, D);
+      qkv_done = true;
+    } else {
+      L().arena.release(m2);
+    }
+  }
+  if (!qkv_done) {
+    q = qkv_branch(x, p + ".queries");
+    k = qkv_branch(x, p + ".keys");
+    v = qkv_branch(x, p + ".values");
+  }
   const ConvW& rp = cw(p + ".reprojection");
   View a = alloc(rp.Cout, H, W);
   linatt_reproject(k, v, q, heads, hd, 0, 0, rp, a, p + ".attn");
-  View m1 = conv1x1(a, p + ".mlp.0", 1, EPI_GELU);
+  View m1, s;
+  bool sm_done = false;
+  if ((grp & 2) && convs_.count(p + ".skipmlp")) {
+    const ConvW& g = cw(p + ".skipmlp");
+    const ConvW& w0 = cw(p + ".mlp.0");
+    const size_t m2 = L().arena.mark();
+    View ms = alloc(g.Cout, H, W);
+    if (conv_group(a, g, {&w0, &sk}, w0.Cout, 0, ms)) {
+      m1 = ms.ch(0, w0.Cout);
+      s = ms.ch(w0.Cout, sk.Cout);
+      sm_done = true;
+    } else {
+      L().arena.release(m2);
+    }
+  }
+  if (!sm_done) m1 = conv1x1(a, p + ".mlp.0", 1, EPI_GELU);
   View m2 = alloc(m1.C, H, W);
   dw({m1}, dww(p + ".mlp.2"), 1, m2, true);
-  View s = conv1x1(a, p + ".skip", 1, EPI_NONE);
+  if (!sm_done) s = conv1x1(a, p + ".skip", 1, EPI_NONE);
   conv({m2}, cw(p + ".mlp.4"), 1, 0, out, EPI_NONE, nullptr, &s);
   L().arena.release(m);
   return out;
@@ -1070,7 +1231,25 @@
   View q, k;
   {
     const size_t m2 = L().arena.mark();
-    if (!masked_branch(p + ".queries", 2, q) || !masked_branch(p + ".keys", 1, k)) {
+    bool grouped = false;
+    if (!on && (opt(OPT_CTX_GROUP) & 4) && convs_.count(p + ".qk.0") && dws_.count(p + ".qk.1")) {
+      const ConvW& g = cw(p + ".qk.0");
+      const DwW& gd = dww(p + ".qk.1");
+      const ConvW &wq = cw(p + ".queries.0"), &wk = cw(p + ".keys.0");
+      View o = alloc(gd.C, H, W);
+      const size_t m3 = L().arena.mark();
+      View t = alloc(g.Cout, H, W);
+      if (gd.C == g.Cout && wq.Cout == D && wk.Cout == D && conv_group(x1, g, {&wq, &wk}, 0, wq.Cout, t)) {
+        dw({t}, gd, 1, o, false);
+        L().arena.release(m3);
+        q = o.ch(0, D);
+        k = o.ch(D, D);
+        grouped = true;
+      } else {
+        L().arena.release(m2);
+      }
+    }
+    if (!grouped && (!masked_branch(p + ".queries", 2, q) || !masked_branch(p + ".keys", 1, k))) {
       L().arena.release(m2);
       View x1n = alloc(D, H, W);
       View x1a = alloc(D, H, W);
diff --git a/mlic_amd/csrc/model.h b/mlic_amd/csrc/model.h
--- a/mlic_amd/csrc/model.h
+++ b/mlic_amd/csrc/model.h
@@ -33,6 +33,8 @@
   _Float16* wx4 = nullptr;
   _Float16* wx4h = nullptr;
   int wexp = 0;
+  int grp_rows[2] = {0, 0};
+  int grp_wexp[2] = {0, 0};
   std::string name;
 };
 
@@ -217,6 +219,9 @@
   int hoist_rows_ = 0;
   bool hoist_on() const;
   void add_hoist(const std::map<std::string, std::pair<const float*, int>>& ep0, hipStream_t st);
+  void add_groups(hipStream_t st);
+  bool conv_group(const View& x, const ConvW& g, const std::vector<const ConvW*>& mem, int act_rows, int mask_split,
+                  const View& out);
   ConvW make_conv(const float* w_dev, int Cout, int Cin, int K, const std::string& name, hipStream_t st);
   void add_chains(hipStream_t st);
   bool range_hit(Lane& l);
@@ -266,7 +271,8 @@
             const View* aux = nullptr, const View* res = nullptr);
   ConvParams conv_params(const std::vector<View>& ins, const ConvW& w, int stride, int pad, const View& out, int epi,
                          const View* aux, const View* res);
-  void run_conv(const ConvParams& P, const ConvW& w, const _Float16* packed, bool hi = false, bool split = false);
+  void run_conv(const ConvParams& P, const ConvW& w, const _Float16* packed, bool hi = false, bool split = false,
+                int force = -1, double extra_bytes = 0.0);
   void linatt_reproject(const View& k, const View& v, const View& q, int heads, int hd, int kmask, int qmask,
                         const ConvW& rp, const View& a, const std::string& tag);
   void add_fusion_x4(const std::string& base, const float* w_dev, int Cout, hipStream_t st);
diff --git a/mlic_amd/csrc/options.cpp b/mlic_amd/csrc/options.cpp
--- a/mlic_amd/csrc/options.cpp
+++ b/mlic_amd/csrc/options.cpp
@@ -39,6 +39,7 @@
     {"lrp_half", "MLIC_LRP_HALF", 0, flag},
     {"intra_half", "MLIC_INTRA_HALF", 0, raw},
     {"gdn_skip", "MLIC_GDN_SKIP", 1, flag},
+    {"ctx_group", "MLIC_CTX_GROUP", 7, raw},
     {nullptr, "MLIC_X4", 1, flag},           {nullptr, "MLIC_X4_K", 0, str},
     {nullptr, "MLIC_X4_BM_FOR", 0, str},     {nullptr, "MLIC_X4_BM96", 1, lead0},
     {nullptr, "MLIC_X4_BM224", 1, lead0},    {nullptr, "MLIC_X4_RS", 1, flag},
diff --git a/mlic_amd/csrc/options.h b/mlic_amd/csrc/options.h
--- a/mlic_amd/csrc/options.h
+++ b/mlic_amd/csrc/options.h
@@ -4,7 +4,7 @@
 
 enum Opt : int {
   OPT_X4_HALO, OPT_X4_SPLITK, OPT_LINATT_FUSED, OPT_DW_STRIP, OPT_EP_HALF, OPT_CHAIN_NJ, OPT_DWPW2, OPT_PW3,
-  OPT_NARROW_LIMIT, OPT_IMAGE_IO_PATH, OPT_LRP_HALF, OPT_INTRA_HALF, OPT_GDN_SKIP,
+  OPT_NARROW_LIMIT, OPT_IMAGE_IO_PATH, OPT_LRP_HALF, OPT_INTRA_HALF, OPT_GDN_SKIP, OPT_CTX_GROUP,
   OPT_SETTABLE,
   OPT_X4 = OPT_SETTABLE, OPT_X4_K, OPT_X4_BM_FOR, OPT_X4_BM96, OPT_X4_BM224, OPT_X4_RS, OPT_X4_DIRECT, OPT_X4_ABL,
   OPT_V2_WIDE, OPT_LOCAL_ATTN_VALU, OPT_TAPS, OPT_HOIST, OPT_DWPW, OPT_CHAIN, OPT_LA_PACKED, OPT_LANE_PRIORITY,
```

Result: no change. 117.1 images/sec, median of 2 (+0.8%).
